# yangliu9527/Object_SLAM

Measured on AMD Instinct MI355X. Metric: frames/sec tracking+localBA, higher is better.
Workload: dtype f64

## Files before the change

include/oslam_hip.h:

```cpp
#ifndef OSLAM_HIP_H
#define OSLAM_HIP_H

#include <stddef.h>
#include <stdint.h>

#ifdef __cplusplus
extern "C" {
#endif

#define OSLAM_OK 0
#define OSLAM_E_INVALID (-1)
#define OSLAM_E_HIP (-2)
#define OSLAM_E_CAPACITY (-3)
#define OSLAM_E_NUMERIC (-4)

#define OSLAM_MAX_LEVELS 16

typedef struct oslam_keypoint {
    float x, y;
    float size;
    float angle;
    float response;
    int32_t octave;
    int32_t class_id;
} oslam_keypoint_t;

const char* oslam_last_error(void);
int oslam_device_count(void);

typedef struct oslam_orb oslam_orb_t;

int oslam_orb_create(oslam_orb_t** out, int nfeatures, float scaleFactor, int nlevels, int iniThFAST,
                     int minThFAST, int width, int height, int max_batch, int device);
void oslam_orb_destroy(oslam_orb_t* h);

int oslam_orb_get_scale_tables(const oslam_orb_t* h, float* scaleFactors, float* invScaleFactors,
                               float* levelSigma2, float* invLevelSigma2, int* nFeaturesPerLevel);
int oslam_orb_set_blur_rounding(oslam_orb_t* h, int sse2);
int oslam_orb_max_keypoints(const oslam_orb_t* h);

int oslam_orb_extract(oslam_orb_t* h, const uint8_t* gray, int width, int height, int stride,
                      oslam_keypoint_t* keypoints, uint8_t* descriptors, int cap, int* n_out);

int oslam_orb_extract_batch_device(oslam_orb_t* h, const uint8_t* d_gray, int batch, int stride,
                                   size_t image_stride, void* stream);
int oslam_orb_results_device(const oslam_orb_t* h, const oslam_keypoint_t** d_keypoints,
                             const uint8_t** d_descriptors, const int32_t** d_counts,
                             const int32_t** d_status);
int oslam_orb_fetch(oslam_orb_t* h, int b, oslam_keypoint_t* keypoints, uint8_t* descriptors, int cap,
                    int* n_out);

int oslam_orb_level_size(const oslam_orb_t* h, int level, int* width, int* height);
int oslam_orb_get_pyramid_level(oslam_orb_t* h, int b, int level, uint8_t* out);
int oslam_orb_pyramid_level_device(const oslam_orb_t* h, int b, int level, const uint8_t** d_ptr,
                                   int* pitch);

int oslam_orb_debug_get_blurred(oslam_orb_t* h, int b, int level, uint8_t* out);
int oslam_orb_debug_get_candidates(oslam_orb_t* h, int b, int level, int32_t* out, int cap, int* n_out);
int oslam_orb_debug_get_level_keys(oslam_orb_t* h, int b, int level, int32_t* out, int cap, int* n_out);

#define OSLAM_ORB_RESIZE_NONE 0
#define OSLAM_ORB_RESIZE_PLAIN 1
#define OSLAM_ORB_RESIZE_WORDS 2
#define OSLAM_ORB_RESIZE_LDS 3
typedef struct oslam_orb_plan {
    int32_t nlevels;
    int32_t batch;
    int32_t n_halves;
    int32_t half_nb[2];
    int32_t half_kpw[2];
    int32_t half_src_aligned4[2];
    int32_t half_src_aligned16[2];
    int32_t half_oct_nodes_hbm[2];
    int32_t half_big_cell_kernel[2];
    int32_t half_resize[2][OSLAM_MAX_LEVELS];
    int32_t big_cell[OSLAM_MAX_LEVELS];
    int32_t skipped_cells[OSLAM_MAX_LEVELS];
} oslam_orb_plan_t;
int oslam_orb_debug_get_plan(const oslam_orb_t* h, oslam_orb_plan_t* out);

int oslam_orb_set_profiling(oslam_orb_t* h, int on);
int oslam_orb_get_profile(oslam_orb_t* h, double ms[5], long long* batches, long long* images);

int oslam_orb_debug_counters(oslam_orb_t* h, unsigned long long out[16], int reset);

int oslam_memcpy_from_device(void* dst, const void* d_src, size_t bytes);
int64_t oslam_orb_algorithmic_bytes(const oslam_orb_t* h, int n_keypoints);
// ... 119 lines not shown
                       float bf, float b, float* uRight, float* depth);
int oslam_stereo_match_batch_device(oslam_stereo_t* h, oslam_orb_t* orbL, oslam_orb_t* orbR, int batch, int kp_stride,
                                    const oslam_keypoint_t* d_kpL, const uint8_t* d_descL, const int32_t* d_nL,
                                    int nL_const, const oslam_keypoint_t* d_kpR, const uint8_t* d_descR,
                                    const int32_t* d_nR, int nR_const, int nlevels, float bf, float b, void* stream);
int oslam_stereo_results_device(const oslam_stereo_t* h, const float** d_uRight, const float** d_depth,
                                const int32_t** d_n_matched);

typedef struct oslam_poseopt oslam_poseopt_t;
int oslam_poseopt_create(oslam_poseopt_t** out, int max_batch, int max_points , int device);
void oslam_poseopt_destroy(oslam_poseopt_t* h);
int oslam_pose_optimize(oslam_poseopt_t* h, int N, const float Tcw_in[16], const float* Xw, const float* obs,
                        const float* invSigma2, const uint8_t* has_mp, const float K5[5], float Tcw_out[16],
                        uint8_t* outlier, int32_t* n_inliers, int32_t stats[2] );
int oslam_poseopt_trace(oslam_poseopt_t* h, int cap);
int oslam_poseopt_trace_read(oslam_poseopt_t* h, double* out, int32_t* n);
int oslam_pose_optimize_batch_device(oslam_poseopt_t* h, int batch, int stride, const int32_t* d_n, int n_const,
                                     const float* d_Tcw, const float* d_Xw, const float* d_obs,
                                     const float* d_invSigma2, const uint8_t* d_has_mp, const float K5[5],
                                     void* stream);
int oslam_poseopt_results_device(const oslam_poseopt_t* h, const float** d_Tcw_out, const uint8_t** d_outlier,
                                 const int32_t** d_n_inliers, const int32_t** d_stats);

typedef struct oslam_semantic {
    int32_t nObj, H, W;
    const uint8_t* masks;
    int32_t nObjMp; const float* objmp_Xw; const int32_t* objmp_obj;
    int32_t nJoint; const int32_t* joint_kp; const int32_t* joint_obj;
    const float* kp_uv;
    float bounds[4];
    float invSigma2_0;
} oslam_semantic_t;
int oslam_pose_optimize2(oslam_poseopt_t* h, int N, const float Tcw_in[16], const float* Xw, const float* obs,
                         const float* invSigma2, const uint8_t* has_mp, const float K5[5], const oslam_semantic_t* sem,
                         float Tcw_out[16], uint8_t* outlier, int32_t* n_inliers, int32_t* n_semantic);

typedef struct oslam_sem_frame { int32_t nObj, obj0, nObjMp, objmp0, nJoint, joint0; } oslam_sem_frame_t;
int oslam_pose_optimize2_batch_device(oslam_poseopt_t* h, int batch, int stride, const int32_t* d_n, const float* d_Tcw, const float* d_Xw, const float* d_obs,
                                      const float* d_invSigma2, const uint8_t* d_has_mp, const float K5[5], const oslam_sem_frame_t* d_frames, int total_obj,
                                      const uint8_t* const* d_mask_ptrs, int H, int W, int mask_pitch, int total_objmp, const float* d_objmp_Xw,
                                      const int32_t* d_objmp_obj, int total_joint, const int32_t* d_joint_kp, const int32_t* d_joint_obj, const float bounds[4],
                                      float invSigma2_0, void* stream);
int oslam_poseopt_semantic_results_device(const oslam_poseopt_t* h, const int32_t** d_n_semantic);
int oslam_mask_bits_device(const uint8_t* const* d_mask_ptrs, int n, int H, int W, int pitch, uint64_t* d_bits, void* stream);
int oslam_poseopt_use_mask_bits(oslam_poseopt_t* h, const uint64_t* d_bits, const int32_t* d_bits_index);
int oslam_frame_object_kp_test_bits_batch_device(const oslam_keypoint_t* d_keysUn, int kp_stride, const int32_t* d_n_kps, int batch, const uint64_t* d_bits,
                                                 const int32_t* d_mask0, const int32_t* d_n_masks, int H, int W, uint8_t* d_out, void* stream);
int oslam_frame_object_kp_test_batch_device(const oslam_keypoint_t* d_keysUn, int kp_stride, const int32_t* d_n_kps, int batch, const uint8_t* const* d_mask_ptrs,
                                            const int32_t* d_mask0, const int32_t* d_n_masks, int H, int W, int mask_pitch, uint8_t* d_out, void* stream);

typedef struct oslam_lba oslam_lba_t;
int oslam_lba_create(oslam_lba_t** out, int max_batch, int max_keyframes , int max_points,
                     int max_edges, int device);
void oslam_lba_destroy(oslam_lba_t* h);
volatile int32_t* oslam_lba_stop_flag(oslam_lba_t* h);
int oslam_lba_set_mode(oslam_lba_t* h, int wide);
int oslam_lba_set_schur(oslam_lba_t* h, int mode);
int oslam_lba_kernel_time(oslam_lba_t* h, int enable, double* ms_out, long long* launches_out);
int oslam_lba_trace(oslam_lba_t* h, int cap);
int oslam_lba_trace_read(oslam_lba_t* h, double* out, int32_t* n);
int oslam_lba_set_solver(oslam_lba_t* h, int mode);
int oslam_lba_debug_stats(oslam_lba_t* h, int32_t out[16]);
int oslam_lba_optimize(oslam_lba_t* h, int nKF, const float* poses, const uint8_t* fixed, int nP,
                       const float* points, int nE, const int32_t* edge_kf, const int32_t* edge_pt,
                       const float* edge_obs, const float* edge_invSigma2, const float K5[5], int use_stop_flag,
                       float* poses_out, float* points_out, uint8_t* erase,
                       int32_t stats[4] );

typedef struct oslam_lba_problem {
    int32_t nKF; const float* poses; const uint8_t* fixed;
    int32_t nP; const float* points;
    int32_t nE; const int32_t* edge_kf; const int32_t* edge_pt; const float* edge_obs; const float* edge_invSigma2;
    float* poses_out; float* points_out; uint8_t* erase; int32_t* stats;
} oslam_lba_problem_t;
int oslam_lba_optimize_batch(oslam_lba_t* h, int n, const oslam_lba_problem_t* probs, const float K5[5]);

int oslam_ba_optimize(oslam_lba_t* h, int nKF, const float* poses, const uint8_t* fixed, int nP, const float* points, int nE,
                      const int32_t* edge_kf, const int32_t* edge_pt, const float* edge_obs, const float* edge_invSigma2,
                      const float K5[5], int nIterations, int bRobust, int use_stop_flag, float* poses_out, float* points_out);

typedef struct oslam_mappoint oslam_mappoint_t;
int oslam_mappoint_create(oslam_mappoint_t** out, int device);
void oslam_mappoint_destroy(oslam_mappoint_t* h);
int oslam_bow_kernel_time(oslam_bow_t* h, int enable, double* ms_out, long long* launches_out);
int oslam_mappoint_kernel_time(oslam_mappoint_t* h, int enable, double* ms_out, long long* launches_out);

int oslam_mp_distinctive_descriptors(oslam_mappoint_t* h, int P, const int32_t* obs_start, const uint8_t* obs_desc ,
                                     int32_t* best_idx , uint8_t* out_desc );

int oslam_mp_update_normal_depth(oslam_mappoint_t* h, int P, const float* Pos , const int32_t* obs_start, const float* obs_Ow ,
                                 const float* OwRef , const float* levelScaleFactor , float lastScaleFactor, float* out );

int oslam_mp_update_fused_device(int P, int do_desc, int do_normal, const int32_t* d_obs_start, const int32_t* d_desc_start, const int32_t* d_rec, const uint8_t* const* d_rec_desc,
                                 const float* d_obs_Ow, const float* d_Pos, const float* d_OwRef, const float* d_lsf, float lastScale, const int32_t* d_items, uint8_t* const* d_tab,
                                 int32_t* o_best, uint8_t* o_desc, float* o_out5, void* stream);
int oslam_mp_update_windows_device(int P, const int32_t* d_items, uint8_t* const* d_tab, const int32_t* d_e0, const int32_t* d_ne, const int32_t* d_kbase, const int32_t* d_ref,
                                   const float* d_lsf, const uint8_t* d_skip, const float* d_Pos, const int32_t* d_edge_kf, const uint8_t* d_erase, const float* d_Ow, float lastScale,
                                   float* d_out5, void* stream);
int oslam_mp_table_write_device(int P, const int32_t* d_items, uint8_t* const* d_tab, const int32_t* d_obs_start, const int32_t* d_desc_start, const float* d_Pos,
                                const float* d_out5, const uint8_t* d_out_desc, int do_desc, int do_normal, void* stream);
int oslam_pose_inputs_gather_device(int batch, int stride, const int32_t* d_slots, const int32_t* d_n, const int32_t* d_ids, uint8_t* const* d_tab,
                                    const oslam_keypoint_t* d_keysUn, const float* d_uRight, int kp_stride, const float* invLevelSigma2, int nLevels,
                                    float* d_Xw, float* d_obs, float* d_invSigma2, uint8_t* d_has_mp, void* stream);
int oslam_fuse_queries_device(int n, int stride, const int32_t* d_slots, const int32_t* d_M, const int32_t* d_ids, const uint8_t* d_excl, uint8_t* const* d_tab,
                              const float* d_Tcw, const float* d_Ow, const float K5[5], const float bounds[4], float th, float logScaleFactor,
                              const float* scaleFactors, int nLevels, oslam_proj_query_t* d_q, void* stream);
// ... 649 lines not shown
```

include/oslam_slam.h:

```cpp
#ifndef OSLAM_SLAM_H
#define OSLAM_SLAM_H

#include "oslam_hip.h"

#ifdef __cplusplus
extern "C" {
#endif

typedef struct oslam_slam oslam_slam_t;

typedef struct oslam_slam_config {
    int32_t width, height;
    float fx, fy, cx, cy;
    float dist[5]; int32_t ndist;
    float bf;
    float thDepth;
    float fps;
    int32_t nFeatures; float scaleFactor; int32_t nLevels, iniThFAST, minThFAST;
    int32_t n_sequences;
    int32_t device;
    int32_t host_threads;
    int32_t local_mapping;
    int32_t sensor;
} oslam_slam_config_t;

#define OSLAM_SLAM_LM_DEFERRED 0x20
#define OSLAM_SLAM_NOT_INITIALIZED 1
#define OSLAM_SLAM_OK 2
#define OSLAM_SLAM_LOST 3

typedef struct oslam_slam_frame {
    int32_t N;
    oslam_keypoint_t* keys;
    oslam_keypoint_t* keysUn;
    uint8_t* desc;
    float* uRight;
    float* depth;
} oslam_slam_frame_t;

typedef struct oslam_job_search_last {
    int32_t slot;
    const oslam_slam_frame_t* cur;
    int32_t Nlast; const float* Xw; const uint8_t* has_mp; const oslam_keypoint_t* last_keysUn; const uint8_t* mp_desc;
    float Tcw[16], Tlw[16]; float th;
    int32_t* kp_match;
    int32_t nmatches;
    const int32_t* mp_ids;
} oslam_job_search_last_t;

typedef struct oslam_job_search_local {
    int32_t slot; const oslam_slam_frame_t* cur; const uint8_t* blocked ;
    int32_t M; const float* Pw; const float* Pn; const float* maxDist; const float* minDist; const uint8_t* obs_gt0; const uint8_t* mp_desc;
    float Tcw[16]; float th;
    const uint8_t* skip;
    int64_t content_id;
    uint8_t* in_view;
    int32_t* kp_match;
    int32_t nmatches;
    const int32_t* local_ids;
} oslam_job_search_local_t;

typedef struct oslam_job_pose {
    int32_t slot; int32_t N; float Tcw_in[16];
    const float* Xw; const float* obs; const float* invSigma2; const uint8_t* has_mp;
    float Tcw_out[16]; uint8_t* outlier; int32_t n_inliers;
    const int32_t* mp_ids;
} oslam_job_pose_t;

typedef struct oslam_job_mp_update {
    int32_t P; const int32_t* obs_start; const uint8_t* obs_desc; const float* obs_Ow;
    const float* Pos; const float* OwRef; const float* levelScaleFactor;
    int32_t do_desc, do_normal;
    const int32_t* items;
    const int32_t* desc_start;
    int32_t* best_idx; uint8_t* out_desc; float* out5;
} oslam_job_mp_update_t;

typedef struct oslam_job_mp_window {
    int32_t slot;
    int32_t nP, nE, nK;
    const int32_t* pt_ids;
    const int32_t* pt_start;
    const int32_t* edge_kf;
// ... 173 lines not shown
```

object_slam_amd/_lib.py:

```python
import contextlib
import ctypes as C
import os

import numpy as np

HERE = os.path.dirname(os.path.abspath(__file__))
LIB_PATH = os.environ.get("OSLAM_LIB_PATH") or os.path.join(HERE, "liboslam_hip.so")

KP_DTYPE = np.dtype([("x", "<f4"), ("y", "<f4"), ("size", "<f4"), ("angle", "<f4"),
                     ("response", "<f4"), ("octave", "<i4"), ("class_id", "<i4")])

OSLAM_E_INVALID, OSLAM_E_HIP, OSLAM_E_CAPACITY, OSLAM_E_NUMERIC = -1, -2, -3, -4


class OslamError(RuntimeError):
    def __init__(self, code, msg):
        super().__init__("oslam error %d: %s" % (code, msg))
        self.code = code


_lib = None


def lib():
    global _lib
    if _lib is None:
        if not os.path.exists(LIB_PATH):
            raise OslamError(OSLAM_E_HIP, "%s not built: run python -m object_slam_amd.build "
                             "(the HIP path has no CPU fallback)" % LIB_PATH)
        try:
            import torch
        except ImportError:
            pass
        L = C.CDLL(LIB_PATH)
        L.oslam_last_error.restype = C.c_char_p
        L.oslam_orb_algorithmic_bytes.restype = C.c_int64
        L.oslam_orb_algorithmic_bytes.argtypes = [C.c_void_p, C.c_int]
        L.oslam_orb_create.argtypes = [C.POINTER(C.c_void_p), C.c_int, C.c_float, C.c_int, C.c_int, C.c_int,
                                       C.c_int, C.c_int, C.c_int, C.c_int]
        L.oslam_orb_destroy.argtypes = [C.c_void_p]
        L.oslam_orb_extract_batch_device.argtypes = [C.c_void_p, C.c_void_p, C.c_int, C.c_int, C.c_size_t, C.c_void_p]
        _lib = L
    return _lib


def check(rc):
    if rc != 0:
        raise OslamError(rc, lib().oslam_last_error().decode())


def ptr(a):
    return C.c_void_p(a.__array_interface__["data"][0])


def optptr(a):
    return None if a is None else ptr(a)


class Handle:

    def __init__(self, L, prefix, *args):
        self.L, self.h, self._destroy = L, C.c_void_p(), prefix + "_destroy"
        check(getattr(L, prefix + "_create")(C.byref(self.h), *args))

    def close(self):
        h = getattr(self, "h", None)
        if h is not None and h.value:
            getattr(self.L, self._destroy)(h)
            h.value = None

    def __del__(self):
        try:
            self.close()
        except Exception:
            pass


def upload(a):
    if a is None:
        return None
    import torch
    return torch.from_numpy(np.ascontiguousarray(a).view(np.uint8).reshape(-1) if a.size else np.zeros(8, np.uint8)).to(torch.device("cuda", torch.cuda.current_device()))


@contextlib.contextmanager
def device_call(arrays, outputs):
    import torch
    t = {id(a): upload(a) for a in arrays if a is not None}
    torch.cuda.synchronize()
    side = torch.cuda.Stream()
    with torch.cuda.stream(side):
        yield (lambda a: None if a is None else t[id(a)].data_ptr()), C.c_void_p(side.cuda_stream)
    side.synchronize()
    for a in outputs:
        if a is not None and a.size:
            a.reshape(-1).view(np.uint8)[:] = t[id(a)].cpu().numpy()[:a.nbytes]
# ... 1 lines not shown
```

object_slam_amd/csrc/bow_matcher.hip:

```cpp
#include <hip/hip_runtime.h>
#include <stdint.h>

#include <algorithm>
#include <vector>

#include "common.h"
#include "slam_pool.h"

namespace oslam {

constexpr int kBowThreads = 1024;
constexpr int kBowMaxKps = 2400;
constexpr int kBowHisto = 30;

struct BowCtx {
    int mode;
    int nq; const int* q_idx1; const uint32_t* q_node;
    int N1; const oslam_keypoint_t* keys1; const uint8_t* desc1; const float* uRight1; const uint8_t* flag1;
    int N2; const oslam_keypoint_t* keys2; const uint8_t* desc2; const float* uRight2; const uint8_t* has_mp2;
    int nNodes; const uint32_t* nodes; const int* start; const int* items;
    float nnratio; int checkOri; int bOnlyStereo;
    float F12[9], ex, ey, scale[OSLAM_MAX_LEVELS], sigma2[OSLAM_MAX_LEVELS];
    int* out; int* nmatches; int* q_best;
};
// ... 146 lines not shown
            int bin = (int)roundf(rot * factor);
            if (bin == kBowHisto) bin = 0;
            if (bin != s_ind[0] && bin != s_ind[1] && bin != s_ind[2]) {
                removed++;
                if (c.mode == 0) c.out[k] = -2; else c.out[idx1] = c.mode == 2 ? -2 : -1;
            }
        }
        if (removed) atomicSub(&s_nm, removed);
        __syncthreads();
    }
    if (tid == 0) *c.nmatches = s_nm;
}

__global__ __launch_bounds__(kBowThreads) void k_search_bow(BowCtx c, int ncap) { bow_body(c, ncap); }
__global__ __launch_bounds__(kBowThreads) void k_search_bow_batch(const BowCtx* cs, int ncap) { bow_body(cs[blockIdx.x], ncap); }

}

using namespace oslam;

struct oslam_bow {
    int device = 0, max_kps = 0;
    size_t lds = 0;
    DeviceBuffer q_idx1, q_node, keys1, desc1, ur1, flag1, keys2, desc2, ur2, mp2, nodes, start, items, out, qbest, nm;
    StagePair st;
    hipStream_t strm = nullptr;
    bool owns_strm = true;
    int timing = 0; hipEvent_t ev0 = nullptr, ev1 = nullptr; double kern_ms = 0; long long kern_n = 0;
};

static int bow_up(DeviceBuffer& b, const void* src, size_t bytes) {
    int rc = b.grow(bytes ? bytes : 4, 256);
    if (rc) return rc;
    if (bytes && src) OSLAM_HIP_CHECK(hipMemcpy(b.ptr(), src, bytes, hipMemcpyHostToDevice));
    return OSLAM_OK;
}

extern "C" {

int oslam_bow_kernel_time(oslam_bow_t* h, int enable, double* ms_out, long long* launches_out) {
    if (!h) { set_error("NULL handle"); return OSLAM_E_INVALID; }
    OSLAM_HIP_CHECK(hipSetDevice(h->device));
    if (enable && !h->ev0) { OSLAM_HIP_CHECK(hipEventCreate(&h->ev0)); OSLAM_HIP_CHECK(hipEventCreate(&h->ev1)); }
    if (ms_out) *ms_out = h->kern_ms;
    if (launches_out) *launches_out = h->kern_n;
    h->kern_ms = 0; h->kern_n = 0; h->timing = enable;
    return OSLAM_OK;
}

void oslam_bow_destroy(oslam_bow_t* h) {
    if (!h) return;
    if (h->ev0) (void)hipEventDestroy(h->ev0);
    if (h->ev1) (void)hipEventDestroy(h->ev1);
    if (h->strm && h->owns_strm) (void)hipStreamDestroy(h->strm);
    delete h;
}

extern "C++" {
namespace oslam {
void bow_use_stream(oslam_bow* h, hipStream_t s) {
    if (!h || !s) return;
    if (h->strm && h->owns_strm) (void)hipStreamDestroy(h->strm);
    h->strm = s; h->owns_strm = false;
}
}
}

int oslam_bow_create(oslam_bow_t** out, int max_keypoints, int device) {
    if (!out) { set_error("out is NULL"); return OSLAM_E_INVALID; }
    *out = nullptr;
    if (max_keypoints < 1 || max_keypoints > kBowMaxKps) { set_error("oslam_bow_create: max_keypoints must be in [1,%d]", kBowMaxKps); return OSLAM_E_INVALID; }
    int ndev = oslam_device_count();
    if (ndev <= 0) { set_error("no HIP device visible: the gfx950 BoW matchers have no CPU fallback"); return OSLAM_E_HIP; }
    if (device < 0 || device >= ndev) { set_error("device out of range"); return OSLAM_E_INVALID; }
    OSLAM_HIP_CHECK(hipSetDevice(device));
    oslam_bow* h = new oslam_bow();
    h->device = device; h->max_kps = max_keypoints;
    h->lds = (size_t)max_keypoints * 40 + 64;
    OSLAM_HIP_CHECK(hipFuncSetAttribute((const void*)k_search_bow, hipFuncAttributeMaxDynamicSharedMemorySize, (int)h->lds));
    *out = h;
    return OSLAM_OK;
}

static int bow_run(oslam_bow_t* h, int mode, const oslam_bow_side1_t* s1, const oslam_bow_side2_t* s2, float nnratio, int checkOri,
                   const float* F12, float ex, float ey, const float* scaleFactors, const float* levelSigma2, int nlevels, int bOnlyStereo,
                   int32_t* out, int32_t* nmatches) {
    if (!h || !s1 || !s2 || !out || !nmatches) { set_error("NULL argument"); return OSLAM_E_INVALID; }
    if (s1->N < 0 || s2->N < 0 || s1->nq < 0 || s2->nNodes < 0 || s2->N > h->max_kps || s1->N > 65536 * 16) { set_error("keypoint counts exceed capacity %d", h->max_kps); return OSLAM_E_CAPACITY; }
    for (int q = 0; q < s1->nq; q++)
        if (s1->q_idx[q] < 0 || s1->q_idx[q] >= s1->N) { set_error("side-1 index out of range"); return OSLAM_E_INVALID; }
    const int nitems = s2->nNodes ? s2->start[s2->nNodes] : 0;
    for (int i = 0; i < nitems; i++)
        if (s2->items[i] < 0 || s2->items[i] >= s2->N) { set_error("side-2 index out of range"); return OSLAM_E_INVALID; }
    for (int i = 1; i < s2->nNodes; i++)
        if (!(s2->nodes[i - 1] < s2->nodes[i])) { set_error("side-2 node ids must be strictly ascending"); return OSLAM_E_INVALID; }
    OSLAM_HIP_CHECK(hipSetDevice(h->device));
    int rc;
    std::vector<float> negs((size_t)std::max(std::max(s1->N, s2->N), 1), -1.0f);
    std::vector<uint8_t> zeros((size_t)std::max(std::max(s1->N, s2->N), 1), 0);
    if ((rc = bow_up(h->q_idx1, s1->q_idx, (size_t)s1->nq * 4)) || (rc = bow_up(h->q_node, s1->q_node, (size_t)s1->nq * 4)) ||
        (rc = bow_up(h->keys1, s1->keys, (size_t)s1->N * sizeof(oslam_keypoint_t))) || (rc = bow_up(h->desc1, s1->desc, (size_t)s1->N * 32)) ||
        (rc = bow_up(h->ur1, s1->uRight ? s1->uRight : negs.data(), (size_t)s1->N * 4)) || (rc = bow_up(h->flag1, s1->flag ? s1->flag : zeros.data(), (size_t)s1->N)) ||
        (rc = bow_up(h->keys2, s2->keys, (size_t)s2->N * sizeof(oslam_keypoint_t))) || (rc = bow_up(h->desc2, s2->desc, (size_t)s2->N * 32)) ||
        (rc = bow_up(h->ur2, s2->uRight ? s2->uRight : negs.data(), (size_t)s2->N * 4)) || (rc = bow_up(h->mp2, s2->has_mp ? s2->has_mp : zeros.data(), (size_t)s2->N)) ||
        (rc = bow_up(h->nodes, s2->nodes, (size_t)s2->nNodes * 4)) || (rc = bow_up(h->start, s2->start, (size_t)(s2->nNodes + 1) * 4)) ||
        (rc = bow_up(h->items, s2->items, (size_t)nitems * 4)) || (rc = h->out.grow((size_t)std::max(std::max(s1->N, s2->N), 1) * 4, 256)) ||
        (rc = h->qbest.grow((size_t)std::max(s1->nq, 1) * 4, 256)) || (rc = h->nm.grow(4, 256)))
        return rc;
    BowCtx c;
    memset(&c, 0, sizeof(c));
    c.mode = mode; c.nq = s1->nq; c.q_idx1 = (const int*)h->q_idx1.ptr(); c.q_node = (const uint32_t*)h->q_node.ptr();
    c.N1 = s1->N; c.keys1 = (const oslam_keypoint_t*)h->keys1.ptr(); c.desc1 = (const uint8_t*)h->desc1.ptr(); c.uRight1 = (const float*)h->ur1.ptr(); c.flag1 = (const uint8_t*)h->flag1.ptr();
    c.N2 = s2->N; c.keys2 = (const oslam_keypoint_t*)h->keys2.ptr(); c.desc2 = (const uint8_t*)h->desc2.ptr(); c.uRight2 = (const float*)h->ur2.ptr(); c.has_mp2 = (const uint8_t*)h->mp2.ptr();
    c.nNodes = s2->nNodes; c.nodes = (const uint32_t*)h->nodes.ptr(); c.start = (const int*)h->start.ptr(); c.items = (const int*)h->items.ptr();
    c.nnratio = nnratio; c.checkOri = checkOri; c.bOnlyStereo = bOnlyStereo;
// ... 69 lines not shown
        Off& o = off[i];
        o.nitems = nitems; o.nout = jobs[i].triangulation ? s1.N : s2.N;
        const bool r1 = res && res[i].d_keys1 && res[i].d_desc1, r2 = res && res[i].d_keys2 && res[i].d_desc2;
        const bool u1 = r1 && res[i].d_uRight1 && s1.uRight, u2 = r2 && res[i].d_uRight2 && s2.uRight;
        o.q_idx = take((size_t)s1.nq * 4); o.q_node = take((size_t)s1.nq * 4);
        o.keys1 = r1 ? 0 : take((size_t)s1.N * sizeof(oslam_keypoint_t)); o.desc1 = r1 ? 0 : take((size_t)s1.N * 32);
        o.ur1 = u1 ? 0 : take((size_t)s1.N * 4); o.flag1 = take((size_t)s1.N);
        o.keys2 = r2 ? 0 : take((size_t)s2.N * sizeof(oslam_keypoint_t)); o.desc2 = r2 ? 0 : take((size_t)s2.N * 32);
        o.ur2 = u2 ? 0 : take((size_t)s2.N * 4); o.mp2 = take((size_t)s2.N); o.nodes = take((size_t)s2.nNodes * 4); o.start = take((size_t)(s2.nNodes + 1) * 4);
        o.items = take((size_t)nitems * 4);
    }
    const size_t in_bytes = at;
    for (int i = 0; i < n; i++) { off[i].out = take((size_t)std::max(off[i].nout, 1) * 4); off[i].nm = take(4); }
    const size_t io_bytes = at;
    for (int i = 0; i < n; i++) off[i].qbest = take((size_t)std::max(jobs[i].s1.nq, 1) * 4);
    OSLAM_HIP_CHECK(hipSetDevice(h->device));
    if (at > h->st.cap()) OSLAM_HIP_CHECK(hipDeviceSynchronize());
    OSLAM_CHECK(h->st.grow(at, 0));
    uint8_t* H = h->st.h.bytes();
    uint8_t* D = h->st.d.bytes();
    BowCtx* cs = (BowCtx*)H;
    oslam_drv::shared_parallel_for(n, [&](int i) {
        const oslam_bow_job_t& j = jobs[i];
        const oslam_bow_side1_t& s1 = j.s1;
        const oslam_bow_side2_t& s2 = j.s2;
        const Off& o = off[i];
        memcpy(H + o.q_idx, s1.q_idx, (size_t)s1.nq * 4); memcpy(H + o.q_node, s1.q_node, (size_t)s1.nq * 4);
        if (o.keys1) { memcpy(H + o.keys1, s1.keys, (size_t)s1.N * sizeof(oslam_keypoint_t)); memcpy(H + o.desc1, s1.desc, (size_t)s1.N * 32); }
        if (o.ur1) { if (s1.uRight) memcpy(H + o.ur1, s1.uRight, (size_t)s1.N * 4); else for (int k = 0; k < s1.N; k++) ((float*)(H + o.ur1))[k] = -1.0f; }
        if (s1.flag) memcpy(H + o.flag1, s1.flag, (size_t)s1.N); else memset(H + o.flag1, 0, (size_t)s1.N);
        if (o.keys2) { memcpy(H + o.keys2, s2.keys, (size_t)s2.N * sizeof(oslam_keypoint_t)); memcpy(H + o.desc2, s2.desc, (size_t)s2.N * 32); }
        if (o.ur2) { if (s2.uRight) memcpy(H + o.ur2, s2.uRight, (size_t)s2.N * 4); else for (int k = 0; k < s2.N; k++) ((float*)(H + o.ur2))[k] = -1.0f; }
        if (s2.has_mp) memcpy(H + o.mp2, s2.has_mp, (size_t)s2.N); else memset(H + o.mp2, 0, (size_t)s2.N);
        memcpy(H + o.nodes, s2.nodes, (size_t)s2.nNodes * 4);
        if (s2.nNodes) memcpy(H + o.start, s2.start, (size_t)(s2.nNodes + 1) * 4); else *(int*)(H + o.start) = 0;
        memcpy(H + o.items, s2.items, (size_t)o.nitems * 4);
        BowCtx& c = cs[i];
        memset(&c, 0, sizeof(c));
        c.mode = j.triangulation == 2 ? 2 : (j.triangulation ? 1 : 0); c.nq = s1.nq; c.q_idx1 = (const int*)(D + o.q_idx); c.q_node = (const uint32_t*)(D + o.q_node);
        c.N1 = s1.N; c.keys1 = o.keys1 ? (const oslam_keypoint_t*)(D + o.keys1) : res[i].d_keys1; c.desc1 = o.desc1 ? D + o.desc1 : res[i].d_desc1;
        c.uRight1 = o.ur1 ? (const float*)(D + o.ur1) : res[i].d_uRight1; c.flag1 = D + o.flag1;
        c.N2 = s2.N; c.keys2 = o.keys2 ? (const oslam_keypoint_t*)(D + o.keys2) : res[i].d_keys2; c.desc2 = o.desc2 ? D + o.desc2 : res[i].d_desc2;
        c.uRight2 = o.ur2 ? (const float*)(D + o.ur2) : res[i].d_uRight2; c.has_mp2 = D + o.mp2;
        c.nNodes = s2.nNodes; c.nodes = (const uint32_t*)(D + o.nodes); c.start = (const int*)(D + o.start); c.items = (const int*)(D + o.items);
        c.nnratio = j.nnratio; c.checkOri = j.checkOri; c.bOnlyStereo = 0;
        for (int k = 0; k < 9; k++) c.F12[k] = j.F12[k];
        c.ex = j.ex; c.ey = j.ey;
        for (int k = 0; k < OSLAM_MAX_LEVELS; k++) {
            c.scale[k] = (scaleFactors && k < nlevels) ? scaleFactors[k] : 0.f;
            c.sigma2[k] = (levelSigma2 && k < nlevels) ? levelSigma2[k] : 0.f;
        }
        c.out = (int*)(D + o.out); c.nmatches = (int*)(D + o.nm); c.q_best = (int*)(D + o.qbest);
    });
    if (!h->strm) OSLAM_HIP_CHECK(hipStreamCreateWithFlags(&h->strm, hipStreamNonBlocking));
    OSLAM_HIP_CHECK(hipMemcpyAsync(D, H, in_bytes, hipMemcpyHostToDevice, h->strm));
    if (h->timing) (void)hipEventRecord(h->ev0, h->strm);
    hipLaunchKernelGGL(k_search_bow_batch, dim3(n), dim3(kBowThreads), h->lds, h->strm, (const BowCtx*)D, h->max_kps);
    if (h->timing) (void)hipEventRecord(h->ev1, h->strm);
    OSLAM_HIP_CHECK(hipGetLastError());
    OSLAM_HIP_CHECK(hipMemcpyAsync(H + in_bytes, D + in_bytes, io_bytes - in_bytes, hipMemcpyDeviceToHost, h->strm));
    OSLAM_HIP_CHECK(stream_wait(h->strm));
    if (h->timing) { float ms = 0.f; if (hipEventElapsedTime(&ms, h->ev0, h->ev1) == hipSuccess) { h->kern_ms += ms; h->kern_n += 1; } }
    for (int i = 0; i < n; i++) {
        jobs[i].nmatches = *(const int*)(H + off[i].nm);
        if (jobs[i].nmatches < 0) { set_error("BoW matcher kernel rejected pair %d (capacity)", i); return OSLAM_E_CAPACITY; }
        memcpy(jobs[i].match, H + off[i].out, (size_t)off[i].nout * 4);
    }
    return OSLAM_OK;
}
```

object_slam_amd/csrc/common.h:

```cpp
#pragma once
#include <hip/hip_runtime.h>
#include <mutex>

#include <cstdarg>
#include <cstdint>
#include <cstdio>
#include <cstdlib>
#include <cstring>

#include "../../include/oslam_hip.h"
#include "device_buffer.h"

namespace oslam {

void set_error(const char* fmt, ...);

#define OSLAM_HIP_CHECK(expr)                                                              \
    do {                                                                                   \
        hipError_t _e = (expr);                                                            \
        if (_e != hipSuccess) {                                                            \
            oslam::set_error("%s failed: %s (%s:%d)", #expr, hipGetErrorString(_e), __FILE__, __LINE__); \
            return OSLAM_E_HIP;                                                            \
        }                                                                                  \
    } while (0)
#define OSLAM_CHECK(expr) do { const int rc_ = (expr); if (rc_) return rc_; } while (0)

hipError_t stream_wait(hipStream_t s);
void stream_wait_thread_mode(int spin_us);
void lba_use_stream(struct ::oslam_lba* h, hipStream_t s);
void lba_use_gate(struct ::oslam_lba* h, std::mutex* gate);
void bow_use_stream(struct ::oslam_bow* h, hipStream_t s);
void mappoint_use_stream(struct ::oslam_mappoint* h, hipStream_t s);

static inline int no_device(const char* fn) {
    set_error("no HIP device visible: %s has no CPU fallback", fn);
    return OSLAM_E_HIP;
}

static inline int div_up(int a, int b) { return (a + b - 1) / b; }

hipError_t copy_to_host_async(void* dst_pinned, const void* src_dev, size_t bytes, hipStream_t s);
static inline size_t align_up(size_t a, size_t b) { return (a + b - 1) / b * b; }

struct PinStage {
    PinnedBuffer blk;
    size_t off = 0;
    void reset() { off = 0; }
    int reserve_total(size_t bytes) {
        if (bytes > blk.cap()) OSLAM_HIP_CHECK(hipDeviceSynchronize());
        return blk.grow(bytes, 4096);
    }
    uint8_t* take(size_t bytes) { uint8_t* at = blk.bytes() + off; off += align_up(bytes ? bytes : 1, 256); return at; }
    int upload(void* dst, const void* src, size_t bytes) {
        if (!bytes) return OSLAM_OK;
        if (off + align_up(bytes, 256) > blk.cap()) { set_error("pinned staging overflow"); return OSLAM_E_CAPACITY; }
        uint8_t* at = take(bytes);
        memcpy(at, src, bytes);
        OSLAM_HIP_CHECK(hipMemcpyAsync(dst, at, bytes, hipMemcpyHostToDevice, nullptr));
        return OSLAM_OK;
    }
    int download(const void* src, size_t bytes, uint8_t** at_out) {
        if (off + align_up(bytes ? bytes : 1, 256) > blk.cap()) { set_error("pinned staging overflow"); return OSLAM_E_CAPACITY; }
        uint8_t* at = take(bytes);
        if (bytes) OSLAM_HIP_CHECK(hipMemcpyAsync(at, src, bytes, hipMemcpyDeviceToHost, nullptr));
        *at_out = at;
        return OSLAM_OK;
    }
};

}
```

object_slam_amd/csrc/covisibility.hip:

```cpp
#include <climits>
#include <mutex>
#include <vector>

#include "common.h"
#include "stage_layout.h"

using oslam::set_error;

namespace {

constexpr int kThreads = 256, kWaves = kThreads / 64;
constexpr int kTh = 15;
constexpr int kLocalLimit = 80;
constexpr int kBest = 10;
constexpr uint32_t kPtCnt = 0xffu, kPtBad = OSLAM_COVIS_PT_BAD << 8, kPtOvf = OSLAM_COVIS_PT_OVERFLOW << 8;
constexpr uint32_t kKfAll = OSLAM_COVIS_KF_ORDERED_ALL, kKfConnected = OSLAM_COVIS_KF_CONNECTED, kKfBad = OSLAM_COVIS_KF_IS_BAD;
static_assert(OSLAM_COVIS_MAX_OBS == 64, "an observation list is at most one entry per lane");
static_assert(OSLAM_COVIS_MAX_KEYFRAMES <= 2048, "three rows of K ints and two bitsets in LDS");

struct CovisState {
    int2* obs;
    uint32_t* pmeta;
    int32_t* weights;
    uint32_t* kmeta;
    int32_t* parent;
    int n_graphs, K, P, C, W;
};

size_t lds_bytes(int K, int W) { return ((size_t)3 * K + 2 * W) * 4; }

}

struct oslam_covis {
    int device = 0;
    size_t lds = 0;
    CovisState st{};
    oslam::DeviceBuffer obs, pmeta, weights, kmeta, parent, unsorted;
    hipStream_t stream = nullptr;
    oslam::StagePair io;
    std::mutex mu;
    ~oslam_covis() { if (stream) (void)hipStreamDestroy(stream); }
};

namespace {

struct Shared {
    int wcnt[kWaves];
    int nnz, nq, tmp;
    unsigned long long lo, hi, key;
};

__device__ int compact(bool hit, int base, Shared& s, int* total) {
    const int lane = threadIdx.x & 63, wave = threadIdx.x >> 6;
    const unsigned long long m = __ballot(hit);
    if (lane == 0) s.wcnt[wave] = __popcll(m);
    __syncthreads();
    int before = 0, all = 0;
    for (int w = 0; w < kWaves; w++) { const int c = s.wcnt[w]; before += w < wave ? c : 0; all += c; }
    __syncthreads();
    *total = all;
    return base + before + __popcll(m & ((1ull << lane) - 1ull));
}

__device__ void row_stats(const int32_t* row, int K, Shared& s) {
    if (threadIdx.x == 0) { s.nnz = 0; s.nq = 0; s.lo = 0; s.hi = 0; }
    __syncthreads();
    int nnz = 0, nq = 0;
    unsigned long long lo = 0, hi = 0;
    for (int o = threadIdx.x; o < K; o += kThreads) {
        const int w = row[o];
        if (w > 0) {
            nnz++; nq += w >= kTh ? 1 : 0;
            const unsigned long long klo = ((unsigned long long)w << 32) | (0xffffffffu - (uint32_t)o), khi = ((unsigned long long)w << 32) | (uint32_t)o;
            lo = klo > lo ? klo : lo; hi = khi > hi ? khi : hi;
        }
    }
    if (nnz) { atomicAdd(&s.nnz, nnz); atomicAdd(&s.nq, nq); atomicMax(&s.lo, lo); atomicMax(&s.hi, hi); }
    __syncthreads();
}
__device__ inline int lo_id(const Shared& s) { return (int)(0xffffffffu - (uint32_t)s.lo); }
__device__ inline int hi_id(const Shared& s) { return (int)(uint32_t)s.hi; }

__device__ inline bool in_ordered(int w, int o, bool all, int nq, int lo) { return w > 0 && (all || w >= kTh || (nq == 0 && o == lo)); }

__device__ int emit_ordered(const int32_t* row, bool all, int K, int max_n, int min_w, int32_t* out_ids, int32_t* out_w, int* s_q, int* s_qw, Shared& s) {
    row_stats(row, K, s);
    const int nq = s.nq, lo = lo_id(s);
    int m = 0;
    for (int o0 = 0; o0 < K; o0 += kThreads) {
        const int o = o0 + threadIdx.x, w = o < K ? row[o] : 0;
        const bool hit = o < K && in_ordered(w, o, all, nq, lo);
        int n;
        const int pos = compact(hit, m, s, &n);
        if (hit) { s_q[pos] = o; s_qw[pos] = w; }
// ... 397 lines not shown
    if (!h) { set_error("%s: NULL handle", fn); return OSLAM_E_INVALID; }
    if (n < 0 || n2 < 0 || n3 < 0) { set_error("%s: a count is negative", fn); return OSLAM_E_INVALID; }
    return OSLAM_OK;
}

bool span_ok(int off, int n, int total) { return n >= 0 && off >= 0 && off <= total - n; }

}

extern "C" {

void oslam_covis_destroy(oslam_covis_t* h) {
    if (!h) return;
    delete h;
}

static int covis_clear(oslam_covis* h, size_t g0, size_t ng) {
    const size_t K = (size_t)h->st.K, P = (size_t)h->st.P, C = (size_t)h->st.C;
    OSLAM_HIP_CHECK(hipMemsetAsync(h->obs.bytes() + g0 * P * C * 8, 0, ng * P * C * 8, h->stream));
    OSLAM_HIP_CHECK(hipMemsetAsync(h->pmeta.bytes() + g0 * P * 4, 0, ng * P * 4, h->stream));
    OSLAM_HIP_CHECK(hipMemsetAsync(h->weights.bytes() + g0 * K * K * 4, 0, ng * K * K * 4, h->stream));
    OSLAM_HIP_CHECK(hipMemsetAsync(h->kmeta.bytes() + g0 * K * 4, 0, ng * K * 4, h->stream));
    OSLAM_HIP_CHECK(hipMemsetAsync(h->parent.bytes() + g0 * K * 4, 0xff, ng * K * 4, h->stream));
    return OSLAM_OK;
}

int oslam_covis_create(oslam_covis_t** out, int n_graphs, int max_keyframes, int max_points, int obs_cap, int device) {
    const char* fn = "oslam_covis_create";
    if (!out) { set_error("%s: out is NULL", fn); return OSLAM_E_INVALID; }
    *out = nullptr;
    if (n_graphs < 1 || max_keyframes < 1 || max_keyframes > OSLAM_COVIS_MAX_KEYFRAMES || max_points < 1 || obs_cap < 1 || obs_cap > OSLAM_COVIS_MAX_OBS) {
        set_error("%s: n_graphs %d, max_keyframes %d (1 .. %d), max_points %d or obs_cap %d (1 .. %d) out of range", fn, n_graphs, max_keyframes, OSLAM_COVIS_MAX_KEYFRAMES,
                  max_points, obs_cap, OSLAM_COVIS_MAX_OBS);
        return OSLAM_E_INVALID;
    }
    const size_t G = (size_t)n_graphs, K = (size_t)max_keyframes, P = (size_t)max_points, C = (size_t)obs_cap;
    if (G * K * K > (1ull << 34) || G * P * C > (1ull << 34)) { set_error("%s: %zu graphs of this size are more than the handle holds", fn, G); return OSLAM_E_INVALID; }
    const int ndev = oslam_device_count();
    if (ndev <= 0) return oslam::no_device(fn);
    if (device < 0 || device >= ndev) { set_error("%s: device out of range", fn); return OSLAM_E_INVALID; }
    OSLAM_HIP_CHECK(hipSetDevice(device));
    oslam_covis* h = new oslam_covis;
    h->device = device;
    const int W = oslam::div_up(max_keyframes, 32);
    h->lds = lds_bytes(max_keyframes, W);
    int rc = OSLAM_OK;
    if ((rc = h->obs.alloc(G * P * C * 8)) || (rc = h->pmeta.alloc(G * P * 4)) || (rc = h->weights.alloc(G * K * K * 4)) || (rc = h->kmeta.alloc(G * K * 4)) ||
        (rc = h->parent.alloc(G * K * 4)) || (rc = h->unsorted.alloc(4))) {
        delete h;
        return rc;
    }
    h->st = CovisState{h->obs.as<int2>(), h->pmeta.as<uint32_t>(), h->weights.as<int32_t>(), h->kmeta.as<uint32_t>(), h->parent.as<int32_t>(), n_graphs, max_keyframes,
                       max_points, obs_cap, W};
    hipError_t e = hipStreamCreateWithFlags(&h->stream, hipStreamNonBlocking);
    if (e == hipSuccess) {
        rc = covis_clear(h, 0, G);
        if (rc == OSLAM_OK) e = hipStreamSynchronize(h->stream);
    }
    if (e != hipSuccess || rc != OSLAM_OK) {
        if (e != hipSuccess) set_error("%s: %s", fn, hipGetErrorString(e));
        delete h;
        return rc ? rc : OSLAM_E_HIP;
    }
    *out = h;
    return OSLAM_OK;
}

int oslam_covis_reset(oslam_covis_t* h, int n, const int32_t* graphs) {
    const char* fn = "oslam_covis_reset";
    if (!h || n < 0 || (n > 0 && !graphs)) { set_error("%s: bad argument", fn); return OSLAM_E_INVALID; }
    if (n == 0) return OSLAM_OK;
    std::lock_guard<std::mutex> lock(h->mu);
    for (int r = 0; r < n; r++)
        if (graphs[r] < 0 || graphs[r] >= h->st.n_graphs) { set_error("%s: record %d names graph %d of %d", fn, r, graphs[r], h->st.n_graphs); return OSLAM_E_INVALID; }
    OSLAM_HIP_CHECK(hipSetDevice(h->device));
    for (int r = 0; r < n; r++) OSLAM_CHECK(covis_clear(h, (size_t)graphs[r], 1));
    OSLAM_HIP_CHECK(hipStreamSynchronize(h->stream));
    return OSLAM_OK;
}

int oslam_covis_apply(oslam_covis_t* h, int n_events, const oslam_covis_event_t* events, int32_t* n_overflow_out) {
    const char* fn = "oslam_covis_apply";
    OSLAM_CHECK(check_counts(fn, h, n_events));
    if (!n_overflow_out || (n_events > 0 && !events)) { set_error("%s: NULL argument", fn); return OSLAM_E_INVALID; }
    std::lock_guard<std::mutex> lock(h->mu);
    const int K = h->st.K, P = h->st.P, G = h->st.n_graphs;
    for (int i = 0; i < n_events; i++) {
        const oslam_covis_event_t& e = events[i];
        const bool kf_a = e.a >= 0 && e.a < K, kf_b = e.b >= 0 && e.b < K, pt_a = e.a >= 0 && e.a < P;
        bool ok = e.graph >= 0 && e.graph < G;
        switch (e.type) {
            case OSLAM_COVIS_EV_OBS_ADD: case OSLAM_COVIS_EV_OBS_ERASE: ok = ok && pt_a && kf_b; break;
            case OSLAM_COVIS_EV_POINT_BAD: ok = ok && pt_a; break;
            case OSLAM_COVIS_EV_CONN_ADD: ok = ok && kf_a && kf_b && e.c > 0; break;
            case OSLAM_COVIS_EV_CONN_ERASE: case OSLAM_COVIS_EV_PARENT_SET: ok = ok && kf_a && kf_b; break;
            case OSLAM_COVIS_EV_KF_BAD: ok = ok && kf_a; break;
            default: ok = false;
        }
        if (!ok) { set_error("%s: event %d {graph %d, type %d, %d, %d, %d} names an id outside the handle or has an unknown type", fn, i, e.graph, e.type, e.a, e.b, e.c); return OSLAM_E_INVALID; }
    }
    OSLAM_HIP_CHECK(hipSetDevice(h->device));
    oslam::StageLayout lay;
    const auto fEv = lay.add<oslam_covis_event_t>((size_t)n_events);
    const auto fOv = lay.add<int32_t>((size_t)G);
    OSLAM_CHECK(h->io.grow(lay.total(), 4096));
    uint8_t *ph = h->io.h.bytes(), *pd = h->io.d.bytes();
    put(fEv, ph, events);
// ... 241 lines not shown
```

object_slam_amd/csrc/keyframe_db.hip:

```cpp
#include <algorithm>
#include <climits>
#include <cmath>
#include <mutex>
#include <vector>

#include "common.h"
#include "kfdb_state.h"
#include "lane_ops.h"
#include "stage_layout.h"

using oslam::KfdbState;
using oslam::set_error;

namespace {

constexpr int kThreads = 512, kGroup = 16, kGroups = kThreads / kGroup;
constexpr int kChunk = OSLAM_KFDB_CHUNK, kCovis = OSLAM_KFDB_COVIS;
constexpr int kMutThreads = 256;

struct AddRec { int32_t slot, n_words, word_off, chunk_off; uint32_t serial; };

__global__ __launch_bounds__(kMutThreads) void k_kfdb_add(KfdbState st, const AddRec* recs, const uint32_t* ids, const double* vals, const int32_t* chunk_list) {
    const AddRec r = recs[blockIdx.x];
    const int nc = (r.n_words + kChunk - 1) / kChunk;
// ... 399 lines not shown

void free_slot(oslam_kfdb* h, size_t slot) {
    const int nw = h->h_nwords[slot];
    if (nw < 0) return;
    for (int i = 0; i < oslam::div_up(nw, kChunk); i++) h->free_chunks.push_back(h->h_chunks[slot * h->st.MC + i]);
    h->h_nwords[slot] = -1;
    h->n_present--;
}

int stage_up(oslam_kfdb* h, size_t bytes) {
    OSLAM_HIP_CHECK(hipMemcpyAsync(h->io.d.bytes(), h->io.h.bytes(), bytes, hipMemcpyHostToDevice, h->stream));
    return OSLAM_OK;
}

}

extern "C" {

void oslam_kfdb_destroy(oslam_kfdb_t* h) {
    if (!h) return;
    delete h;
}

int oslam_kfdb_create(oslam_kfdb_t** out, int n_databases, int max_keyframes, int max_words, long long pool_words, int device) {
    const char* fn = "oslam_kfdb_create";
    if (!out) { set_error("%s: out is NULL", fn); return OSLAM_E_INVALID; }
    *out = nullptr;
    if (n_databases < 1 || max_keyframes < 1 || max_words < 1 || pool_words < 1) { set_error("%s: bad argument", fn); return OSLAM_E_INVALID; }
    if (max_keyframes > OSLAM_KFDB_MAX_KEYFRAMES || max_words > OSLAM_KFDB_MAX_WORDS) {
        set_error("%s: max_keyframes %d > %d or max_words %d > %d (the query vector and the per-slot scratch of a query live in LDS)", fn, max_keyframes, OSLAM_KFDB_MAX_KEYFRAMES,
                  max_words, OSLAM_KFDB_MAX_WORDS);
        return OSLAM_E_INVALID;
    }
    const long long S = (long long)n_databases * max_keyframes, n_chunks = (pool_words + kChunk - 1) / kChunk;
    if (S > (1ll << 28) || n_chunks > (1ll << 24)) { set_error("%s: %lld slots or %lld chunks are more than the handle's index types hold", fn, S, n_chunks); return OSLAM_E_INVALID; }
    const int ndev = oslam_device_count();
    if (ndev <= 0) return oslam::no_device(fn);
    if (device < 0 || device >= ndev) { set_error("%s: device out of range", fn); return OSLAM_E_INVALID; }
    OSLAM_HIP_CHECK(hipSetDevice(device));
    oslam_kfdb* h = new oslam_kfdb;
    h->device = device;
    const int MC = oslam::div_up(max_words, kChunk);
    int P = 1;
    while (P < max_keyframes) P <<= 1;
    h->P = P;
    h->lds = lds_bytes(max_keyframes, max_words, P);
    h->n_chunks = n_chunks;
    int rc = OSLAM_OK;
    if ((rc = h->nwords.alloc((size_t)S * 4)) || (rc = h->serial.alloc((size_t)S * 4)) || (rc = h->reloc.alloc((size_t)S * 4)) || (rc = h->covis.alloc((size_t)S * kCovis * 4)) ||
        (rc = h->chunks.alloc((size_t)S * MC * 4)) || (rc = h->pool_ids.alloc((size_t)n_chunks * kChunk * 4)) || (rc = h->pool_vals.alloc((size_t)n_chunks * kChunk * 8))) {
        delete h;
        return rc;
    }
    hipError_t e = hipStreamCreateWithFlags(&h->stream, hipStreamNonBlocking);
    if (e == hipSuccess) e = hipMemsetAsync(h->nwords.ptr(), 0xff, (size_t)S * 4, h->stream);
    if (e == hipSuccess) e = hipMemsetAsync(h->serial.ptr(), 0, (size_t)S * 4, h->stream);
    if (e == hipSuccess) e = hipMemsetAsync(h->reloc.ptr(), 0, (size_t)S * 4, h->stream);
    if (e == hipSuccess) e = hipMemsetAsync(h->covis.ptr(), 0xff, (size_t)S * kCovis * 4, h->stream);
    if (e == hipSuccess) e = hipMemsetAsync(h->chunks.ptr(), 0, (size_t)S * MC * 4, h->stream);
    if (e == hipSuccess) e = hipMemsetAsync(h->pool_ids.ptr(), 0, (size_t)n_chunks * kChunk * 4, h->stream);
    if (e == hipSuccess) e = hipMemsetAsync(h->pool_vals.ptr(), 0, (size_t)n_chunks * kChunk * 8, h->stream);
    if (e == hipSuccess) e = hipFuncSetAttribute((const void*)k_kfdb_query, hipFuncAttributeMaxDynamicSharedMemorySize,
                                                 (int)lds_bytes(OSLAM_KFDB_MAX_KEYFRAMES, OSLAM_KFDB_MAX_WORDS, OSLAM_KFDB_MAX_KEYFRAMES));
    if (e == hipSuccess) e = hipStreamSynchronize(h->stream);
    if (e != hipSuccess) {
        set_error("%s: %s", fn, hipGetErrorString(e));
        delete h;
        return OSLAM_E_HIP;
    }
    h->st = KfdbState{h->nwords.as<int32_t>(), h->serial.as<uint32_t>(), h->reloc.as<float>(), h->covis.as<int32_t>(), h->chunks.as<int32_t>(), h->pool_ids.as<uint32_t>(),
                      h->pool_vals.as<double>(), n_databases, max_keyframes, max_words, MC};
    h->h_nwords.assign((size_t)S, -1);
    h->h_chunks.assign((size_t)S * MC, 0);
    h->next_serial.assign(n_databases, 0);
    h->free_chunks.resize((size_t)n_chunks);
    for (long long i = 0; i < n_chunks; i++) h->free_chunks[i] = (int32_t)(n_chunks - 1 - i);
    *out = h;
    return OSLAM_OK;
}

int oslam_kfdb_info(const oslam_kfdb_t* h, int64_t out[3]) {
    if (!h || !out) { set_error("oslam_kfdb_info: NULL argument"); return OSLAM_E_INVALID; }
    out[0] = (int64_t)h->free_chunks.size(); out[1] = h->n_chunks; out[2] = h->n_present;
    return OSLAM_OK;
}

int oslam_kfdb_add(oslam_kfdb_t* h, int n, const oslam_kfdb_add_t* recs, int n_words_total, const uint32_t* ids, const double* vals) {
    const char* fn = "oslam_kfdb_add";
    if (!h || n < 0 || n_words_total < 0 || (n > 0 && !recs) || (n_words_total > 0 && (!ids || !vals))) { set_error("%s: bad argument", fn); return OSLAM_E_INVALID; }
    if (n == 0) return OSLAM_OK;
    std::lock_guard<std::mutex> lock(h->mu);
    const int K = h->st.K, MC = h->st.MC;
    size_t need = 0;
    std::vector<size_t> slots(n);
    for (int r = 0; r < n; r++) {
        const oslam_kfdb_add_t& A = recs[r];
        if (A.database < 0 || A.database >= h->st.n_db || A.keyframe < 0) { set_error("%s: record %d names database %d, keyframe %d", fn, r, A.database, A.keyframe); return OSLAM_E_INVALID; }
        if (A.keyframe >= K) { set_error("%s: record %d: keyframe %d, a database holds %d", fn, r, A.keyframe, K); return OSLAM_E_CAPACITY; }
        if (A.n_words > h->st.MW) { set_error("%s: record %d has %d words, a keyframe holds %d", fn, r, A.n_words, h->st.MW); return OSLAM_E_CAPACITY; }
        if (A.n_words < 0 || A.word_off < 0 || A.word_off > n_words_total - A.n_words) { set_error("%s: record %d's words lie outside the %d given", fn, r, n_words_total); return OSLAM_E_INVALID; }
        for (int i = 1; i < A.n_words; i++)
            if (ids[A.word_off + i - 1] >= ids[A.word_off + i]) { set_error("%s: record %d's word ids are not strictly ascending at %d", fn, r, i); return OSLAM_E_INVALID; }
        slots[r] = (size_t)A.database * K + A.keyframe;
        if (h->h_nwords[slots[r]] >= 0) { set_error("%s: record %d: keyframe %d of database %d is present already", fn, r, A.keyframe, A.database); return OSLAM_E_INVALID; }
        need += (size_t)oslam::div_up(A.n_words, kChunk);
    }
    {
// ... 138 lines not shown
```

object_slam_amd/csrc/kfdb_state.h:

```cpp
#pragma once
#include <mutex>
#include <vector>

#include "common.h"

namespace oslam {

struct KfdbState {
    int32_t* nwords;
    uint32_t* serial;
    float* reloc;
    int32_t* covis;
    int32_t* chunks;
    uint32_t* pool_ids;
    double* pool_vals;
    int n_db, K, MW, MC;
};

}

struct oslam_kfdb {
    int device = 0, P = 1;
    size_t lds = 0;
    oslam::KfdbState st{};
    oslam::DeviceBuffer nwords, serial, reloc, covis, chunks, pool_ids, pool_vals;
    std::vector<int32_t> h_nwords, h_chunks, free_chunks;
    std::vector<uint32_t> next_serial;
    long long n_chunks = 0, n_present = 0;
    hipStream_t stream = nullptr;
    oslam::StagePair io;
    std::mutex mu;
    ~oslam_kfdb() { if (stream) (void)hipStreamDestroy(stream); }
};

namespace oslam {

int kfdb_check_query_call(const char* fn, const oslam_kfdb* h, const oslam_voc_t* voc, int n_queries, int n_words_total, int n_conn_total);
int kfdb_check_queries(const char* fn, const oslam_kfdb* h, bool loop, int n_queries, const oslam_kfdb_query_t* queries, int n_words_total, const uint32_t* ids, int n_conn_total);
int kfdb_launch_query(oslam_kfdb* h, bool loop, int n_queries, const oslam_kfdb_query_t* d_queries, int n_words_total, const uint32_t* d_ids, const double* d_vals,
                      int n_conn_total, const int32_t* d_conn, int32_t* d_cand, float* d_cand_acc, int32_t* d_n_cand, int32_t* d_diag, float* d_conn_score,
                      float* d_min_score, hipStream_t stream);

}
```

object_slam_amd/csrc/lba.hip:

```cpp
#include <hip/hip_runtime.h>
#include <string.h>
#include <type_traits>
#include <stdint.h>

#include <algorithm>
#include <atomic>
#include <chrono>
#include <mutex>
#include <array>
#include <vector>

#include "common.h"
#include "se3_math.h"
#include "lane_ops.h"
#include "slam_pool.h"

namespace oslam {

#ifdef OSLAM_LBA_PROFILE
#define LBA_STAMP(i) do { if (tid == 0) { long long t_ = clock64(); prof[i] += t_ - tlast; tlast = t_; } } while (0)
#else
#define LBA_STAMP(i) do { } while (0)
#endif

// ... 1917 lines not shown
    return OSLAM_OK;
}

extern "C" {

int oslam_lba_kernel_time(oslam_lba_t* h, int enable, double* ms_out, long long* launches_out) {
    if (!h) { set_error("NULL handle"); return OSLAM_E_INVALID; }
    OSLAM_HIP_CHECK(hipSetDevice(h->device));
    if (enable && !h->ev0) { OSLAM_HIP_CHECK(hipEventCreate(&h->ev0)); OSLAM_HIP_CHECK(hipEventCreate(&h->ev1)); }
    if (ms_out) *ms_out = h->kern_ms;
    if (launches_out) *launches_out = h->kern_launches;
    h->kern_ms = 0; h->kern_launches = 0;
    h->timing = enable;
    return OSLAM_OK;
}

static double* s_lba_trace_buf = nullptr;
static int s_lba_trace_cap = 0;
int oslam_lba_trace(oslam_lba_t* h, int cap) {
    if (!h || cap < 0) { set_error("oslam_lba_trace: bad argument"); return OSLAM_E_INVALID; }
    OSLAM_HIP_CHECK(hipSetDevice(h->device));
    OSLAM_HIP_CHECK(hipDeviceSynchronize());
    double* none = nullptr; int zero = 0;
    OSLAM_HIP_CHECK(hipMemcpyToSymbol(HIP_SYMBOL(g_lba_trace), &none, sizeof(none)));
    OSLAM_HIP_CHECK(hipMemcpyToSymbol(HIP_SYMBOL(g_lba_trace_cap), &zero, sizeof(zero)));
    if (s_lba_trace_buf) (void)hipFree(s_lba_trace_buf);
    s_lba_trace_buf = nullptr; s_lba_trace_cap = 0;
    if (cap == 0) return OSLAM_OK;
    OSLAM_HIP_CHECK(hipMalloc((void**)&s_lba_trace_buf, sizeof(double) * (1 + 6 * (size_t)cap)));
    OSLAM_HIP_CHECK(hipMemset(s_lba_trace_buf, 0, sizeof(double) * (1 + 6 * (size_t)cap)));
    s_lba_trace_cap = cap;
    OSLAM_HIP_CHECK(hipMemcpyToSymbol(HIP_SYMBOL(g_lba_trace), &s_lba_trace_buf, sizeof(s_lba_trace_buf)));
    OSLAM_HIP_CHECK(hipMemcpyToSymbol(HIP_SYMBOL(g_lba_trace_cap), &cap, sizeof(cap)));
    return OSLAM_OK;
}

int oslam_lba_trace_read(oslam_lba_t* h, double* out, int32_t* n) {
    if (!h || !out || !n || !s_lba_trace_buf) { set_error("oslam_lba_trace_read: no trace"); return OSLAM_E_INVALID; }
    OSLAM_HIP_CHECK(hipSetDevice(h->device));
    OSLAM_HIP_CHECK(hipDeviceSynchronize());
    double cnt = 0;
    OSLAM_HIP_CHECK(hipMemcpy(&cnt, s_lba_trace_buf, sizeof(double), hipMemcpyDeviceToHost));
    OSLAM_HIP_CHECK(hipMemcpy(out, s_lba_trace_buf + 1, sizeof(double) * 6 * (size_t)s_lba_trace_cap, hipMemcpyDeviceToHost));
    OSLAM_HIP_CHECK(hipMemset(s_lba_trace_buf, 0, sizeof(double)));
    *n = (int32_t)cnt;
    return OSLAM_OK;
}

void oslam_lba_destroy(oslam_lba_t* h) {
    if (!h) return;
    (void)hipSetDevice(h->device);
    if (h->ev0) (void)hipEventDestroy(h->ev0);
    if (h->ev1) (void)hipEventDestroy(h->ev1);
    if (h->strm && h->owns_strm) (void)hipStreamDestroy(h->strm);
    delete h;
}

extern "C++" {
namespace oslam {
void lba_use_gate(oslam_lba* h, std::mutex* gate) { if (h) h->launch_gate = gate; }
void lba_use_stream(oslam_lba* h, hipStream_t s) {
    if (!h || !s) return;
    if (h->strm && h->owns_strm) { (void)hipStreamSynchronize(h->strm); (void)hipStreamDestroy(h->strm); }
    h->strm = s; h->owns_strm = false;
}
}
}

int oslam_lba_create(oslam_lba_t** out, int max_batch, int max_keyframes, int max_points, int max_edges, int device) {
    if (!out) { set_error("out is NULL"); return OSLAM_E_INVALID; }
    *out = nullptr;
    if (max_batch < 1 || max_keyframes < 1 || max_keyframes > kLbaMaxWindowKF || max_points < 1 || max_edges < 1) {
        set_error("oslam_lba_create: invalid argument (max_keyframes <= %d)", kLbaMaxWindowKF);
        return OSLAM_E_INVALID;
    }
    int ndev = oslam_device_count();
    if (ndev <= 0) { set_error("no HIP device visible: the gfx950 local BA has no CPU fallback"); return OSLAM_E_HIP; }
    if (device < 0 || device >= ndev) { set_error("device out of range"); return OSLAM_E_INVALID; }
    OSLAM_HIP_CHECK(hipSetDevice(device));
    oslam_lba* h = new oslam_lba();
    if (hipStreamCreateWithFlags(&h->strm, hipStreamNonBlocking) != hipSuccess) { set_error("hipStreamCreate failed"); delete h; return OSLAM_E_HIP; }
    h->device = device; h->max_batch = max_batch; h->max_kf = max_keyframes;
    if (const int rc = h->h_stop.alloc_mapped(sizeof(int))) { oslam_lba_destroy(h); return rc; }
    *h->h_stop.as<int>() = 0;
    if (hipHostGetDevicePointer((void**)&h->d_stop, h->h_stop.ptr(), 0) != hipSuccess) { set_error("hipHostGetDevicePointer failed"); oslam_lba_destroy(h); return OSLAM_E_HIP; }
    h->lds = kRowBufBytes + 64;
    h->win_lds_max = kWinLdsMax;
    if (hipFuncSetAttribute((const void*)k_lba, hipFuncAttributeMaxDynamicSharedMemorySize, (int)h->lds) != hipSuccess ||
        hipFuncSetAttribute((const void*)k_w_chol<true>, hipFuncAttributeMaxDynamicSharedMemorySize, kCholLdsN * (kCholLdsN + 1) * (int)sizeof(double)) != hipSuccess ||
        hipFuncSetAttribute((const void*)k_w_chol_mfma, hipFuncAttributeMaxDynamicSharedMemorySize, kMB * (kMfmaMaxN + 2 * kMB) * (int)sizeof(double)) != hipSuccess ||
        hipFuncSetAttribute((const void*)k_lba_win, hipFuncAttributeMaxDynamicSharedMemorySize, kWinLdsMax) != hipSuccess ||
        hipFuncSetAttribute((const void*)k_w_schur_tiles, hipFuncAttributeMaxDynamicSharedMemorySize, kWinLdsMax) != hipSuccess ||
        hipFuncSetAttribute((const void*)k_w_chol_packed, hipFuncAttributeMaxDynamicSharedMemorySize, kCholPackedLds) != hipSuccess ||
        hipFuncSetAttribute((const void*)k_w_chol_lds_mfma, hipFuncAttributeMaxDynamicSharedMemorySize, (int)chol16_lds_bytes(kCholLdsMfmaN)) != hipSuccess) {
        set_error("hipFuncSetAttribute failed"); oslam_lba_destroy(h); return OSLAM_E_HIP;
    }
    *out = h;
    return OSLAM_OK;
}

int oslam_lba_debug_stats(oslam_lba_t* h, int32_t out[16]) {
    if (!h || h->n_prep < 1 || !h->out_h.ptr()) return OSLAM_E_INVALID;
    memcpy(out, h->out_h.bytes() + h->prep[0].o_out_stats, 64);
    return OSLAM_OK;
}

int oslam_lba_set_mode(oslam_lba_t* h, int wide) {
    if (!h || wide < 0 || wide > 2) { set_error("oslam_lba_set_mode: mode must be 0 (compact), 1 (wide) or 2 (one workgroup per window, LDS-resident)"); return OSLAM_E_INVALID; }
    h->wide = wide;
    return OSLAM_OK;
}

int oslam_lba_set_schur(oslam_lba_t* h, int mode) {
    if (!h || mode < 0 || mode > 3) { set_error("oslam_lba_set_schur: mode must be 0 (pair gather), 1 (LDS tiles), 2 (per call) or 3 (pair gather, host-built lists)"); return OSLAM_E_INVALID; }
    h->schur_tiles = mode == 3 ? 0 : mode;
    h->device_pairs = mode != 3;
    return OSLAM_OK;
}

int oslam_lba_set_solver(oslam_lba_t* h, int mode) {
    if (!h || mode < 0 || mode > 4) { set_error("oslam_lba_set_solver: bad argument"); return OSLAM_E_INVALID; }
    h->chol_mode = mode;
    return OSLAM_OK;
}

volatile int32_t* oslam_lba_stop_flag(oslam_lba_t* h) { return h ? h->h_stop.as<volatile int32_t>() : nullptr; }

}

static int lba_build_tiles(oslam_lba::Prep& q, const std::vector<int>& blk, int nfree, int nP, int nE, size_t region_bytes, char* err, size_t errn) {
#pragma clang diagnostic push
#pragma clang diagnostic ignored "-Wformat-security"
    auto fail = [&](int rc, const char* fmt, auto... a) { snprintf(err, errn, fmt, a...); return rc; };
#pragma clang diagnostic pop
// ... 618 lines not shown
```

object_slam_amd/csrc/mappoint.hip:

```cpp
#include <hip/hip_runtime.h>
#include <stdint.h>

#include <string.h>

#include <algorithm>
#include <atomic>
#include <mutex>
#include <vector>

#include "common.h"
#include "small_svd.h"

namespace oslam {

constexpr int kDdMaxObs = 128;

__global__ __launch_bounds__(256) void k_distinctive(int P, const int* obs_start, const uint8_t* obs_desc, int* best_idx, uint8_t* out_desc) {
    const int lane = threadIdx.x & 63, wv = threadIdx.x >> 6;
    const int p = blockIdx.x * 4 + wv;
    __shared__ uint32_t s_d[4][kDdMaxObs * 8];
    if (p >= P) return;
    const int s = obs_start[p], N = obs_start[p + 1] - s;
    if (N <= 0) { if (lane == 0) best_idx[p] = -1; return; }
    const uint32_t* g = (const uint32_t*)(obs_desc + (size_t)s * 32);
// ... 139 lines not shown
    if (ok) {
        float r = (double)viewCos > 0.998 ? 2.5f : 4.0f;
        if (th != 1.0f) r *= th;
        q.u = u; q.v = v; q.ur = u - c.bf * invz;
        q.radius = r * c.scale[nScale];
        q.minLevel = nScale - 1; q.maxLevel = nScale;
        q.flags = 1 | (c.obs_gt0[i] ? 2 : 0);
        q.angle = viewCos;
    }
    const uint32_t* sd = (const uint32_t*)(c.mp_desc + (size_t)i * 32);
    uint32_t* qd = (uint32_t*)q.desc;
#pragma unroll
    for (int w = 0; w < 8; w++) qd[w] = ok ? sd[w] : 0u;
    *out = q;
    return ok;
}

}

using namespace oslam;

struct oslam_mappoint {
    int device = 0;
    DeviceBuffer a, b, c, d, e, e2, f, g, g2, o1, o2;
    StagePair st;
    hipStream_t strm = nullptr;
    bool owns_strm = true;
    int timing = 0; hipEvent_t ev0 = nullptr, ev1 = nullptr; double kern_ms = 0; long long kern_n = 0;
};

static int mp_up(DeviceBuffer& b, const void* src, size_t bytes) {
    int rc = b.grow(bytes ? bytes : 4, 256);
    if (rc) return rc;
    if (bytes && src) OSLAM_HIP_CHECK(hipMemcpy(b.ptr(), src, bytes, hipMemcpyHostToDevice));
    return OSLAM_OK;
}

extern "C" {

int oslam_mappoint_kernel_time(oslam_mappoint_t* h, int enable, double* ms_out, long long* launches_out) {
    if (!h) { set_error("NULL handle"); return OSLAM_E_INVALID; }
    OSLAM_HIP_CHECK(hipSetDevice(h->device));
    if (enable && !h->ev0) { OSLAM_HIP_CHECK(hipEventCreate(&h->ev0)); OSLAM_HIP_CHECK(hipEventCreate(&h->ev1)); }
    if (ms_out) *ms_out = h->kern_ms;
    if (launches_out) *launches_out = h->kern_n;
    h->kern_ms = 0; h->kern_n = 0; h->timing = enable;
    return OSLAM_OK;
}

void oslam_mappoint_destroy(oslam_mappoint_t* h) {
    if (!h) return;
    if (h->ev0) (void)hipEventDestroy(h->ev0);
    if (h->ev1) (void)hipEventDestroy(h->ev1);
    if (h->strm && h->owns_strm) (void)hipStreamDestroy(h->strm);
    delete h;
}

extern "C++" {
namespace oslam {
void mappoint_use_stream(oslam_mappoint* h, hipStream_t s) {
    if (!h || !s) return;
    if (h->strm && h->owns_strm) (void)hipStreamDestroy(h->strm);
    h->strm = s; h->owns_strm = false;
}
}
}

int oslam_mappoint_create(oslam_mappoint_t** out, int device) {
    if (!out) { set_error("out is NULL"); return OSLAM_E_INVALID; }
    *out = nullptr;
    int ndev = oslam_device_count();
    if (ndev <= 0) { set_error("no HIP device visible: the gfx950 map-point kernels have no CPU fallback"); return OSLAM_E_HIP; }
    if (device < 0 || device >= ndev) { set_error("device out of range"); return OSLAM_E_INVALID; }
    OSLAM_HIP_CHECK(hipSetDevice(device));
    oslam_mappoint* h = new oslam_mappoint();
    h->device = device;
    *out = h;
    return OSLAM_OK;
}

int oslam_mp_distinctive_descriptors(oslam_mappoint_t* h, int P, const int32_t* obs_start, const uint8_t* obs_desc, int32_t* best_idx, uint8_t* out_desc) {
    if (!h || P < 0 || (P > 0 && (!obs_start || !best_idx || !out_desc))) { set_error("bad argument"); return OSLAM_E_INVALID; }
    if (P == 0) return OSLAM_OK;
    const int total = obs_start[P];
    if (total < 0 || (total > 0 && !obs_desc)) { set_error("bad observation table"); return OSLAM_E_INVALID; }
    for (int p = 0; p < P; p++) if (obs_start[p + 1] < obs_start[p]) { set_error("obs_start not monotone"); return OSLAM_E_INVALID; }
    OSLAM_HIP_CHECK(hipSetDevice(h->device));
    int rc;
    if ((rc = mp_up(h->a, obs_start, (size_t)(P + 1) * 4)) || (rc = mp_up(h->b, obs_desc, (size_t)total * 32)) || (rc = h->o1.grow((size_t)P * 4, 256)) ||
        (rc = h->o2.grow((size_t)P * 32, 256)))
        return rc;
    OSLAM_HIP_CHECK(hipMemset(h->o2.ptr(), 0, (size_t)P * 32));
    hipLaunchKernelGGL(k_distinctive, dim3(div_up(P, 4)), dim3(256), 0, nullptr, P, (const int*)h->a.ptr(), (const uint8_t*)h->b.ptr(), (int*)h->o1.ptr(), (uint8_t*)h->o2.ptr());
    OSLAM_HIP_CHECK(hipGetLastError());
    OSLAM_HIP_CHECK(hipMemcpy(best_idx, h->o1.ptr(), (size_t)P * 4, hipMemcpyDeviceToHost));
    OSLAM_HIP_CHECK(hipMemcpy(out_desc, h->o2.ptr(), (size_t)P * 32, hipMemcpyDeviceToHost));
    return OSLAM_OK;
}

__global__ __launch_bounds__(256) void k_mp_table_write(int P, const int32_t* items, uint8_t* const* tab, const int32_t* obs_start, const int32_t* desc_start,
                                                        const float* Pos, const float* out5, const uint8_t* out_desc, int do_desc, int do_normal) {
    const int i = blockIdx.x * 32 + (threadIdx.x >> 3), part = threadIdx.x & 7;
    if (i >= P) return;
    uint32_t* rec = (uint32_t*)(tab[items[2 * i]] + (size_t)items[2 * i + 1] * 64);
    const bool has_obs = obs_start[i + 1] > obs_start[i];
    if (do_normal) {
        const uint32_t* ps = (const uint32_t*)(Pos + (size_t)i * 3);
        const uint32_t* o5 = (const uint32_t*)(out5 + (size_t)i * 5);
        if (part < 3) rec[part] = ps[part];
        else if (has_obs) rec[part] = part < 6 ? o5[part - 3] : part == 6 ? o5[4] : o5[3];
    }
    if (!has_obs) return;
    if (do_desc && desc_start[i + 1] > desc_start[i]) rec[8 + part] = ((const uint32_t*)(out_desc + (size_t)i * 32))[part];
}

// ... 751 lines not shown
    auto put = [&](const oslam_tri_kf_t& k, size_t off) {
        if (!k.n_kps) return;
        memcpy(&kun[off], k.keysUn, (size_t)k.n_kps * sizeof(oslam_keypoint_t));
        memcpy(&kraw[off], k.keys, (size_t)k.n_kps * sizeof(oslam_keypoint_t));
        memcpy(&ur[off], k.uRight, (size_t)k.n_kps * 4);
        memcpy(&dep[off], k.depth, (size_t)k.n_kps * 4);
    };
    put(*kf1, 0);
    for (int p = 0; p < nPairs; p++) put(kf2[p], (size_t)dev2[p].kp_off);
    int rc;
    if ((rc = mp_up(h->a, kun.data(), total * sizeof(oslam_keypoint_t))) || (rc = mp_up(h->b, kraw.data(), total * sizeof(oslam_keypoint_t))) ||
        (rc = mp_up(h->c, ur.data(), total * 4)) || (rc = mp_up(h->d, dep.data(), total * 4)) || (rc = mp_up(h->e, dev2.data(), dev2.size() * sizeof(TriKfDev))) ||
        (rc = mp_up(h->f, pair_of.data(), (size_t)M * 4)) || (rc = mp_up(h->g, idx1, (size_t)M * 4)) || (rc = mp_up(h->g2, idx2, (size_t)M * 4)) ||
        (rc = h->o1.grow((size_t)M, 256)) || (rc = h->o2.grow((size_t)M * 12, 256)))
        return rc;
    TriCtx c;
    c.M = M; c.nLevels = nLevels;
    fill(c.kf1, *kf1, 0);
    c.kf1s = nullptr;
    c.kf2 = (const TriKfDev*)h->e.ptr(); c.pair_of = (const int*)h->f.ptr(); c.idx1 = (const int*)h->g.ptr(); c.idx2 = (const int*)h->g2.ptr();
    c.keysUn = (const oslam_keypoint_t*)h->a.ptr(); c.keys = (const oslam_keypoint_t*)h->b.ptr(); c.uRight = (const float*)h->c.ptr(); c.depth = (const float*)h->d.ptr();
    for (int i = 0; i < OSLAM_MAX_LEVELS; i++) { c.scale[i] = i < nLevels ? scaleFactors[i] : 1.f; c.sigma2[i] = i < nLevels ? levelSigma2[i] : 1.f; }
    c.ratioFactor = ratioFactor;
    c.ok = (uint8_t*)h->o1.ptr(); c.x3D = (float*)h->o2.ptr();
    hipLaunchKernelGGL(k_triangulate, dim3(div_up(M, 128)), dim3(128), 0, nullptr, c);
    OSLAM_HIP_CHECK(hipGetLastError());
    OSLAM_HIP_CHECK(hipMemcpy(ok, h->o1.ptr(), (size_t)M, hipMemcpyDeviceToHost));
    OSLAM_HIP_CHECK(hipMemcpy(x3D, h->o2.ptr(), (size_t)M * 12, hipMemcpyDeviceToHost));
    if (nnew) { int n = 0; for (int m = 0; m < M; m++) n += ok[m]; *nnew = n; }
    return OSLAM_OK;
}

extern "C" int oslam_mp_triangulate_pairs(oslam_mappoint_t* h, int nPairs, const oslam_tri_kf_t* kf1, const oslam_tri_kf_t* kf2, const int32_t* pair_start,
                                          const int32_t* idx1, const int32_t* idx2, const float* scaleFactors, const float* levelSigma2, int nLevels,
                                          float ratioFactor, uint8_t* ok, float* x3D) {
    if (!h || nPairs < 0 || (nPairs > 0 && (!kf1 || !kf2 || !pair_start)) || !scaleFactors || !levelSigma2 || nLevels < 1 || nLevels > OSLAM_MAX_LEVELS) {
        set_error("bad argument");
        return OSLAM_E_INVALID;
    }
    const int M = nPairs ? pair_start[nPairs] : 0;
    if (M == 0) return OSLAM_OK;
    if (M < 0 || !idx1 || !idx2 || !ok || !x3D || pair_start[0] != 0) { set_error("bad match table"); return OSLAM_E_INVALID; }
    OSLAM_HIP_CHECK(hipSetDevice(h->device));
    size_t at = 0;
    auto take = [&](size_t bytes) { const size_t o = at; at += (bytes + 255) & ~(size_t)255; return o; };
    const size_t total = (size_t)2 * M;
    const size_t o_kun = take(total * sizeof(oslam_keypoint_t)), o_kraw = take(total * sizeof(oslam_keypoint_t)), o_ur = take(total * 4), o_dep = take(total * 4),
                 o_dev1 = take((size_t)nPairs * sizeof(TriKfDev)), o_dev2 = take((size_t)nPairs * sizeof(TriKfDev)), o_pair = take((size_t)M * 4), o_d1 = take((size_t)M * 4),
                 o_d2 = take((size_t)M * 4);
    const size_t in_bytes = at;
    const size_t o_ok = take((size_t)M), o_x3 = take((size_t)M * 12);
    if (at > h->st.cap()) OSLAM_HIP_CHECK(hipDeviceSynchronize());
    OSLAM_CHECK(h->st.grow(at, 4096));
    if (!h->strm) OSLAM_HIP_CHECK(hipStreamCreateWithFlags(&h->strm, hipStreamNonBlocking));
    uint8_t* H = h->st.h.bytes();
    uint8_t* D = h->st.d.bytes();
    int* pair_of = (int*)(H + o_pair); int* d1 = (int*)(H + o_d1); int* d2 = (int*)(H + o_d2);
    TriKfDev* dev1 = (TriKfDev*)(H + o_dev1); TriKfDev* dev2 = (TriKfDev*)(H + o_dev2);
    oslam_keypoint_t* kun = (oslam_keypoint_t*)(H + o_kun); oslam_keypoint_t* kraw = (oslam_keypoint_t*)(H + o_kraw);
    float* ur = (float*)(H + o_ur); float* dep = (float*)(H + o_dep);
    auto fill = [](TriKfDev& d, const oslam_tri_kf_t& k) {
        for (int i = 0; i < 16; i++) { d.Tcw[i] = k.Tcw[i]; d.Twc[i] = k.Twc[i]; }
        d.fx = k.fx; d.fy = k.fy; d.cx = k.cx; d.cy = k.cy; d.invfx = k.invfx; d.invfy = k.invfy; d.mbf = k.mbf; d.mb = k.mb;
        d.kp_off = 0;
    };
    for (int p = 0; p < nPairs; p++) {
        const oslam_tri_kf_t& a = kf1[p];
        const oslam_tri_kf_t& b = kf2[p];
        if (pair_start[p + 1] < pair_start[p]) { set_error("bad pair %d", p); return OSLAM_E_INVALID; }
        fill(dev1[p], a); fill(dev2[p], b);
        for (int m = pair_start[p]; m < pair_start[p + 1]; m++) {
            if (idx1[m] < 0 || idx1[m] >= a.n_kps || idx2[m] < 0 || idx2[m] >= b.n_kps || !a.keysUn || !a.keys || !a.uRight || !a.depth || !b.keysUn || !b.keys ||
                !b.uRight || !b.depth) { set_error("match %d: keypoint index out of range", m); return OSLAM_E_INVALID; }
            const int o1 = a.keysUn[idx1[m]].octave, o2 = b.keysUn[idx2[m]].octave;
            if (o1 < 0 || o1 >= nLevels || o2 < 0 || o2 >= nLevels) { set_error("match %d: octave out of range", m); return OSLAM_E_INVALID; }
            pair_of[m] = p; d1[m] = 2 * m; d2[m] = 2 * m + 1;
            kun[(size_t)2 * m] = a.keysUn[idx1[m]]; kraw[(size_t)2 * m] = a.keys[idx1[m]]; ur[(size_t)2 * m] = a.uRight[idx1[m]]; dep[(size_t)2 * m] = a.depth[idx1[m]];
            kun[(size_t)2 * m + 1] = b.keysUn[idx2[m]]; kraw[(size_t)2 * m + 1] = b.keys[idx2[m]]; ur[(size_t)2 * m + 1] = b.uRight[idx2[m]]; dep[(size_t)2 * m + 1] = b.depth[idx2[m]];
        }
    }
    OSLAM_HIP_CHECK(hipMemcpyAsync(D, H, in_bytes, hipMemcpyHostToDevice, h->strm));
    TriCtx c;
    c.M = M; c.nLevels = nLevels;
    fill(c.kf1, kf1[0]);
    c.kf1s = (const TriKfDev*)(D + o_dev1);
    c.kf2 = (const TriKfDev*)(D + o_dev2); c.pair_of = (const int*)(D + o_pair); c.idx1 = (const int*)(D + o_d1); c.idx2 = (const int*)(D + o_d2);
    c.keysUn = (const oslam_keypoint_t*)(D + o_kun); c.keys = (const oslam_keypoint_t*)(D + o_kraw); c.uRight = (const float*)(D + o_ur); c.depth = (const float*)(D + o_dep);
    for (int i = 0; i < OSLAM_MAX_LEVELS; i++) { c.scale[i] = i < nLevels ? scaleFactors[i] : 1.f; c.sigma2[i] = i < nLevels ? levelSigma2[i] : 1.f; }
    c.ratioFactor = ratioFactor;
    c.ok = D + o_ok; c.x3D = (float*)(D + o_x3);
    if (h->timing) (void)hipEventRecord(h->ev0, h->strm);
    hipLaunchKernelGGL(k_triangulate, dim3(div_up(M, 128)), dim3(128), 0, h->strm, c);
    if (h->timing) (void)hipEventRecord(h->ev1, h->strm);
    OSLAM_HIP_CHECK(hipGetLastError());
    OSLAM_HIP_CHECK(hipMemcpyAsync(H + o_ok, D + o_ok, at - in_bytes, hipMemcpyDeviceToHost, h->strm));
    OSLAM_HIP_CHECK(stream_wait(h->strm));
    if (h->timing) { float ms = 0.f; if (hipEventElapsedTime(&ms, h->ev0, h->ev1) == hipSuccess) { h->kern_ms += ms; h->kern_n += 1; } }
    memcpy(ok, H + o_ok, (size_t)M);
    memcpy(x3D, H + o_x3, (size_t)M * 12);
    return OSLAM_OK;
}
```

object_slam_amd/csrc/orb_extractor.hip:

```cpp
#include "orb_kernels.hip"

#include <algorithm>
#include <cmath>
#include <vector>

#include "common.h"

#include <time.h>
#include <stdlib.h>

namespace oslam {

static thread_local char g_err[512] = "";
void set_error(const char* fmt, ...) {
    va_list ap;
    va_start(ap, fmt);
    vsnprintf(g_err, sizeof(g_err), fmt, ap);
    va_end(ap);
}

static thread_local int t_wait_mode = -3;
void stream_wait_thread_mode(int spin_us) { t_wait_mode = spin_us; }
hipError_t stream_wait(hipStream_t s) {
    static const int spin_env = [] { const char* e = getenv("OSLAM_WAIT_SPIN_US"); return e ? atoi(e) : -1; }();
    const int spin_us = t_wait_mode != -3 ? t_wait_mode : spin_env;
    if (spin_us == -2) {
        for (;;) {
            const hipError_t q = hipStreamQuery(s);
            if (q != hipErrorNotReady) return q;
#if defined(__x86_64__)
            __builtin_ia32_pause();
#endif
        }
    }
    if (spin_us < 0) return hipStreamSynchronize(s);
    struct Ev { hipEvent_t ev = nullptr; int dev = -1; };
    static thread_local Ev t;
    int dev = 0;
    hipError_t e = hipGetDevice(&dev);
    if (e != hipSuccess) return e;
    if (!t.ev || t.dev != dev) {
        if (t.ev) (void)hipEventDestroy(t.ev);
        t.ev = nullptr;
        if ((e = hipEventCreateWithFlags(&t.ev, hipEventBlockingSync | hipEventDisableTiming)) != hipSuccess) return e;
        t.dev = dev;
    }
    if ((e = hipEventRecord(t.ev, s)) != hipSuccess) return e;
    timespec t0, t1;
    clock_gettime(CLOCK_MONOTONIC, &t0);
    for (;;) {
        e = hipEventQuery(t.ev);
        if (e != hipErrorNotReady) return e;
        clock_gettime(CLOCK_MONOTONIC, &t1);
        if ((t1.tv_sec - t0.tv_sec) * 1000000L + (t1.tv_nsec - t0.tv_nsec) / 1000 > spin_us) break;
#if defined(__x86_64__)
        __builtin_ia32_pause();
#endif
    }
    return hipEventSynchronize(t.ev);
}

__global__ void k_copy_to_host(uint8_t* __restrict__ dst, const uint8_t* __restrict__ src, size_t n16, size_t bytes) {
    const size_t stride = (size_t)gridDim.x * blockDim.x, t0 = (size_t)blockIdx.x * blockDim.x + threadIdx.x;
    for (size_t i = t0; i < n16; i += stride) ((uint4*)dst)[i] = ((const uint4*)src)[i];
    for (size_t i = n16 * 16 + t0; i < bytes; i += stride) dst[i] = src[i];
}
hipError_t copy_to_host_async(void* dst_pinned, const void* src_dev, size_t bytes, hipStream_t s) {
    if (!bytes) return hipSuccess;
    const bool aligned = ((((uintptr_t)dst_pinned) | ((uintptr_t)src_dev)) & 15) == 0;
    const size_t n16 = aligned ? bytes / 16 : 0, units = n16 + (bytes - n16 * 16);
    const int blocks = (int)((units + 255) / 256 < 1024 ? (units + 255) / 256 : 1024);
    hipLaunchKernelGGL(k_copy_to_host, dim3(blocks), dim3(256), 0, s, (uint8_t*)dst_pinned, (const uint8_t*)src_dev, n16, bytes);
    return hipGetLastError();
}

static inline int cv_round(float v) { return (int)lrintf(v); }
static inline int cv_round(double v) { return (int)lrint(v); }
static inline short sat_short(float v) {
    int i = cv_round(v);
    return (short)std::min(std::max(i, -32768), 32767);
}

}

using namespace oslam;

struct oslam_orb {
    int device = 0;
    int nfeatures = 0, nlevels = 0, iniTh = 0, minTh = 0;
    double scaleFactor = 0;
    int width = 0, height = 0, max_batch = 0;
    int blur_sse2 = 1;
    OrbParams P;
    std::vector<float> scale, invScale, sigma2, invSigma2;
    std::vector<int> quota;

    DeviceBuffer dP;
    DeviceBuffer d_rtab;
    DeviceBuffer d_qbase; DeviceBuffer d_qpx;
    DeviceBuffer d_root_of_x;
    DeviceBuffer d_root_x;
    DeviceBuffer d_stage;
    int stage_pitch = 0;
    DeviceBuffer d_pyr;
    long long pyr_stride = 0;
    DeviceBuffer d_blur;
    long long blur_stride = 0;
    DeviceBuffer d_cell_count;
    DeviceBuffer d_cand;
    DeviceBuffer d_fast_cells;
    DeviceBuffer d_ovf_count;
    DeviceBuffer d_ent_g;
    DeviceBuffer d_knode_g;
    DeviceBuffer d_sel;
    DeviceBuffer d_sel_count;
    DeviceBuffer d_out_kp;
    DeviceBuffer d_out_desc;
    DeviceBuffer d_out_count;
    DeviceBuffer d_status;
    DeviceBuffer d_dbg;
    size_t oct_lds = 0;
    DeviceBuffer d_oct_nodes; long long oct_nodes_stride = 0;
    hipStream_t side_stream = nullptr;
    hipEvent_t ev_fork = nullptr, ev_join = nullptr;
    hipStream_t fast0_stream = nullptr;
    hipEvent_t ev_fork0 = nullptr, ev_join0 = nullptr;
    hipStream_t aux_stream = nullptr, aux_side_stream = nullptr;
    hipEvent_t ev_fork2 = nullptr, ev_join2 = nullptr, ev_fork3 = nullptr, ev_join3 = nullptr;
    int split_min = 1 << 30;
    int prof_batch_images = 0;
    bool no_lds_resize = false;

    int profiling = 0;
    hipEvent_t ev[10] = {nullptr, nullptr, nullptr, nullptr, nullptr, nullptr, nullptr, nullptr, nullptr, nullptr};
    double prof_ms[5] = {0, 0, 0, 0, 0};
    long long prof_batches = 0, prof_images = 0;
    bool prof_pending = false, prof_fast0 = false;

    OrbCtx ctx;
    int last_batch = 0;
    oslam_orb_plan_t plan = {};
    hipStream_t last_stream = nullptr;
};

static void build_resize_tab(int ssize, int dsize, bool is_x, std::vector<int2>& tab) {
    const double inv_scale = (double)dsize / ssize;
    const double scale = 1. / inv_scale;
    for (int d = 0; d < dsize; d++) {
        float f = (float)((d + 0.5) * scale - 0.5);
        int s = (int)std::floor(f);
        f -= s;
        if (is_x) {
            if (s < 0) { f = 0; s = 0; }
            if (s >= ssize - 1) { f = 0; s = ssize - 1; }
        }
        const float c0 = 1.f - f, c1 = f;
        const int a0 = (unsigned short)sat_short(c0 * 2048), a1 = (unsigned short)sat_short(c1 * 2048);
        tab.push_back(make_int2(s, a0 | (a1 << 16)));
    }
}

extern "C" {

const char* oslam_last_error(void) { return g_err; }

int oslam_device_count(void) {
    int n = 0;
    if (hipGetDeviceCount(&n) != hipSuccess) return 0;
    return n;
}

void oslam_orb_destroy(oslam_orb_t* h) {
    if (!h) return;
    for (hipEvent_t e : h->ev)
        if (e) (void)hipEventDestroy(e);
    if (h->ev_fork) (void)hipEventDestroy(h->ev_fork);
    if (h->ev_join) (void)hipEventDestroy(h->ev_join);
    if (h->side_stream) (void)hipStreamDestroy(h->side_stream);
    if (h->fast0_stream) (void)hipStreamDestroy(h->fast0_stream);
    if (h->ev_fork0) (void)hipEventDestroy(h->ev_fork0);
    if (h->ev_join0) (void)hipEventDestroy(h->ev_join0);
    if (h->aux_stream) (void)hipStreamDestroy(h->aux_stream);
    if (h->aux_side_stream) (void)hipStreamDestroy(h->aux_side_stream);
    for (hipEvent_t e : {h->ev_fork2, h->ev_join2, h->ev_fork3, h->ev_join3}) if (e) (void)hipEventDestroy(e);
    delete h;
}

int oslam_orb_create(oslam_orb_t** out, int nfeatures, float scaleFactor_, int nlevels, int iniTh, int minTh,
                     int width, int height, int max_batch, int device) {
    if (!out) { set_error("out is NULL"); return OSLAM_E_INVALID; }
    *out = nullptr;
    if (nfeatures <= 0 || nlevels < 1 || nlevels > OSLAM_MAX_LEVELS || !(scaleFactor_ > 1.0f) || width <= 0 ||
        height <= 0 || max_batch < 1 || iniTh < 1 || minTh < 1 || iniTh > 255 || minTh > 255) {
        set_error("oslam_orb_create: invalid argument");
        return OSLAM_E_INVALID;
    }
    int ndev = oslam_device_count();
    if (ndev <= 0) { set_error("no HIP device visible: the gfx950 extractor has no CPU fallback"); return OSLAM_E_HIP; }
    if (device < 0 || device >= ndev) { set_error("device %d out of range (%d visible)", device, ndev); return OSLAM_E_INVALID; }
    OSLAM_HIP_CHECK(hipSetDevice(device));

    oslam_orb* h = new oslam_orb();
#define ORB_CREATE_CHECK(expr) do { hipError_t e_ = (expr); if (e_ != hipSuccess) { set_error("%s failed: %s (%s:%d)", #expr, hipGetErrorString(e_), __FILE__, __LINE__); oslam_orb_destroy(h); return OSLAM_E_HIP; } } while (0)
    h->device = device; h->nfeatures = nfeatures; h->nlevels = nlevels; h->iniTh = iniTh; h->minTh = minTh;
    h->scaleFactor = scaleFactor_;
    h->width = width; h->height = height; h->max_batch = max_batch;
    const double scaleFactor = h->scaleFactor;

    h->scale.resize(nlevels); h->sigma2.resize(nlevels); h->invScale.resize(nlevels); h->invSigma2.resize(nlevels);
    h->scale[0] = 1.0f; h->sigma2[0] = 1.0f;
    for (int i = 1; i < nlevels; i++) {
        h->scale[i] = (float)(h->scale[i - 1] * scaleFactor);
        h->sigma2[i] = h->scale[i] * h->scale[i];
    }
    for (int i = 0; i < nlevels; i++) {
        h->invScale[i] = 1.0f / h->scale[i];
        h->invSigma2[i] = 1.0f / h->sigma2[i];
    }
    h->quota.resize(nlevels);
    {
        float factor = (float)(1.0f / scaleFactor);
        float nDesired = nfeatures * (1 - factor) / (1 - (float)pow((double)factor, (double)nlevels));
        int sum = 0;
        for (int l = 0; l < nlevels - 1; l++) {
            h->quota[l] = cv_round(nDesired);
            sum += h->quota[l];
            nDesired *= factor;
        }
        h->quota[nlevels - 1] = std::max(nfeatures - sum, 0);
    }

    OrbParams& P = h->P;
    memset(&P, 0, sizeof(P));
    P.nlevels = nlevels; P.iniTh = iniTh; P.minTh = minTh;
    {
        int v, v0, vmax = (int)std::floor(kHalfPatch * sqrt(2.f) / 2 + 1);
        int vmin = (int)std::ceil(kHalfPatch * sqrt(2.f) / 2);
        const double hp2 = kHalfPatch * kHalfPatch;
        for (v = 0; v <= vmax; ++v) P.umax[v] = cv_round(sqrt(hp2 - v * v));
        for (v = kHalfPatch, v0 = 0; v >= vmin; --v) {
            while (P.umax[v0] == P.umax[v0 + 1]) ++v0;
            P.umax[v] = v0;
// ... 169 lines not shown
        (rc = h->d_sel.alloc(B * (size_t)P.sel_per_image * sizeof(uint32_t))) || (rc = h->d_sel_count.alloc(B * (size_t)nlevels * sizeof(int))) ||
        (rc = h->d_out_kp.alloc(B * (size_t)P.out_cap * sizeof(oslam_keypoint_t))) || (rc = h->d_out_desc.alloc(B * (size_t)P.out_cap * 32)) ||
        (rc = h->d_out_count.alloc(B * sizeof(int))) || (rc = h->d_status.alloc(sizeof(int))) || (rc = h->d_dbg.alloc(16 * sizeof(unsigned long long)))) {
        oslam_orb_destroy(h);
        return rc;
    }
    ORB_CREATE_CHECK(hipMemset(h->d_ovf_count.as<int>(), 0, 64));
    ORB_CREATE_CHECK(hipMemset(h->d_dbg.as<unsigned long long>(), 0, 16 * sizeof(unsigned long long)));
    ORB_CREATE_CHECK(hipMemcpy(h->dP.as<OrbParams>(), &P, sizeof(P), hipMemcpyHostToDevice));
    {
        std::vector<FastCellRec> cells((size_t)P.total_cells);
        for (int l = 0; l < nlevels; l++) {
            const LevelGeom& g = P.lv[l];
            const int ncell = g.nCols * g.nRows;
            for (int cell = 0; cell < ncell; cell++) {
                FastCellRec r{};
                const int ci = cell / g.nCols, cj = cell - ci * g.nCols;
                const int maxBX = g.w - kRegionBorder, maxBY = g.h - kRegionBorder;
                const int iniY = kRegionBorder + ci * g.hCell, iniX = kRegionBorder + cj * g.wCell;
                int maxY = iniY + g.hCell + 6, maxX = iniX + g.wCell + 6;
                const bool skip = (iniY >= maxBY - 3) || (iniX >= maxBX - 6);
                if (maxY > maxBY) maxY = maxBY;
                if (maxX > maxBX) maxX = maxBX;
                const int cw = maxX - iniX - 6, ch = maxY - iniY - 6;
                int valid = 1;
                if (g.wCell > kWCell || g.hCell > kWCell) { valid = 0; h->plan.big_cell[l] = 1; }
                else if (skip || cw <= 0 || ch <= 0) { valid = 2; h->plan.skipped_cells[l]++; }
                if (iniX > 0xFFFF || iniY > 0xFFFF || g.img_off > 0xFFFFFFFFll) { set_error("oslam_orb_create: image too large for the FAST cell records"); oslam_orb_destroy(h); return OSLAM_E_INVALID; }
                r.xy = (uint32_t)iniX | ((uint32_t)iniY << 16);
                r.dims = (uint32_t)(valid == 1 ? cw : 0) | ((uint32_t)(valid == 1 ? ch : 0) << 8) | ((uint32_t)l << 16) | ((uint32_t)valid << 24);
                r.cand_ofs = (uint32_t)(g.cand_base + (long long)cell * g.cell_cap);
                r.img_off = (uint32_t)g.img_off;
                r.cell_cap = (uint32_t)g.cell_cap;
                r.pitch = (uint32_t)g.pitch;
                cells[(size_t)g.cell_base + cell] = r;
            }
        }
        if ((rc = h->d_fast_cells.alloc(cells.size() * sizeof(FastCellRec)))) { oslam_orb_destroy(h); return rc; }
        ORB_CREATE_CHECK(hipMemcpy(h->d_fast_cells.as<FastCellRec>(), cells.data(), cells.size() * sizeof(FastCellRec), hipMemcpyHostToDevice));
    }
    if (!rtab.empty()) ORB_CREATE_CHECK(hipMemcpy(h->d_rtab.as<int2>(), rtab.data(), rtab.size() * sizeof(int2), hipMemcpyHostToDevice));
    if (!qbase.empty()) {
        ORB_CREATE_CHECK(hipMemcpy(h->d_qbase.as<int>(), qbase.data(), qbase.size() * sizeof(int), hipMemcpyHostToDevice));
        ORB_CREATE_CHECK(hipMemcpy(h->d_qpx.as<uint4>(), qpx.data(), qpx.size() * sizeof(uint4), hipMemcpyHostToDevice));
    }
    ORB_CREATE_CHECK(hipMemcpy(h->d_root_of_x.bytes(), root_of_x.data(), root_of_x.size(), hipMemcpyHostToDevice));
    ORB_CREATE_CHECK(hipMemcpy(h->d_root_x.as<short>(), root_x.data(), root_x.size() * sizeof(short), hipMemcpyHostToDevice));
    ORB_CREATE_CHECK(hipMemset(h->d_status.as<int>(), 0, sizeof(int)));
    ORB_CREATE_CHECK(hipMemset(h->d_out_count.as<int>(), 0, B * sizeof(int)));
    ORB_CREATE_CHECK(hipFuncSetAttribute((const void*)k_octree, hipFuncAttributeMaxDynamicSharedMemorySize, (int)h->oct_lds));
    ORB_CREATE_CHECK(hipFuncSetAttribute((const void*)k_octree_spill, hipFuncAttributeMaxDynamicSharedMemorySize, (int)h->oct_lds));
    ORB_CREATE_CHECK(hipFuncSetAttribute((const void*)k_octree_hbm, hipFuncAttributeMaxDynamicSharedMemorySize, (int)h->oct_lds));
    {
        ORB_CREATE_CHECK(hipStreamCreateWithFlags(&h->side_stream, hipStreamNonBlocking));
    }
    ORB_CREATE_CHECK(hipEventCreateWithFlags(&h->ev_fork, hipEventDisableTiming));
    if (getenv("OSLAM_ORB_FAST0_STREAM")) {
        ORB_CREATE_CHECK(hipStreamCreateWithFlags(&h->fast0_stream, hipStreamNonBlocking));
        ORB_CREATE_CHECK(hipEventCreateWithFlags(&h->ev_fork0, hipEventDisableTiming));
        ORB_CREATE_CHECK(hipEventCreateWithFlags(&h->ev_join0, hipEventDisableTiming));
    }
    ORB_CREATE_CHECK(hipEventCreateWithFlags(&h->ev_join, hipEventDisableTiming));
    if (getenv("OSLAM_ORB_SPLIT_MIN")) h->split_min = atoi(getenv("OSLAM_ORB_SPLIT_MIN"));
    h->no_lds_resize = getenv("OSLAM_ORB_NO_LDS_RESIZE") != nullptr;
    if (max_batch >= h->split_min) {
        ORB_CREATE_CHECK(hipStreamCreateWithFlags(&h->aux_stream, hipStreamNonBlocking));
        ORB_CREATE_CHECK(hipStreamCreateWithFlags(&h->aux_side_stream, hipStreamNonBlocking));
        for (hipEvent_t* e : {&h->ev_fork2, &h->ev_join2, &h->ev_fork3, &h->ev_join3}) ORB_CREATE_CHECK(hipEventCreateWithFlags(e, hipEventDisableTiming));
    }
#undef ORB_CREATE_CHECK
    *out = h;
    return OSLAM_OK;
}

int oslam_orb_get_scale_tables(const oslam_orb_t* h, float* sf, float* isf, float* s2, float* is2, int* nf) {
    if (!h) { set_error("NULL handle"); return OSLAM_E_INVALID; }
    for (int i = 0; i < h->nlevels; i++) {
        if (sf) sf[i] = h->scale[i];
        if (isf) isf[i] = h->invScale[i];
        if (s2) s2[i] = h->sigma2[i];
        if (is2) is2[i] = h->invSigma2[i];
        if (nf) nf[i] = h->quota[i];
    }
    return OSLAM_OK;
}

int oslam_orb_max_keypoints(const oslam_orb_t* h) { return h ? h->P.out_cap : OSLAM_E_INVALID; }

int oslam_orb_set_blur_rounding(oslam_orb_t* h, int sse2) {
    if (!h) return OSLAM_E_INVALID;
    h->blur_sse2 = sse2 != 0;
    return OSLAM_OK;
}

static int collect_profile(oslam_orb* h) {
    if (!h->prof_pending) return OSLAM_OK;
    OSLAM_HIP_CHECK(hipEventSynchronize(h->ev[5]));
    const int a[5] = {0, 1, 6, 2, 4}, b[5] = {1, 2, 7, 3, 5};
    OSLAM_HIP_CHECK(hipEventSynchronize(h->ev[7]));
    for (int i = 0; i < 5; i++) {
        float ms = 0;
        OSLAM_HIP_CHECK(hipEventElapsedTime(&ms, h->ev[a[i]], h->ev[b[i]]));
        h->prof_ms[i] += ms;
    }
    if (h->prof_fast0) {
        float ms = 0;
        OSLAM_HIP_CHECK(hipEventSynchronize(h->ev[9]));
        OSLAM_HIP_CHECK(hipEventElapsedTime(&ms, h->ev[8], h->ev[9]));
        h->prof_ms[1] += ms;
    }
    h->prof_batches++;
    h->prof_images += h->prof_batch_images;
    h->prof_pending = false;
    return OSLAM_OK;
}

static int launch_batch(oslam_orb* h, const uint8_t* d_gray, int batch, int stride, size_t image_stride, hipStream_t st) {
    const OrbParams& P = h->P;
    OrbCtx c;
    c.P = h->dP.as<OrbParams>();
    c.img0 = d_gray; c.img0_pitch = stride; c.img0_stride = (long long)image_stride;
    c.pyr = h->d_pyr.bytes(); c.pyr_stride = h->pyr_stride;
    c.blur = h->d_blur.bytes(); c.blur_stride = h->blur_stride;
    c.rtab = h->d_rtab.as<int2>(); c.qbase = h->d_qbase.as<int>(); c.qpx = h->d_qpx.as<uint4>(); c.root_of_x = h->d_root_of_x.bytes(); c.root_x = h->d_root_x.as<short>();
    c.cell_count = h->d_cell_count.as<int>(); c.cand = h->d_cand.as<uint32_t>(); c.fast_cells = h->d_fast_cells.as<FastCellRec>(); c.oct_nodes = h->d_oct_nodes.as<int>(); c.oct_nodes_stride = h->oct_nodes_stride; c.ovf_count = h->d_ovf_count.as<int>(); c.ent_g = h->d_ent_g.as<uint32_t>(); c.knode_g = h->d_knode_g.as<uint16_t>(); c.sel = h->d_sel.as<uint32_t>(); c.sel_count = h->d_sel_count.as<int>();
    c.out_kp = h->d_out_kp.as<oslam_keypoint_t>(); c.out_desc = h->d_out_desc.bytes(); c.out_count = h->d_out_count.as<int>(); c.status = h->d_status.as<int>(); c.dbg = h->d_dbg.as<unsigned long long>();
    const bool prof = h->profiling != 0;
    if (prof) {
        int rc = collect_profile(h);
        if (rc) return rc;
    }
    h->ctx = c; h->last_batch = batch; h->last_stream = st;
    oslam_orb_plan_t& plan = h->plan;
    plan.nlevels = P.nlevels; plan.batch = batch; plan.n_halves = 0;
    for (int i = 0; i < 2; i++) {
        plan.half_nb[i] = plan.half_kpw[i] = plan.half_oct_nodes_hbm[i] = plan.half_big_cell_kernel[i] = 0;
        plan.half_src_aligned4[i] = plan.half_src_aligned16[i] = -1;
        for (int l = 0; l < OSLAM_MAX_LEVELS; l++) plan.half_resize[i][l] = OSLAM_ORB_RESIZE_NONE;
    }
    auto issue = [&](const OrbCtx& cs, int nb, hipStream_t sm, hipStream_t sb, hipStream_t f0, hipEvent_t fork, hipEvent_t join, bool pr) -> int {
#define PROF_MARK(i) do { if (pr) OSLAM_HIP_CHECK(hipEventRecord(h->ev[i], sm)); } while (0)
        if (pr) h->prof_fast0 = false;
        const int hi = plan.n_halves++;
        plan.half_nb[hi] = nb;
        PROF_MARK(0);
        const int cells0 = (f0 && P.nlevels > 1) ? P.lv[1].cell_base : 0;
        if (cells0 > 0) {
            OSLAM_HIP_CHECK(hipEventRecord(h->ev_fork0, sm));
            OSLAM_HIP_CHECK(hipStreamWaitEvent(f0, h->ev_fork0, 0));
            if (pr) OSLAM_HIP_CHECK(hipEventRecord(h->ev[8], f0));
            hipLaunchKernelGGL(k_fast_cells_wave, dim3(div_up(cells0, 4 * kFastCellsPerWave), nb), dim3(256), 0, f0, cs, 0, cells0);
            if (pr) { OSLAM_HIP_CHECK(hipEventRecord(h->ev[9], f0)); h->prof_fast0 = true; }
            OSLAM_HIP_CHECK(hipEventRecord(h->ev_join0, f0));
        }
        for (int l = 1; l < P.nlevels; l++) {
            const LevelGeom& g = P.lv[l];
            dim3 grid(div_up(g.w, 256), div_up(g.h, 4), nb);
            dim3 gridw(div_up(g.w, 256), div_up(g.h, 4 * kResizeRows), nb);
            const bool src_aligned = l > 1 || (((stride & 3) == 0) && ((((uintptr_t)cs.img0) & 3) == 0) && ((image_stride & 3) == 0));
            const bool src_aligned16 = l > 1 || (((stride & 15) == 0) && ((((uintptr_t)cs.img0) & 15) == 0) && ((image_stride & 15) == 0));
            if (l == 1) { plan.half_src_aligned4[hi] = src_aligned; plan.half_src_aligned16[hi] = src_aligned16; }
            if (g.qtab_off >= 0 && g.lds_tile_ok && src_aligned16 && !h->no_lds_resize) {
                plan.half_resize[hi][l] = OSLAM_ORB_RESIZE_LDS;
                hipLaunchKernelGGL(k_resize_lds, dim3(div_up(g.w, kRzTW), div_up(g.h, kRzTH), nb), dim3(256), 0, sm, cs, l);
            } else if (g.qtab_off >= 0 && src_aligned) {
                plan.half_resize[hi][l] = OSLAM_ORB_RESIZE_WORDS;
                hipLaunchKernelGGL(k_resize_words, gridw, dim3(256), 0, sm, cs, l);
            } else {
                plan.half_resize[hi][l] = OSLAM_ORB_RESIZE_PLAIN;
                hipLaunchKernelGGL(k_resize, grid, dim3(256), 0, sm, cs, l);
            }
        }
        PROF_MARK(1);
        const bool overlap = sb != sm;
        if (overlap) {
            OSLAM_HIP_CHECK(hipEventRecord(fork, sm));
            OSLAM_HIP_CHECK(hipStreamWaitEvent(sb, fork, 0));
        }
        hipLaunchKernelGGL(k_fast_cells_wave, dim3(div_up(P.total_cells - cells0, 4 * kFastCellsPerWave), nb), dim3(256), 0, sm, cs, cells0, P.total_cells);
        if (cells0 > 0) OSLAM_HIP_CHECK(hipStreamWaitEvent(sm, h->ev_join0, 0));
        if (getenv("OSLAM_ORB_DEBUG_OVF")) { int n = 0; (void)hipStreamSynchronize(sm); (void)hipMemcpy(&n, cs.ovf_count, 4, hipMemcpyDeviceToHost); fprintf(stderr, "fast overflow cells since creation: %d (this batch has %d cells)\n", n, P.total_cells * nb); }
        if (P.any_big_cell) {
            plan.half_big_cell_kernel[hi] = 1;
            hipLaunchKernelGGL(k_fast_cells, dim3(P.total_cells, nb), dim3(256), 0, sm, cs);
        }
        PROF_MARK(2);
        if (pr) OSLAM_HIP_CHECK(hipEventRecord(h->ev[6], sb));
        hipLaunchKernelGGL(k_blur_strip<false>, dim3(P.blur_block_base[P.nlevels], nb), dim3(256), 0, sb, cs, h->blur_sse2);
        hipLaunchKernelGGL(k_blur_strip<true>, dim3(P.blurb_block_base[P.nlevels], nb), dim3(256), 0, sb, cs, h->blur_sse2);
        if (pr) OSLAM_HIP_CHECK(hipEventRecord(h->ev[7], sb));
        if (cs.oct_nodes) {
            plan.half_oct_nodes_hbm[hi] = 1;
            hipLaunchKernelGGL(k_octree_hbm, dim3(P.nlevels, nb), dim3(kOctThreads), h->oct_lds, sm, cs);
        } else {
            hipLaunchKernelGGL(k_octree, dim3(P.nlevels, nb), dim3(kOctThreads), h->oct_lds, sm, cs);
            hipLaunchKernelGGL(k_octree_spill, dim3(P.nlevels, nb), dim3(kOctThreads), h->oct_lds, sm, cs);
        }
        PROF_MARK(3);
        if (overlap) {
            OSLAM_HIP_CHECK(hipEventRecord(join, sb));
            OSLAM_HIP_CHECK(hipStreamWaitEvent(sm, join, 0));
        }
        PROF_MARK(4);
        {
            const int kpw = nb >= 32 ? 16 : (nb >= 8 ? 4 : 1);
            plan.half_kpw[hi] = kpw;
            hipLaunchKernelGGL(k_orient_describe, dim3(div_up(P.out_cap, 4 * kpw), nb), dim3(256), 0, sm, cs, kpw);
        }
        PROF_MARK(5);
#undef PROF_MARK
        return OSLAM_OK;
    };
    auto sub_ctx = [&](int b0) {
        OrbCtx cs = c;
        const long long o = b0;
        cs.img0 += o * c.img0_stride; cs.pyr += o * c.pyr_stride; cs.blur += o * c.blur_stride;
        cs.cell_count += o * P.total_cells; if (cs.oct_nodes) cs.oct_nodes += o * P.nlevels * c.oct_nodes_stride; cs.cand += o * P.cand_per_image; cs.ent_g += o * P.cand_per_image; cs.knode_g += o * P.cand_per_image;
        cs.sel += o * P.sel_per_image; cs.sel_count += o * P.nlevels;
        cs.out_kp += o * P.out_cap; cs.out_desc += o * P.out_cap * 32; cs.out_count += o;
        return cs;
    };
    int rc;
    const bool split = batch >= h->split_min && h->aux_stream != nullptr;
    if (!split) {
        rc = issue(c, batch, st, h->side_stream ? h->side_stream : st, h->fast0_stream, h->ev_fork, h->ev_join, prof);
        if (rc) return rc;
        h->prof_batch_images = batch;
    } else {
        const int nb0 = batch / 2, nb1 = batch - nb0;
        OSLAM_HIP_CHECK(hipEventRecord(h->ev_fork2, st));
        OSLAM_HIP_CHECK(hipStreamWaitEvent(h->aux_stream, h->ev_fork2, 0));
        if ((rc = issue(c, nb0, st, h->side_stream, h->fast0_stream, h->ev_fork, h->ev_join, prof))) return rc;
        if ((rc = issue(sub_ctx(nb0), nb1, h->aux_stream, h->aux_side_stream, nullptr, h->ev_fork3, h->ev_join3, false))) return rc;
        OSLAM_HIP_CHECK(hipEventRecord(h->ev_join2, h->aux_stream));
        OSLAM_HIP_CHECK(hipStreamWaitEvent(st, h->ev_join2, 0));
        h->prof_batch_images = nb0;
    }
    if (prof) h->prof_pending = true;
    OSLAM_HIP_CHECK(hipGetLastError());
    return OSLAM_OK;
}

int oslam_orb_extract_batch_device(oslam_orb_t* h, const uint8_t* d_gray, int batch, int stride, size_t image_stride,
                                   void* stream) {
    if (!h || !d_gray) { set_error("NULL argument"); return OSLAM_E_INVALID; }
    if (batch < 1 || batch > h->max_batch) { set_error("batch %d outside [1,%d]", batch, h->max_batch); return OSLAM_E_INVALID; }
    if (stride < h->width || (batch > 1 && image_stride < (size_t)stride * h->height)) { set_error("bad strides"); return OSLAM_E_INVALID; }
    OSLAM_HIP_CHECK(hipSetDevice(h->device));
    return launch_batch(h, d_gray, batch, stride, image_stride, (hipStream_t)stream);
}

int oslam_orb_results_device(const oslam_orb_t* h, const oslam_keypoint_t** kp, const uint8_t** desc, const int32_t** counts,
                             const int32_t** status) {
    if (!h) { set_error("NULL handle"); return OSLAM_E_INVALID; }
    if (kp) *kp = h->d_out_kp.as<oslam_keypoint_t>();
    if (desc) *desc = h->d_out_desc.bytes();
    if (counts) *counts = h->d_out_count.as<int>();
    if (status) *status = h->d_status.as<int>();
    return OSLAM_OK;
}

static int check_status(oslam_orb* h) {
    int st = 0;
    OSLAM_HIP_CHECK(hipMemcpy(&st, h->d_status.as<int>(), sizeof(int), hipMemcpyDeviceToHost));
    if (st) {
        OSLAM_HIP_CHECK(hipMemset(h->d_status.as<int>(), 0, sizeof(int)));
        set_error("extractor arena overflow, status bits 0x%x (1 cell, 2 candidates per level, 4/8 quad-tree nodes, 16 outputs)", st);
        return OSLAM_E_CAPACITY;
    }
    return OSLAM_OK;
}

int oslam_orb_fetch(oslam_orb_t* h, int b, oslam_keypoint_t* kps, uint8_t* desc, int cap, int* n_out) {
    if (!h || !n_out) { set_error("NULL argument"); return OSLAM_E_INVALID; }
    if (b < 0 || b >= h->last_batch) { set_error("image %d not in the last batch (%d)", b, h->last_batch); return OSLAM_E_INVALID; }
    OSLAM_HIP_CHECK(hipSetDevice(h->device));
    OSLAM_HIP_CHECK(hipStreamSynchronize(h->last_stream));
    int rc = check_status(h);
    if (rc) return rc;
    int n = 0;
    OSLAM_HIP_CHECK(hipMemcpy(&n, h->d_out_count.as<int>() + b, sizeof(int), hipMemcpyDeviceToHost));
    *n_out = n;
    if (n > cap) { set_error("caller capacity %d < %d keypoints", cap, n); return OSLAM_E_CAPACITY; }
    if (n > 0) {
        if (!kps || !desc) { set_error("NULL output"); return OSLAM_E_INVALID; }
// ... 145 lines not shown
```

object_slam_amd/csrc/slam_driver.hip:

```cpp
#include <atomic>
#include <chrono>
#include <map>
#include <memory>

#include "common.h"
#include "slam_map.h"
#include "slam_pool.h"


namespace oslam_drv {

struct Vocab {
    uint64_t top[10][4], sub[10][10][4];
    Vocab() {
        uint64_t s = 0x853c49e6748fea9bULL;
        auto next = [&]() {
            const uint64_t old = s;
            s = old * 6364136223846793005ULL + 1442695040888963407ULL;
            const uint32_t x = (uint32_t)(((old >> 18u) ^ old) >> 27u), r = (uint32_t)(old >> 59u);
            return (x >> r) | (x << ((-r) & 31));
        };
        auto word = [&]() { const uint64_t hi = next(); const uint64_t lo = next(); return (hi << 32) | lo; };
        for (int i = 0; i < 10; i++)
            for (int w = 0; w < 4; w++) top[i][w] = word();
// ... 186 lines not shown
};

}

using namespace oslam_drv;

struct oslam_slam { Ctx c; };

namespace oslam_drv {

static void compute_bow(const Ctx& c, int N, const uint8_t* desc, std::vector<uint32_t>& out) {
    if (!out.empty()) return;
    out.resize(N);
    if (c.realVoc) {
        (void)oslam_voc_transform_host(c.realVoc, desc, N, 4, nullptr, out.data(), nullptr);
        return;
    }
    for (int i = 0; i < N; i++) out[i] = c.voc.node(desc + (size_t)i * 32);
}

BowViews& Seq::bow_views(const Ctx& c, int kf) {
    if ((int)kfBow.size() <= kf) kfBow.resize(kf + 1);
    if (!kfBow[kf]) {
        KeyFrm& k = map.kfs[kf];
        compute_bow(c, k.N, k.desc.data(), k.bowNode);
        kfBow[kf].reset(new BowViews);
        kfBow[kf]->side1(k.bowNode);
        kfBow[kf]->side2(k.bowNode);
    }
    return *kfBow[kf];
}

static bool unproject_frame(const Ctx& c, const Frame& f, int i, float out[3]) {
    const float z = f.depth[i];
    if (!(z > 0)) return false;
    const float u = f.keysUn[i].x, v = f.keysUn[i].y;
    const float x = (u - c.cfg.cx) * z * c.invfx, y = (v - c.cfg.cy) * z * c.invfy;
    for (int r = 0; r < 3; r++) {
        float s = f.pose.Rwc[r * 3] * x;
        s += f.pose.Rwc[r * 3 + 1] * y;
        s += f.pose.Rwc[r * 3 + 2] * z;
        out[r] = (float)((double)s + (double)f.pose.Ow[r]);
    }
    return true;
}

static int new_keyframe(Seq& s, const Frame& f) {
    s.mapVersion++;
    s.map.kfs.emplace_back();
    KeyFrm& k = s.map.kfs.back();
    k.id = (int)s.map.kfs.size() - 1;
    k.frameId = f.id; k.stamp = f.stamp; k.N = f.N;
    if (!s.lazyKeys) k.keys.assign(f.keys.begin(), f.keys.begin() + f.N);
    k.keysUn.assign(f.keysUn.begin(), f.keysUn.begin() + f.N);
    k.oct.resize(f.N);
    for (int i = 0; i < f.N; i++) k.oct[i] = (uint8_t)f.keysUn[i].octave;
    if (!s.lazyDesc) k.desc.assign(f.desc.begin(), f.desc.begin() + (size_t)f.N * 32);
    k.uRight.assign(f.uRight.begin(), f.uRight.begin() + f.N);
    k.depth.assign(f.depth.begin(), f.depth.begin() + f.N);
    k.mp.assign(f.mp.begin(), f.mp.begin() + f.N);
    k.bowNode = f.bowNode;
    k.pose.set_keyframe(f.pose.Tcw);
    k.Tcp = eye4();
    s.counter.resize(s.map.kfs.size() + 8, 0);
    s.st[1]++;
    s.pendingKF.push_back(k.id);
    s.map.jr_new_kf(k.id);
    return k.id;
}

struct MpUpdate {
    struct Item { int seq, p; };
    std::vector<Item> items;
    std::vector<int> start;
    std::vector<uint8_t> odesc, outdesc;
    std::vector<int32_t> okey;
    std::vector<float> oOw, pos, owref, lsf, out5;
    std::vector<int> best;
    void clear() { items.clear(); }
    void add(int seq, int p) { items.push_back({seq, p}); }
    std::vector<int> dstart;
    std::vector<int32_t> ikey;
    struct Prof {
        std::atomic<long long> ns[4], calls{0}, pts{0}, obs{0};
        Prof() { for (auto& x : ns) x = 0; }
        ~Prof() {
            if (calls.load()) fprintf(stderr, "[mp_update prof] %lld calls, %lld points, %lld observations: count %.1f ms, pack %.1f ms, operator %.1f ms, scatter %.1f ms\n", calls.load(), pts.load(),
                                      obs.load(), ns[0] * 1e-6, ns[1] * 1e-6, ns[2] * 1e-6, ns[3] * 1e-6);
        }
    };
    static Prof* prof() { static Prof* p = getenv("OSLAM_MPU_PROF") ? new Prof : nullptr; static struct D { ~D() { delete prof(); } } d; return p; }
    bool pending = false, pDesc = false, pNormal = false;
    oslam_job_mp_update_t pjob;
    int run(Ctx& c, bool do_desc, bool do_normal) {
        const int rc = submit(c, do_desc, do_normal, false);
        return rc ? rc : finish(c);
    }
    int submit(Ctx& c, bool do_desc, bool do_normal, bool defer) {
        if (pending) { const int rc0 = finish(c); if (rc0) return rc0; }
        const int P = (int)items.size();
        if (P == 0) return OSLAM_OK;
        Prof* pf = prof();
        auto t0_ = std::chrono::steady_clock::now();
        auto lap_ = [&](int k) { if (pf) { auto t1_ = std::chrono::steady_clock::now(); pf->ns[k] += std::chrono::duration_cast<std::chrono::nanoseconds>(t1_ - t0_).count(); t0_ = t1_; } };
        start.assign(P + 1, 0); dstart.assign(P + 1, 0);
        const int chunk = 256, nchunks = (P + chunk - 1) / chunk;
        c.pool->parallel_for(nchunks, [&](int ch) {
            const int i0 = ch * chunk, i1 = std::min(P, i0 + chunk);
            for (int i = i0; i < i1; i++) {
                if (i + kPF < i1) prefetch_mp(&c.seq[items[i + kPF].seq]->map.mps[items[i + kPF].p]);
                if (i + kPF / 2 < i1) __builtin_prefetch(c.seq[items[i + kPF / 2].seq]->map.mps[items[i + kPF / 2].p].obs.data());
                const Map& m = c.seq[items[i].seq]->map;
// ... 1582 lines not shown
            const int kf = new_keyframe(s, f);
            s.refKF = kf; f.refKF = kf;
            create_stereo_points(c, s, f, kf, false);
            s.newKFs.push_back(kf);
            s.lastKFFrameId = f.id;
        }
        for (int k = 0; k < f.N; k++)
            if (f.mp[k] >= 0 && f.outlier[k]) f.mp[k] = -1;
        if (!f.objs.empty()) update_current_objects(s);
    } else {
        s.st[8]++;
        if (m.nKFsInMap <= 5) s.resetRequested = true;
    }
    if (f.refKF < 0) f.refKF = s.refKF;
}

static int run_pose_jobs(Ctx& c, const std::vector<int>& who) {
    if (who.empty()) return OSLAM_OK;
    std::vector<oslam_job_pose_t> pj(who.size());
    for (size_t q = 0; q < who.size(); q++) pj[q] = c.seq[who[q]]->jPose;
    const int rc = c.ops.pose_opt(c.ops.ctx, (int)pj.size(), pj.data());
    for (size_t q = 0; q < who.size(); q++) c.seq[who[q]]->jPose = pj[q];
    return rc;
}

struct TrackInput {
    enum Kind { RGBD, RAW16, STEREO } kind;
    const uint8_t* const* gray;
    const uint8_t* const* right = nullptr;
    const float* const* depth = nullptr;
    const uint16_t* const* depth16 = nullptr; float depth_factor = 1.f;
    int gray_stride, depth_pitch = 0, on_device;
    const double* stamps;
    const oslam_slam_objects_t* objs; int mask_stride;
    float* Tcw_out; int32_t* state_out;
    TrackInput(Kind k, const uint8_t* const* g, int gs, int dev, const double* ts, const oslam_slam_objects_t* o, int ms, float* T, int32_t* st)
        : kind(k), gray(g), gray_stride(gs), on_device(dev), stamps(ts), objs(o), mask_stride(ms), Tcw_out(T), state_out(st) {}
};

struct TrackPass : PassClock {
    const TrackInput& in;
    const int S;
    std::vector<int> tracking;
    std::vector<int> mapping;
    TrackPass(Ctx& c_, const TrackInput& in_) : PassClock(c_), in(in_), S(c_.S) {}
    Seq& seq(int i) const { return *c.seq[i]; }
    void charge(int stage) { charge_host(4, stage); }
};

static int tk_frames(TrackPass& T) {
    Ctx& c = T.c; const TrackInput& in = T.in;
    std::vector<int32_t> slots(T.S);
    std::vector<oslam_slam_frame_t*> outs(T.S);
    for (int i = 0; i < T.S; i++) { slots[i] = i; outs[i] = &T.seq(i).cur->view; }
    int rc;
    if (in.kind == TrackInput::STEREO) rc = c.ops.frames_stereo(c.ops.ctx, T.S, slots.data(), in.gray, in.right, in.gray_stride, in.on_device, outs.data());
    else if (in.kind == TrackInput::RAW16) rc = c.ops.frames_rgbd_raw16(c.ops.ctx, T.S, slots.data(), in.gray, in.gray_stride, in.depth16, in.depth_pitch, in.depth_factor, in.on_device, outs.data());
    else rc = c.ops.frames_rgbd(c.ops.ctx, T.S, slots.data(), in.gray, in.gray_stride, in.depth, in.depth_pitch, in.on_device, outs.data());
    if (rc) return rc;
    T.charge_op(0);
    return OSLAM_OK;
}

static void tk_begin_frames(TrackPass& T) {
    Ctx& c = T.c;
    T.pool.parallel_for(T.S, [&](int i) {
        Seq& s = T.seq(i);
        if (s.resetRequested) s.reset();
        const int fid = s.nextFrameId++;
        s.cur->begin(fid, T.in.stamps ? T.in.stamps[i] : (double)fid);
        s.seenList.clear(); s.updList.clear();
        s.st[0]++;
        s.path = 0; s.ok = false; s.hasSL = s.hasLoc = false;
        Frame& f = *s.cur;
        if (s.state == ST_NOT_INITIALIZED && f.N > 500) {
            f.pose.set_frame(eye4());
            const int kf = new_keyframe(s, f);
            create_stereo_points(c, s, f, kf, true);
            s.newKFs.push_back(kf);
            s.lastKFFrameId = f.id;
            s.localKFs.assign(1, kf);
            s.localMPs.clear();
            for (int p : s.map.kfs[kf].mp) if (p >= 0) s.localMPs.push_back(p);
            s.locVersion = -1;
            s.refKF = kf; f.refKF = kf;
            s.state = ST_OK;
            s.path = -1;
        }
    });
}

static int tk_object_keypoints(TrackPass& T) {
    Ctx& c = T.c; const TrackInput& in = T.in;
    std::vector<oslam_job_object_kps_t> oj;
    std::vector<int> ojw;
    int rc;
    c.mask_stride = in.mask_stride; c.masks_on_device = in.on_device;
    for (int i = 0; i < T.S; i++) {
        Seq& s = T.seq(i);
        s.det = (in.objs && in.objs[i].n > 0) ? &in.objs[i] : nullptr;
        if (!s.det) continue;
        if (s.det->n > OSLAM_SLAM_MAX_OBJECTS || !s.det->masks) { oslam::set_error("track: sequence %d has %d detections (max %d) or no masks", i, s.det->n, OSLAM_SLAM_MAX_OBJECTS); return OSLAM_E_INVALID; }
        if (!c.ops.object_kps || !c.ops.pose_opt2) { oslam::set_error("track: this operator table has no semantic operators"); return OSLAM_E_INVALID; }
        s.jInMask.assign(s.cur->N + 1, 0);
        oslam_job_object_kps_t j;
        j.slot = i; j.cur = &s.cur->view; j.n_masks = s.det->n; j.masks = s.det->masks; j.mask_stride = in.mask_stride; j.on_device = in.on_device; j.in_mask = s.jInMask.data();
        oj.push_back(j); ojw.push_back(i);
// ... 559 lines not shown
```

object_slam_amd/csrc/slam_map.h:

```cpp
#pragma once
#include <algorithm>
#include <cmath>
#include <cstdint>
#include <cstring>
#include <map>
#include <set>
#include <utility>
#include <vector>

#include "../../include/oslam_slam.h"
#include "seq_arena.h"

namespace oslam_drv {

typedef oslam_keypoint_t KP;

struct M4 { float m[16]; };
inline M4 eye4() { M4 r; memset(r.m, 0, sizeof(r.m)); r.m[0] = r.m[5] = r.m[10] = r.m[15] = 1.f; return r; }
inline M4 mul4(const M4& a, const M4& b) {
    M4 r;
    for (int i = 0; i < 4; i++)
        for (int j = 0; j < 4; j++) {
            float s = a.m[i * 4] * b.m[j];
            s += a.m[i * 4 + 1] * b.m[4 + j];
            s += a.m[i * 4 + 2] * b.m[8 + j];
            s += a.m[i * 4 + 3] * b.m[12 + j];
            r.m[i * 4 + j] = s;
        }
    return r;
}
inline float norm3(const float* v) {
    double s = 0;
    for (int k = 0; k < 3; k++) s += (double)v[k] * (double)v[k];
    return (float)std::sqrt(s);
}

struct PoseM {
    M4 Tcw, Twc;
    float Rwc[9], Ow[3];
    bool valid = false;
    void set_frame(const M4& T) {
        Tcw = T; valid = true;
        for (int r = 0; r < 3; r++)
            for (int c = 0; c < 3; c++) Rwc[r * 3 + c] = T.m[c * 4 + r];
        for (int r = 0; r < 3; r++) {
            double s = 0;
            for (int k = 0; k < 3; k++) s += (double)T.m[k * 4 + r] * (double)T.m[k * 4 + 3];
            Ow[r] = (float)(-1.0 * s);
        }
        fill_twc();
    }
    void set_keyframe(const M4& T) {
        Tcw = T; valid = true;
        for (int r = 0; r < 3; r++)
            for (int c = 0; c < 3; c++) Rwc[r * 3 + c] = T.m[c * 4 + r];
        for (int r = 0; r < 3; r++) {
            float s = Rwc[r * 3] * T.m[3];
            s += Rwc[r * 3 + 1] * T.m[7];
            s += Rwc[r * 3 + 2] * T.m[11];
            Ow[r] = (float)((double)s * -1.0);
        }
        fill_twc();
    }
    void fill_twc() {
        Twc = eye4();
        for (int r = 0; r < 3; r++) {
            for (int c = 0; c < 3; c++) Twc.m[r * 4 + c] = Rwc[r * 3 + c];
            Twc.m[r * 4 + 3] = Ow[r];
        }
    }
};

struct Frame {
    int id = -1;
    double stamp = 0;
    int N = 0;
    std::vector<KP> keys, keysUn;
    std::vector<uint8_t> desc;
    std::vector<float> uRight, depth;
    std::vector<int> mp;
    std::vector<uint8_t> outlier;
    std::vector<uint32_t> bowNode;
    PoseM pose;
    int refKF = -1;
    oslam_slam_frame_t view;
    struct Obj2D { int det = -1, track = -1, obj3d = -1; std::vector<int> kps; };
    std::vector<Obj2D> objs;
    std::vector<int> objOfKp;
    void alloc(int cap) {
        keys.resize(cap); keysUn.resize(cap); desc.resize((size_t)cap * 32); uRight.resize(cap); depth.resize(cap);
        mp.assign(cap, -1); outlier.assign(cap, 0);
        view.N = 0; view.keys = keys.data(); view.keysUn = keysUn.data(); view.desc = desc.data(); view.uRight = uRight.data(); view.depth = depth.data();
    }
    void begin(int id_, double stamp_) {
        id = id_; stamp = stamp_; N = view.N;
        std::fill(mp.begin(), mp.end(), -1);
        std::fill(outlier.begin(), outlier.end(), 0);
        bowNode.clear(); pose.valid = false; refKF = -1;
        objs.clear(); objOfKp.assign(N, -1);
    }
};

struct ObsKp { float x, y, ur; int octave; };
typedef std::pair<int, int> Obs;

struct ObsListRaw { char* blk; uint32_t n, cap; };
struct ObsView {
    char* blk; uint32_t n, cap;
    size_t size() const { return n; }
    bool empty() const { return n == 0; }
    const Obs* data() const { return (const Obs*)blk; }
    const Obs* begin() const { return data(); }
    const Obs* end() const { return data() + n; }
    const Obs& operator[](size_t i) const { return data()[i]; }
    const Obs& front() const { return data()[0]; }
};
struct OkpView {
    char* blk; uint32_t n, cap;
    size_t size() const { return n; }
    bool empty() const { return n == 0; }
    const ObsKp* data() const { return (const ObsKp*)(blk + (size_t)cap * sizeof(Obs)); }
    const ObsKp* begin() const { return data(); }
    const ObsKp* end() const { return data() + n; }
    const ObsKp& operator[](size_t i) const { return data()[i]; }
    const ObsKp& front() const { return data()[0]; }
};
constexpr size_t obs_block_bytes(uint32_t cap) { return (size_t)cap * (sizeof(Obs) + sizeof(ObsKp)); }

struct alignas(64) MapPt {
    union { ObsListRaw lst = {nullptr, 0, 0}; ObsView obs; OkpView okp; };
    float pos[3];
    float normal[3] = {0, 0, 0};
    float minD = 0, maxD = 0;
    int refKF = -1;
    int trackRefForFrame = 0;
    int fuseListIdx = 0, fuseListStamp = 0;
    uint8_t desc[32];
    int firstKF = 0, firstFrame = 0;
    int obsVer = 0, updVer = -1, updStep = -1;
    int obs_index(int kf) const {
        for (size_t i = 0; i < obs.size(); i++) if (obs[i].first == kf) return obs[i].second;
        return -1;
    }
};
static_assert(sizeof(MapPt) == 128 && offsetof(MapPt, desc) == 64, "MapPt: two cache lines, the per-frame fields in the first");

typedef ChunkVec<MapPt, 6> PtTable;
static_assert((sizeof(MapPt) << 6) <= SeqArena::kMaxSmall, "a block of the point table is an arena block");
template <class T> using PtArray = ChunkVec<T, 8>;

constexpr int kPF = 12;
inline void prefetch_mp(const MapPt* p) { __builtin_prefetch(p); __builtin_prefetch((const char*)p + 64); }
template <class Ids>
inline void prefetch_ahead(const PtTable& mps, const Ids& ids, size_t i, size_t n) {
    if (i + kPF < n) { const int q = ids[i + kPF]; if (q >= 0) prefetch_mp(&mps[q]); }
}
template <class Ids>
inline void prefetch_obs_ahead(const PtTable& mps, const Ids& ids, size_t i, size_t n) {
    prefetch_ahead(mps, ids, i, n);
    if (i + kPF / 2 < n) { const int q = ids[i + kPF / 2]; if (q >= 0) __builtin_prefetch(mps[q].obs.data()); }
}
template <class Ids>
inline void prefetch_okp_ahead(const PtTable& mps, const Ids& ids, size_t i, size_t n) {
    prefetch_obs_ahead(mps, ids, i, n);
}

struct KeyFrm {
    int id = 0, frameId = 0;
    double stamp = 0;
    int N = 0;
    std::vector<KP> keys, keysUn;
    std::vector<uint8_t> desc, oct;
    std::vector<float> uRight, depth;
    std::vector<int> mp;
    std::vector<uint32_t> bowNode;
    PoseM pose;
    M4 Tcp;
    std::map<int, int> connW;
    std::vector<int> ordered, orderedW;
    int parent = -1;
    std::set<int> children;
    bool firstConnection = true, bad = false;
    int trackRefForFrame = 0, fuseTargetForKF = 0;
};

struct RelPose { M4 Tcr; int refKF; double stamp; bool lost; };

struct Map {
    SeqArena arena;
    PtTable mps;
    std::vector<KeyFrm> kfs;
    Map() = default;
    Map(Map&&) = default;
    Map& operator=(Map&&) = default;
    int nKFsInMap = 0, nMPsInMap = 0;
    int64_t nCulledKF = 0, nCulledMP = 0;

    PtArray<int> pNObs, pVisible, pFound, pLastSeen, pReplaced;
    PtArray<uint8_t> pBad;
    PtArray<uint64_t> pLvl;
    bool lvlOverflow = false;
    void lvl_add(int p, int oct) {
        if ((unsigned)oct >= 8u || ((pLvl[p] >> (8 * oct)) & 0xFFull) == 0xFFull) { lvlOverflow = true; return; }
        pLvl[p] += 1ull << (8 * oct);
    }
    void lvl_sub(int p, int oct) {
        if ((unsigned)oct >= 8u || ((pLvl[p] >> (8 * oct)) & 0xFFull) == 0ull) { lvlOverflow = true; return; }
        pLvl[p] -= 1ull << (8 * oct);
    }
    int lvl_count_le(int p, int oct) const {
        const uint64_t h = oct >= 7 ? pLvl[p] : (pLvl[p] & ((1ull << (8 * (oct + 1))) - 1ull));
        uint64_t s2 = (h & 0x00FF00FF00FF00FFull) + ((h >> 8) & 0x00FF00FF00FF00FFull);
        s2 = (s2 & 0x0000FFFF0000FFFFull) + ((s2 >> 16) & 0x0000FFFF0000FFFFull);
        return (int)((s2 & 0xFFFFFFFFull) + (s2 >> 32));
    }
    enum { JR_KFMP = 1, JR_KFMP_BULK = 2, JR_OKF_SET = 3, JR_OKF_CLR = 4, JR_PT = 5, JR_RESET = 6 };
    bool jrOn = false, jrReset = false;
    std::vector<std::pair<int, int>> jrCells;
    std::vector<uint32_t> jrOkf;
    std::vector<int> jrPts, jrNewKFs;
    std::vector<uint8_t> jrPtMark;
    bool jr_pending() const { return jrReset || !jrCells.empty() || !jrOkf.empty() || !jrPts.empty() || !jrNewKFs.empty(); }
    void jr_kfmp(int kf, int idx, int) { if (jrOn) jrCells.push_back(std::make_pair(kf, idx)); }
    void jr_okf(int op, int kf, int idx, int p) { if (jrOn) { jrOkf.push_back((uint32_t)kf); jrOkf.push_back((uint32_t)idx | (op == JR_OKF_SET ? 0x80000000u : 0u)); jrOkf.push_back((uint32_t)p); } }
    void jr_pt(int p) {
        if (!jrOn) return;
        if (jrPtMark.size() <= (size_t)p) jrPtMark.resize((size_t)p + 1 + jrPtMark.size() / 2, 0);
        if (!jrPtMark[p]) { jrPtMark[p] = 1; jrPts.push_back(p); }
    }
    void jr_new_kf(int kf) { if (jrOn) jrNewKFs.push_back(kf); }
    struct JrScratch { std::vector<oslam_map_new_kf_t> kfs; std::vector<uint32_t> good, pts; std::vector<int32_t> cells; std::vector<uint32_t> events; };
    void journal_changes(int slot, float thDepth, JrScratch& sc, oslam_map_changes_t& ch) {
        ch.slot = slot; ch.reset = jrReset ? 1 : 0; jrReset = false;
        sc.kfs.clear(); sc.good.clear();
        size_t gw = 0;
        for (int kf : jrNewKFs) gw += (kfs[kf].mp.size() + 31) / 32;
        sc.good.resize(gw);
// ... 266 lines not shown
```

object_slam_amd/csrc/slam_ops_hip.hip:

```cpp
#include <algorithm>
#include <cmath>
#include <atomic>
#include <chrono>
#include <condition_variable>
#include <deque>
#include <memory>
#include <mutex>
#include <thread>
#include <unordered_map>
#include <functional>
#include <vector>

#include "../../include/oslam_slam.h"
#include "common.h"
#include "kf_record_layout.h"
#include "slam_pool.h"
#include "stage_layout.h"

namespace {

using oslam::StageLayout;
using oslam::copy_elems;

class SlotTable {
// ... 19 lines not shown
    int sync(hipStream_t strm) {
        if (!dirty_) return OSLAM_OK;
        if (!d_tab_.ptr()) OSLAM_CHECK(d_tab_.alloc(sizeof(uint8_t*) * blocks_.size()));
        OSLAM_HIP_CHECK(hipMemcpyAsync(d_tab_.ptr(), blocks_.data(), sizeof(uint8_t*) * blocks_.size(), hipMemcpyHostToDevice, strm));
        OSLAM_HIP_CHECK(hipStreamSynchronize(strm));
        dirty_ = false;
        return OSLAM_OK;
    }
private:
    const size_t rec_bytes_;
    const bool zero_fill_;
    oslam::DeviceBlocks blocks_; std::vector<size_t> cap_;
    oslam::DeviceBuffer d_tab_;
    bool dirty_ = true;
};

struct LbaService;
struct LbaJob {
    int n = 0; const oslam_lba_problem_t* probs = nullptr; float K5[5] = {0, 0, 0, 0, 0};
    bool timing = false, done = false; int rc = 0; char err[256] = "";
    double ms = 0, launches = 0, flop = 0;
};

struct HipOps {
    LbaService* svc = nullptr;
    LbaJob job; bool job_active = false;
    oslam_slam_config_t cfg;
    int S = 0, cap = 0;
    oslam_orb_t* orb = nullptr;
    oslam_orb_t* orbR = nullptr;
    oslam_stereo_t* stereo = nullptr;
    oslam::DeviceBuffer d_grayR;
    const float* cur_uRight = nullptr;
    oslam_matcher_t* m_last = nullptr;
    oslam_matcher_t* m_map = nullptr;
    oslam_poseopt_t* po = nullptr;
    oslam_lba_t* ba1 = nullptr;
    oslam_mappoint_t* mp = nullptr;
    oslam_frame_t* fr = nullptr;
    oslam_bow_t* bow = nullptr;
    float scale[OSLAM_MAX_LEVELS], invScale[OSLAM_MAX_LEVELS], sigma2[OSLAM_MAX_LEVELS], invSigma2[OSLAM_MAX_LEVELS];
    float bounds[4], K4[4], K5[5];
    oslam_camera_t cam;
    float logScale;
    int max_local = 0;
    oslam::DeviceBuffer d_gray, d_depth; size_t gray_pitch = 0;
    oslam::DeviceBuffer d_keysUn_prev;
    oslam::DeviceBuffer d_keysUn, d_uRight, d_mvDepth, d_status;
    const oslam_keypoint_t* d_kp = nullptr; const uint8_t* d_desc = nullptr; const int32_t* d_cnt = nullptr;
    std::vector<oslam_proj_query_t> q;
    std::vector<int32_t> qm, qd;
    oslam::StagePair up;
    oslam::PinnedBuffer dn;
    oslam::StagePair upB;
    oslam::PinnedBuffer dnB;
    hipEvent_t tevB0 = nullptr, tevB1 = nullptr;
    bool lazy_rows = false;
    oslam::PinnedBuffer kfk; std::vector<int32_t> kfk_slots;
    oslam::Field<oslam_keypoint_t> kfk_keys{}; oslam::Field<uint8_t> kfk_desc{};
    static constexpr int kFuseCurStride = 16384, kFuseCurPairs = 2048;
    oslam::DeviceBuffer fc; uint32_t fc_stamp = 0;
    struct MpuPending {
        bool on = false; oslam_job_mp_update_t* j = nullptr; oslam::Field<int32_t> rBest{}; oslam::Field<uint8_t> rOut{}; oslam::Field<float> rOut5{}; double dtotal = 0; std::function<int()> launch;
    } mpu_pend;
    int mpu_launch_pending() { if (mpu_pend.on && mpu_pend.launch) { std::function<int()> f; f.swap(mpu_pend.launch); return f(); } return OSLAM_OK; }
    void swap_staging() { std::swap(up, upB); std::swap(dn, dnB); std::swap(tev0, tevB0); std::swap(tev1, tevB1); }
    oslam::DeviceBuffer d_lq, d_inview;
    oslam::DeviceBuffer d_objbits;
    oslam::DeviceBuffer d_loc; size_t loc_st = 0;
    std::vector<long long> loc_id;
    float* loc_Pw() const { return d_loc.as<float>(); }
    float* loc_Pn() const { return (float*)(d_loc.bytes() + 12 * loc_st * S); }
    float* loc_Max() const { return (float*)(d_loc.bytes() + 24 * loc_st * S); }
    float* loc_Min() const { return (float*)(d_loc.bytes() + 28 * loc_st * S); }
    uint8_t* loc_Obs() const { return d_loc.bytes() + 32 * loc_st * S; }
    uint8_t* loc_Desc() const { return d_loc.bytes() + 33 * loc_st * S; }
    int ensure_loc() {
        const size_t want = oslam::align_up((size_t)std::max(max_local, 1), 64);
        if (d_loc.ptr() && loc_st == want) return OSLAM_OK;
        OSLAM_HIP_CHECK(hipStreamSynchronize(strm));
        loc_st = want;
        OSLAM_CHECK(d_loc.alloc(65 * loc_st * S));
        loc_id.assign(S, 0);
        return OSLAM_OK;
    }
    static constexpr int kRecChunk = 256;
    oslam::DeviceBlocks rec_chunks;
    std::vector<std::vector<int>> rec_of_kf;
    long long n_released = 0;
    std::vector<int32_t> mpu_rec;
    std::vector<int> free_recs;
    int n_rec = 0;
    oslam::DeviceBuffer d_rec_desc; int rec_desc_n = 0;
    std::vector<uint8_t*> h_rec_desc;
    oslam::KfRecordLayout rec_lay;
    size_t rec_bytes() const { return rec_lay.bytes; }
    std::vector<uint32_t> okf_seq;
    size_t mir_used = 0;
    oslam::PinnedBuffer cull;
    struct CullPending { int32_t* out; int n; };
    std::vector<CullPending> cull_pending;
    oslam::StagePair mir;
    int ensure_mir(size_t bytes) {
        if (bytes > mir.cap()) OSLAM_HIP_CHECK(hipStreamSynchronize(strm));
        return mir.grow(bytes, 1 << 20);
    }
// ... 28 lines not shown
    long long step_epoch = 0, bits_epoch = -1;
    int ensure_maskbits(size_t words) {
        if (words * 8 > d_maskbits.cap()) OSLAM_HIP_CHECK(hipStreamSynchronize(strm));
        return d_maskbits.reserve(words * 8, (words + words / 4) * 8);
    }
    int ensure_masks(size_t bytes) {
        if (bytes > d_maskstage.cap()) OSLAM_HIP_CHECK(hipDeviceSynchronize());
        return d_maskstage.grow(bytes, 4096);
    }
    oslam_drv::Pool* pool = nullptr;
    hipStream_t strm = nullptr;
    int timing = 0;
    hipEvent_t tev0 = nullptr, tev1 = nullptr;
    double kt[OSLAM_SLAM_KT_GROUPS * 3] = {0};
    void t_begin() { if (timing) (void)hipEventRecord(tev0, strm); }
    void t_end() { if (timing) (void)hipEventRecord(tev1, strm); }
    void t_collect(int g, double launches, double work) {
        if (!timing) return;
        float ms = 0.f;
        if (hipEventElapsedTime(&ms, tev0, tev1) == hipSuccess) { kt[3 * g] += ms; kt[3 * g + 1] += launches; kt[3 * g + 2] += work; }
    }
    int ensure_up(size_t bytes) {
        if (bytes > up.cap()) OSLAM_HIP_CHECK(hipDeviceSynchronize());
        return up.grow(bytes, 4096);
    }
    int ensure_dn(size_t bytes) {
        if (bytes > dn.cap()) OSLAM_HIP_CHECK(hipDeviceSynchronize());
        return dn.grow(bytes, 4096);
    }
    int ensure_lq(size_t entries) {
        if (entries <= d_inview.cap()) return OSLAM_OK;
        OSLAM_HIP_CHECK(hipDeviceSynchronize());
        d_lq.release(); d_inview.release();
        const size_t ncap = entries + entries / 2 + 1024;
        OSLAM_CHECK(d_lq.alloc(ncap * sizeof(oslam_proj_query_t)));
        return d_inview.alloc(ncap);
    }
};

int h_max_keypoints(void* p) { return ((HipOps*)p)->cap; }
int h_scale_tables(void* p, float* a, float* b, float* c, float* d) {
    HipOps* o = (HipOps*)p;
    const int n = o->cfg.nLevels;
    memcpy(a, o->scale, 4 * n); memcpy(b, o->invScale, 4 * n); memcpy(c, o->sigma2, 4 * n); memcpy(d, o->invSigma2, 4 * n);
    return OSLAM_OK;
}
int h_image_bounds(void* p, float* b) { memcpy(b, ((HipOps*)p)->bounds, 16); return OSLAM_OK; }

static int download_frames(HipOps* o, int n, const oslam_keypoint_t* d_kp, const uint8_t* d_desc, const int32_t* d_cnt, const int32_t* d_st, const float* d_uR,
                           const float* d_dp, oslam_slam_frame_t* const* out) {
    o->d_kp = d_kp; o->d_desc = d_desc; o->d_cnt = d_cnt; o->cur_uRight = d_uR;
    const size_t cap = o->cap;
    StageLayout R;
    const auto rCnt = R.add<int32_t>(n), rSt = R.add<int32_t>(2); const auto rKeys = R.add<oslam_keypoint_t>(cap * n), rKeysUn = R.add<oslam_keypoint_t>(cap * n);
    const auto rDesc = R.add<uint8_t>(32 * cap * n); const auto rUr = R.add<float>(cap * n), rDp = R.add<float>(cap * n);
    OSLAM_CHECK(o->ensure_dn(R.total()));
    uint8_t* D = o->dn.bytes();
    int32_t* st = at(rSt, D);
    OSLAM_HIP_CHECK(hipMemcpyAsync(at(rCnt, D), d_cnt, rCnt.bytes, hipMemcpyDeviceToHost, o->strm));
    OSLAM_HIP_CHECK(hipMemcpyAsync(st, d_st, sizeof(*st), hipMemcpyDeviceToHost, o->strm));
    OSLAM_HIP_CHECK(hipMemcpyAsync(st + 1, o->d_status.as<int32_t>(), sizeof(*st), hipMemcpyDeviceToHost, o->strm));
    if (!o->lazy_rows) OSLAM_HIP_CHECK(hipMemcpyAsync(at(rKeys, D), d_kp, rKeys.bytes, hipMemcpyDeviceToHost, o->strm));
    OSLAM_HIP_CHECK(hipMemcpyAsync(at(rKeysUn, D), o->d_keysUn.as<oslam_keypoint_t>(), rKeysUn.bytes, hipMemcpyDeviceToHost, o->strm));
    if (!o->lazy_rows) OSLAM_HIP_CHECK(hipMemcpyAsync(at(rDesc, D), d_desc, rDesc.bytes, hipMemcpyDeviceToHost, o->strm));
    OSLAM_HIP_CHECK(hipMemcpyAsync(at(rUr, D), d_uR, rUr.bytes, hipMemcpyDeviceToHost, o->strm));
    OSLAM_HIP_CHECK(hipMemcpyAsync(at(rDp, D), d_dp, rDp.bytes, hipMemcpyDeviceToHost, o->strm));
    OSLAM_HIP_CHECK(oslam::stream_wait(o->strm));
    if (st[0]) { oslam::set_error("extractor arena overflow"); return OSLAM_E_CAPACITY; }
    if (st[1]) { oslam::set_error("keypoint outside the depth image / right extractor arena overflow"); return OSLAM_E_INVALID; }
    const int32_t* cnt = at(rCnt, D);
    o->pool->parallel_for(n, [&](int i) {
        oslam_slam_frame_t* f = out[i];
        const size_t N = cnt[i];
        f->N = (int)N;
        if (!o->lazy_rows) copy_elems(f->keys, row(rKeys, D, cap, i), N);
        copy_elems(f->keysUn, row(rKeysUn, D, cap, i), N);
        if (!o->lazy_rows) copy_elems(f->desc, row(rDesc, D, 32 * cap, i), 32 * N);
        copy_elems(f->uRight, row(rUr, D, cap, i), N);
        copy_elems(f->depth, row(rDp, D, cap, i), N);
    });
    return OSLAM_OK;
}

static int frames_impl(HipOps* o, int n, const uint8_t* const* gray, int gray_stride, const float* const* depth, const uint16_t* const* depth16, int depth_pitch,
                       float depth_factor, int on_device, oslam_slam_frame_t* const* out) {
    o->step_epoch++;
    std::swap(o->d_keysUn, o->d_keysUn_prev);
    OSLAM_HIP_CHECK(hipSetDevice(o->cfg.device));
    if (n > o->S) { oslam::set_error("frames_rgbd: n > n_sequences"); return OSLAM_E_INVALID; }
    const int W = o->cfg.width, H = o->cfg.height;
    const size_t gimg = o->gray_pitch * H, dimg = (size_t)W * H;
    const void* const* depth_table = nullptr;
    const void* const* dsrc = depth16 ? (const void* const*)depth16 : (const void* const*)depth;
    if (on_device) {
        StageLayout L;
        const auto fGray = L.add<const void*>(n), fDepth = L.add<const void*>(n);
        OSLAM_CHECK(o->ensure_up(L.total()));
        put(fGray, o->up.h.bytes(), (const void* const*)gray); put(fDepth, o->up.h.bytes(), dsrc);
        OSLAM_HIP_CHECK(hipMemcpyAsync(o->up.d.bytes(), o->up.h.bytes(), fDepth.end(), hipMemcpyHostToDevice, o->strm));
        OSLAM_CHECK(oslam_frame_gather_images_device(at(fGray, o->up.d.bytes()), n, gray_stride, W, H, o->d_gray.bytes(), gimg, (int)o->gray_pitch, o->strm));
        depth_table = at(fDepth, o->up.d.bytes());
    } else {
        StageLayout L;
        const auto fGray = L.add<uint8_t>(gimg * n); const auto fDepth = L.add<float>(dimg * n);
        OSLAM_CHECK(o->ensure_up(L.total()));
        uint8_t* U = o->up.h.bytes();
        o->pool->parallel_for(n, [&](int i) {
            for (int r = 0; r < H; r++) {
                copy_elems(row(fGray, U, gimg, i) + o->gray_pitch * r, gray[i] + (size_t)gray_stride * r, (size_t)W);
                float* drow = row(fDepth, U, dimg, i) + (size_t)W * r;
                if (depth16) { const uint16_t* srow = depth16[i] + (size_t)depth_pitch * r; for (int x = 0; x < W; x++) drow[x] = (float)srow[x] * depth_factor; }
                else copy_elems(drow, depth[i] + (size_t)depth_pitch * r, (size_t)W);
            }
        });
        OSLAM_HIP_CHECK(hipMemcpyAsync(o->d_gray.bytes(), at(fGray, U), fGray.bytes, hipMemcpyHostToDevice, o->strm));
        OSLAM_HIP_CHECK(hipMemcpyAsync(o->d_depth.as<float>(), at(fDepth, U), fDepth.bytes, hipMemcpyHostToDevice, o->strm));
    }
    o->t_begin();
    OSLAM_CHECK(oslam_orb_extract_batch_device(o->orb, o->d_gray.bytes(), n, (int)o->gray_pitch, gimg, o->strm));
    const oslam_keypoint_t* d_kp; const uint8_t* d_desc; const int32_t* d_cnt; const int32_t* d_st;
    OSLAM_CHECK(oslam_orb_results_device(o->orb, &d_kp, &d_desc, &d_cnt, &d_st));
    OSLAM_CHECK(oslam_frame_undistort_batch_device(d_kp, o->d_keysUn.as<oslam_keypoint_t>(), d_cnt, 0, o->cap, n, o->K4, o->cfg.dist, o->cfg.ndist, o->strm));
    if (depth_table && depth16) OSLAM_CHECK(oslam_frame_stereo_from_rgbd_batch_ptrs_u16_device(d_kp, o->d_keysUn.as<oslam_keypoint_t>(), d_cnt, 0, o->cap, n, (const uint16_t* const*)depth_table, H, W, depth_pitch,
                                                                                              depth_factor, o->cfg.bf, o->d_uRight.as<float>(), o->d_mvDepth.as<float>(), o->d_status.as<int32_t>(), o->strm));
    else if (depth_table) OSLAM_CHECK(oslam_frame_stereo_from_rgbd_batch_ptrs_device(d_kp, o->d_keysUn.as<oslam_keypoint_t>(), d_cnt, 0, o->cap, n, (const float* const*)depth_table, H, W, depth_pitch, o->cfg.bf,
                                                                                   o->d_uRight.as<float>(), o->d_mvDepth.as<float>(), o->d_status.as<int32_t>(), o->strm));
    else OSLAM_CHECK(oslam_frame_stereo_from_rgbd_batch_device(d_kp, o->d_keysUn.as<oslam_keypoint_t>(), d_cnt, 0, o->cap, n, o->d_depth.as<float>(), H, W, W, dimg, o->cfg.bf, o->d_uRight.as<float>(),
                                                             o->d_mvDepth.as<float>(), o->d_status.as<int32_t>(), o->strm));
    o->t_end();
    OSLAM_CHECK(download_frames(o, n, d_kp, d_desc, d_cnt, d_st, o->d_uRight.as<float>(), o->d_mvDepth.as<float>(), out));
    if (o->timing) { double bytes = 0; for (int i = 0; i < n; i++) bytes += (double)oslam_orb_algorithmic_bytes(o->orb, out[i]->N); o->t_collect(0, 14, bytes); }
    return OSLAM_OK;
// ... 781 lines not shown
    for (int i = 0; i < q.nKF; i++) nfree += q.fixed[i] == 0;
    const double n6 = 6.0 * nfree;
    return (double)(st[1] + st[3]) * (700.0 * q.nE + schur + n6 * n6 * n6 / 3.0 + 2.0 * n6 * n6 + 45.0 * q.nP);
}

struct LbaService {
    typedef LbaJob Job;
    int device = 0;
    struct Worker { oslam_lba_t* ba = nullptr; std::thread th; };
    std::vector<std::unique_ptr<Worker>> workers;
    int max_batch = 0;
    std::mutex launch_mu;
    std::mutex mu;
    std::condition_variable cv_work, cv_done;
    std::deque<Job*> queue;
    bool stop = false;
    int users = 0;
    long long calls = 0, windows = 0, max_windows = 0;

    static std::mutex& reg_mu() { static std::mutex m; return m; }
    static LbaService*& slot(int device) { static LbaService* s[64] = {nullptr}; return s[device & 63]; }

    static LbaService* acquire(int device) {
        std::lock_guard<std::mutex> lk(reg_mu());
        LbaService*& sv = slot(device);
        if (!sv) {
            LbaService* n = new LbaService;
            n->device = device;
            if (n->start()) { delete n; return nullptr; }
            sv = n;
        }
        sv->users++;
        return sv;
    }
    static void release(LbaService* sv) {
        if (!sv) return;
        std::lock_guard<std::mutex> lk(reg_mu());
        if (--sv->users > 0) return;
        { std::lock_guard<std::mutex> l2(sv->mu); sv->stop = true; }
        sv->cv_work.notify_all();
        for (auto& wk : sv->workers) if (wk->th.joinable()) wk->th.join();
        if (getenv("OSLAM_LBA_SERVICE_STATS")) fprintf(stderr, "[lba service] %lld calls, %lld windows (%.1f per call, max %lld)\n", sv->calls, sv->windows, sv->calls ? (double)sv->windows / sv->calls : 0.0, sv->max_windows);
        (void)hipSetDevice(sv->device);
        for (auto& wk : sv->workers) oslam_lba_destroy(wk->ba);
        slot(sv->device) = nullptr;
        delete sv;
    }
    int start() {
        OSLAM_HIP_CHECK(hipSetDevice(device));
        max_batch = getenv("OSLAM_LBA_SERVICE_MAX_BATCH") ? atoi(getenv("OSLAM_LBA_SERVICE_MAX_BATCH")) : 4096;
        const int nthreads = std::max(1, getenv("OSLAM_LBA_SERVICE_THREADS") ? atoi(getenv("OSLAM_LBA_SERVICE_THREADS")) : 2);
        for (int t = 0; t < nthreads; t++) {
            std::unique_ptr<Worker> wk(new Worker);
            int rc = oslam_lba_create(&wk->ba, max_batch, 1 << 16, 4096, 32768, device);
            if (!rc) rc = oslam_lba_set_mode(wk->ba, 1);
            if (rc) { oslam_lba_destroy(wk->ba); return rc; }
            oslam::lba_use_gate(wk->ba, &launch_mu);
            workers.push_back(std::move(wk));
        }
        for (auto& wk : workers) { Worker* w = wk.get(); w->th = std::thread([this, w] { run(*w); }); }
        return OSLAM_OK;
    }
    void submit(Job* j) {
        { std::lock_guard<std::mutex> lk(mu); j->done = false; queue.push_back(j); }
        cv_work.notify_one();
    }
    void wait(Job* j) {
        std::unique_lock<std::mutex> lk(mu);
        cv_done.wait(lk, [&] { return j->done; });
    }
    void run(Worker& wk) {
        (void)hipSetDevice(device);
        oslam::stream_wait_thread_mode(0);
        oslam_lba_t* ba = wk.ba;
        std::vector<Job*> take;
        std::vector<oslam_lba_problem_t> probs;
        std::vector<int32_t> st;
        for (;;) {
            take.clear();
            {
                std::unique_lock<std::mutex> lk(mu);
                cv_work.wait(lk, [&] { return stop || !queue.empty(); });
                if (queue.empty()) return;
                Job* first = queue.front();
                int total = 0;
                for (auto it = queue.begin(); it != queue.end();) {
                    Job* j = *it;
                    if (memcmp(j->K5, first->K5, sizeof(first->K5)) == 0 && (take.empty() || total + j->n <= max_batch)) { take.push_back(j); total += j->n; it = queue.erase(it); }
                    else ++it;
                }
            }
            probs.clear();
            bool timing = false;
            for (Job* j : take) { probs.insert(probs.end(), j->probs, j->probs + j->n); timing = timing || j->timing; }
            const int n = (int)probs.size();
            st.assign((size_t)4 * n, 0);
            std::vector<int32_t*> caller_stats(n);
            for (int i = 0; i < n; i++) { caller_stats[i] = probs[i].stats; probs[i].stats = &st[4 * (size_t)i]; }
            int rc = OSLAM_OK;
            double ms = 0; long long launches = 0;
            if (n > 0) {
                rc = oslam_lba_kernel_time(ba, timing ? 1 : 0, nullptr, nullptr);
                for (int at = 0; !rc && at < n; at += max_batch) rc = oslam_lba_optimize_batch(ba, std::min(max_batch, n - at), probs.data() + at, take[0]->K5);
                if (!rc && timing) rc = oslam_lba_kernel_time(ba, 0, &ms, &launches);
            }
            std::vector<int> job_rc(take.size(), 0);
            if (!rc) {
// ... 789 lines not shown
    });
    o->t_begin();
    OSLAM_CHECK(oslam_fuse_search_device(n, (int)st, at(fRef, U), at(fSl, U), at(fM, U), at(fIds, U), at(fEx, U), o->mp_tab.device_table(), at(fT, U), at(fOw, U), o->K5, o->bounds, jobs[0].th,
                                         o->logScale, o->scale, o->invSigma2, o->cfg.nLevels, at(rQm, D), o->strm));
    o->t_end();
    OSLAM_HIP_CHECK(oslam::stream_wait(o->strm));
    o->t_collect(4, 1, 0);
    o->pool->parallel_for(n, [&](int i) { copy_elems(jobs[i].q_match, row(rQm, D, st, i), (size_t)jobs[i].M); });
    return OSLAM_OK;
}

int h_bow(void* p, int n, oslam_job_bow_t* jobs) {
    HipOps* o = (HipOps*)p;
    OSLAM_HIP_CHECK(hipSetDevice(o->cfg.device));
    return oslam_match_bow_batch(o->bow, n, jobs, o->scale, o->sigma2, o->cfg.nLevels);
}

int h_triangulate(void* p, int n, oslam_job_triangulate_t* jobs) {
    HipOps* o = (HipOps*)p;
    OSLAM_HIP_CHECK(hipSetDevice(o->cfg.device));
    std::vector<oslam_tri_kf_t> k1(n), k2(n);
    std::vector<int32_t> ps(n + 1, 0), i1, i2;
    for (int i = 0; i < n; i++) {
        k1[i] = jobs[i].kf1; k2[i] = jobs[i].kf2;
        ps[i + 1] = ps[i] + jobs[i].M;
        i1.insert(i1.end(), jobs[i].idx1, jobs[i].idx1 + jobs[i].M);
        i2.insert(i2.end(), jobs[i].idx2, jobs[i].idx2 + jobs[i].M);
    }
    const int M = ps[n];
    if (M == 0) return OSLAM_OK;
    std::vector<uint8_t> ok(M);
    std::vector<float> x3(3 * (size_t)M);
    OSLAM_CHECK(oslam_mp_triangulate_pairs(o->mp, n, k1.data(), k2.data(), ps.data(), i1.data(), i2.data(), o->scale, o->sigma2, o->cfg.nLevels,
                                         1.5f * o->cfg.scaleFactor, ok.data(), x3.data()));
    for (int i = 0; i < n; i++) {
        memcpy(jobs[i].ok, &ok[ps[i]], (size_t)jobs[i].M);
        memcpy(jobs[i].x3D, &x3[3 * (size_t)ps[i]], 12 * (size_t)jobs[i].M);
    }
    return OSLAM_OK;
}

void h_destroy(void* p) {
    HipOps* o = (HipOps*)p;
    (void)hipSetDevice(o->cfg.device);
    if (o->job_active) (void)h_lba_wait(o);
    lba_service_release(o->svc);
    oslam_orb_destroy(o->orb); oslam_orb_destroy(o->orbR); oslam_stereo_destroy(o->stereo); oslam_matcher_destroy(o->m_last); oslam_matcher_destroy(o->m_map); oslam_poseopt_destroy(o->po);
    oslam_lba_destroy(o->ba1); oslam_mappoint_destroy(o->mp); oslam_frame_destroy(o->fr); oslam_bow_destroy(o->bow);
    delete o->pool;
    if (o->tev0) (void)hipEventDestroy(o->tev0);
    if (o->tevB0) (void)hipEventDestroy(o->tevB0);
    if (o->tevB1) (void)hipEventDestroy(o->tevB1);
    if (o->tev1) (void)hipEventDestroy(o->tev1);
    if (o->strm) (void)hipStreamDestroy(o->strm);
    delete o;
}

}

extern "C" int oslam_slam_make_hip_ops(const oslam_slam_config_t* cfg, oslam_slam_ops_t* ops) {
    if (oslam_device_count() <= 0 || hipSetDevice(cfg->device) != hipSuccess) {
        oslam::set_error("oslam_slam_create: no HIP device (the tracking driver has no CPU fallback)");
        return OSLAM_E_HIP;
    }
    memset(ops, 0, sizeof(*ops));
    HipOps* o = new HipOps;
    o->cfg = *cfg; o->S = cfg->n_sequences;
    o->mp_tab.resize(o->S); o->pt_aux.resize(o->S);
    o->pool = new oslam_drv::Pool(cfg->host_threads > 1 ? cfg->host_threads : 1,  false);
    if (hipStreamCreateWithFlags(&o->strm, hipStreamNonBlocking) != hipSuccess) o->strm = nullptr;
    const int dev = cfg->device;
    int rc = oslam_orb_create(&o->orb, cfg->nFeatures, cfg->scaleFactor, cfg->nLevels, cfg->iniThFAST, cfg->minThFAST, cfg->width, cfg->height, o->S, dev);
    if (!rc) {
        o->cap = oslam_orb_max_keypoints(o->orb);
        o->rec_lay = oslam::KfRecordLayout(o->cap);
        o->max_local = getenv("OSLAM_SLAM_MAX_LOCAL") ? atoi(getenv("OSLAM_SLAM_MAX_LOCAL")) : 8192;
        rc = oslam_matcher_create(&o->m_last, o->S, o->cap, o->cap, dev);
    }
    if (!rc) rc = oslam_matcher_create(&o->m_map, o->S, o->cap, o->max_local, dev);
    if (!rc && cfg->sensor == 1) rc = oslam_orb_create(&o->orbR, cfg->nFeatures, cfg->scaleFactor, cfg->nLevels, cfg->iniThFAST, cfg->minThFAST, cfg->width, cfg->height, o->S, dev);
    if (!rc && cfg->sensor == 1) rc = oslam_stereo_create(&o->stereo, o->S, o->cap, dev);
    if (!rc) rc = oslam_poseopt_create(&o->po, o->S, o->cap, dev);
    if (!rc) rc = oslam_lba_create(&o->ba1, 1, 1 << 16, 4096, 32768, dev);
    if (!rc) rc = oslam_mappoint_create(&o->mp, dev);
    if (!rc) rc = oslam_frame_create(&o->fr, dev);
    if (!rc) rc = oslam_bow_create(&o->bow, o->cap, dev);
    if (!rc && o->strm) {
        oslam::lba_use_stream(o->ba1, o->strm);
        oslam::bow_use_stream(o->bow, o->strm);
        oslam::mappoint_use_stream(o->mp, o->strm);
    }
    if (!rc) rc = oslam_orb_get_scale_tables(o->orb, o->scale, o->invScale, o->sigma2, o->invSigma2, nullptr);
    o->K4[0] = cfg->fx; o->K4[1] = cfg->fy; o->K4[2] = cfg->cx; o->K4[3] = cfg->cy;
    memcpy(o->K5, o->K4, 16); o->K5[4] = cfg->bf;
    o->cam.fx = cfg->fx; o->cam.fy = cfg->fy; o->cam.cx = cfg->cx; o->cam.cy = cfg->cy; o->cam.bf = cfg->bf; o->cam.b = cfg->bf / cfg->fx;
    o->logScale = std::log(cfg->scaleFactor);
    if (!rc) rc = oslam_frame_image_bounds(o->fr, cfg->width, cfg->height, o->K4, cfg->dist, cfg->ndist, o->bounds);
    if (!rc) {
        o->gray_pitch = oslam::align_up((size_t)cfg->width, 64);
        const size_t S = o->S;
        rc = o->d_gray.alloc(o->gray_pitch * cfg->height * S);
        if (!rc && cfg->sensor == 1) rc = o->d_grayR.alloc(o->gray_pitch * cfg->height * S);
        if (!rc) rc = o->d_depth.alloc((size_t)cfg->width * cfg->height * 4 * S);
        if (!rc) rc = o->d_keysUn.alloc(sizeof(oslam_keypoint_t) * o->cap * S);
        if (!rc) rc = o->d_keysUn_prev.alloc(sizeof(oslam_keypoint_t) * o->cap * S);
        if (!rc) rc = o->d_uRight.alloc(4 * (size_t)o->cap * S);
        if (!rc) rc = o->d_mvDepth.alloc(4 * (size_t)o->cap * S);
        if (!rc) rc = o->d_objbits.alloc((size_t)o->cap * S);
        if (!rc) rc = o->d_status.alloc(64);
        if (!rc && hipMemset(o->d_status.ptr(), 0, 64) != hipSuccess) { oslam::set_error("slam ops: hipMemset failed"); rc = OSLAM_E_HIP; }
    }
    if (!rc && hipDeviceSynchronize() != hipSuccess) { oslam::set_error("slam ops: device synchronisation failed"); rc = OSLAM_E_HIP; }
    if (rc) { h_destroy(o); return rc; }
    ops->ctx = o;
    ops->max_keypoints = h_max_keypoints; ops->scale_tables = h_scale_tables; ops->image_bounds = h_image_bounds; ops->frames_rgbd = h_frames; ops->frames_rgbd_raw16 = h_frames_raw16;
    ops->search_last = h_search_last; ops->search_local = h_search_local; ops->pose_opt = h_pose_opt; ops->mp_update = h_mp_update; ops->lba = h_lba;
    ops->fuse = h_fuse; ops->bow = h_bow; ops->triangulate = h_triangulate; ops->destroy = h_destroy; ops->frames_stereo = cfg->sensor == 1 ? h_frames_stereo : nullptr;
    ops->kernel_times = h_kernel_times; ops->object_kps = h_object_kps; ops->pose_opt2 = h_pose_opt2;
    o->svc = LbaService::acquire(dev);
    if (!o->svc) { h_destroy(o); return OSLAM_E_HIP; }
    if (cfg->local_mapping & OSLAM_SLAM_LM_DEFERRED) {
        ops->lba_submit = h_lba_submit;
        ops->lba_wait = h_lba_wait;
    }
    ops->mp_update_windows = h_mp_update_windows;

    const bool resident_points = getenv("OSLAM_SLAM_NO_RESIDENT_POINTS") == nullptr;
    const bool resident_kf = getenv("OSLAM_SLAM_NO_RESIDENT_KF") == nullptr;
    o->mp_tab_on = resident_points;
    if (resident_points) {
        ops->point_record = h_point_record;
        ops->resident_points = h_resident_points;
    }
    if (resident_kf) {
        o->lazy_rows = true;
        ops->register_keyframes = h_register_keyframes;
        ops->release_keyframes = h_release_keyframes;
        ops->keyframe_raw_keys = h_keyframe_raw_keys;
        ops->keyframe_descriptors = h_keyframe_descriptors;
        ops->frame_descriptors = h_frame_descriptors;
        ops->bow_keyed = h_bow_keyed;
// ... 18 lines not shown
```

object_slam_amd/extractor.py:

```python
import ctypes as C

import numpy as np

from . import _lib
from ._lib import KP_DTYPE, check, ptr


MAX_LEVELS = 16
RESIZE_NONE, RESIZE_PLAIN, RESIZE_WORDS, RESIZE_LDS = 0, 1, 2, 3


class OrbPlan(C.Structure):
    _fields_ = [("nlevels", C.c_int32), ("batch", C.c_int32), ("n_halves", C.c_int32), ("half_nb", C.c_int32 * 2), ("half_kpw", C.c_int32 * 2),
                ("half_src_aligned4", C.c_int32 * 2), ("half_src_aligned16", C.c_int32 * 2), ("half_oct_nodes_hbm", C.c_int32 * 2),
                ("half_big_cell_kernel", C.c_int32 * 2), ("half_resize", (C.c_int32 * MAX_LEVELS) * 2), ("big_cell", C.c_int32 * MAX_LEVELS),
                ("skipped_cells", C.c_int32 * MAX_LEVELS)]


class ORBextractor(_lib.Handle):
    def __init__(self, nfeatures, scaleFactor, nlevels, iniThFAST, minThFAST, width, height,
                 max_batch=1, device=0):
        super().__init__(_lib.lib(), "oslam_orb", nfeatures, scaleFactor, nlevels, iniThFAST, minThFAST, width, height, max_batch, device)
        self.nfeatures, self.nlevels = nfeatures, nlevels
        self.width, self.height, self.max_batch = width, height, max_batch
        self.cap = self.L.oslam_orb_max_keypoints(self.h)

    def _tables(self):
        n = self.nlevels
        sf, isf, s2, is2 = (np.zeros(n, np.float32) for _ in range(4))
        nf = np.zeros(n, np.int32)
        check(self.L.oslam_orb_get_scale_tables(self.h, ptr(sf), ptr(isf), ptr(s2), ptr(is2), ptr(nf)))
        return sf, isf, s2, is2, nf

    def GetLevels(self):
        return self.nlevels

    def GetScaleFactors(self):
        return self._tables()[0]

    def GetInverseScaleFactors(self):
        return self._tables()[1]

    def GetScaleSigmaSquares(self):
        return self._tables()[2]

    def GetInverseScaleSigmaSquares(self):
        return self._tables()[3]

    def GetFeaturesPerLevel(self):
        return self._tables()[4]

    def set_blur_rounding(self, sse2):
        check(self.L.oslam_orb_set_blur_rounding(self.h, int(sse2)))

    def __call__(self, image, mask=None):
        if image is None or image.size == 0:
            return np.zeros(0, KP_DTYPE), np.zeros((0, 32), np.uint8)
        image = np.ascontiguousarray(image, dtype=np.uint8)
        h, w = image.shape
        kps = np.zeros(self.cap, KP_DTYPE)
        desc = np.zeros((self.cap, 32), np.uint8)
        n = C.c_int(0)
        check(self.L.oslam_orb_extract(self.h, ptr(image), w, h, image.strides[0], ptr(kps), ptr(desc), self.cap,
                                       C.byref(n)))
        return kps[:n.value].copy(), desc[:n.value].copy()

    def extract_batch_device(self, d_ptr, batch, stride, image_stride, stream=None):
        check(self.L.oslam_orb_extract_batch_device(self.h, C.c_void_p(d_ptr), batch, stride, image_stride,
                                                    C.c_void_p(stream or 0)))

    def results_device(self):
        kp, desc, cnt, st = C.c_void_p(), C.c_void_p(), C.c_void_p(), C.c_void_p()
        check(self.L.oslam_orb_results_device(self.h, C.byref(kp), C.byref(desc), C.byref(cnt), C.byref(st)))
        return kp.value, desc.value, cnt.value, st.value

# ... 60 lines not shown
```

Baseline: 51170.

## Add stream registry, create LBA on caller stream, zero-copy frame rows

Adds a stream registry that tracks HIP streams by role, plus an option to create the ORB extractor without a side stream. The tracking LBA solver is now created directly on the SLAM handle's stream instead of making and then discarding its own stream. Frame rows (undistorted keypoints, right-image u coordinates, depth) are copied into double-buffered pinned buffers that callers can point into in place rather than copying. This is meant to cut hardware-queue pressure and host copy work, at the cost of more complex buffer lifetimes.

```diff
diff --git a/include/oslam_hip.h b/include/oslam_hip.h
--- a/include/oslam_hip.h
+++ b/include/oslam_hip.h
@@ -32,7 +32,12 @@
 
 int oslam_orb_create(oslam_orb_t** out, int nfeatures, float scaleFactor, int nlevels, int iniThFAST,
                      int minThFAST, int width, int height, int max_batch, int device);
+#define OSLAM_ORB_NO_SIDE_STREAM 1
+int oslam_orb_create_flags(oslam_orb_t** out, int nfeatures, float scaleFactor, int nlevels, int iniThFAST,
+                           int minThFAST, int width, int height, int max_batch, int device, int flags);
 void oslam_orb_destroy(oslam_orb_t* h);
+
+int oslam_hip_stream_stats(int device, int64_t out[8]);
 
 int oslam_orb_get_scale_tables(const oslam_orb_t* h, float* scaleFactors, float* invScaleFactors,
                                float* levelSigma2, float* invLevelSigma2, int* nFeaturesPerLevel);
@@ -258,6 +263,7 @@
 typedef struct oslam_lba oslam_lba_t;
 int oslam_lba_create(oslam_lba_t** out, int max_batch, int max_keyframes , int max_points,
                      int max_edges, int device);
+int oslam_lba_create_on_stream(oslam_lba_t** out, int max_batch, int max_keyframes, int max_points, int max_edges, int device, void* stream);
 void oslam_lba_destroy(oslam_lba_t* h);
 volatile int32_t* oslam_lba_stop_flag(oslam_lba_t* h);
 int oslam_lba_set_mode(oslam_lba_t* h, int wide);
diff --git a/include/oslam_slam.h b/include/oslam_slam.h
--- a/include/oslam_slam.h
+++ b/include/oslam_slam.h
@@ -29,6 +29,7 @@
 #define OSLAM_SLAM_OK 2
 #define OSLAM_SLAM_LOST 3
 
+#define OSLAM_SLAM_FRAME_ROWS_IN_PLACE (-1)
 typedef struct oslam_slam_frame {
     int32_t N;
     oslam_keypoint_t* keys;
diff --git a/object_slam_amd/_lib.py b/object_slam_amd/_lib.py
--- a/object_slam_amd/_lib.py
+++ b/object_slam_amd/_lib.py
@@ -38,10 +38,22 @@
         L.oslam_orb_algorithmic_bytes.argtypes = [C.c_void_p, C.c_int]
         L.oslam_orb_create.argtypes = [C.POINTER(C.c_void_p), C.c_int, C.c_float, C.c_int, C.c_int, C.c_int,
                                        C.c_int, C.c_int, C.c_int, C.c_int]
+        L.oslam_orb_create_flags.argtypes = L.oslam_orb_create.argtypes + [C.c_int]
         L.oslam_orb_destroy.argtypes = [C.c_void_p]
+        L.oslam_hip_stream_stats.argtypes = [C.c_int, C.POINTER(C.c_int64)]
         L.oslam_orb_extract_batch_device.argtypes = [C.c_void_p, C.c_void_p, C.c_int, C.c_int, C.c_size_t, C.c_void_p]
         _lib = L
     return _lib
+
+
+ORB_NO_SIDE_STREAM = 1
+STREAM_STATS_FIELDS = ("budget", "handle", "extractor_side", "solver", "service", "other", "side_declined", "live")
+
+
+def stream_stats(device=0):
+    out = (C.c_int64 * 8)()
+    check(lib().oslam_hip_stream_stats(int(device), out))
+    return dict(zip(STREAM_STATS_FIELDS, (int(v) for v in out)))
 
 
 def check(rc):
diff --git a/object_slam_amd/csrc/bow_matcher.hip b/object_slam_amd/csrc/bow_matcher.hip
--- a/object_slam_amd/csrc/bow_matcher.hip
+++ b/object_slam_amd/csrc/bow_matcher.hip
@@ -222,7 +222,7 @@
     if (!h) return;
     if (h->ev0) (void)hipEventDestroy(h->ev0);
     if (h->ev1) (void)hipEventDestroy(h->ev1);
-    if (h->strm && h->owns_strm) (void)hipStreamDestroy(h->strm);
+    if (h->strm && h->owns_strm) oslam::stream_destroy(h->strm);
     delete h;
 }
 
@@ -230,7 +230,7 @@
 namespace oslam {
 void bow_use_stream(oslam_bow* h, hipStream_t s) {
     if (!h || !s) return;
-    if (h->strm && h->owns_strm) (void)hipStreamDestroy(h->strm);
+    if (h->strm && h->owns_strm) oslam::stream_destroy(h->strm);
     h->strm = s; h->owns_strm = false;
 }
 }
@@ -406,7 +406,7 @@
         }
         c.out = (int*)(D + o.out); c.nmatches = (int*)(D + o.nm); c.q_best = (int*)(D + o.qbest);
     });
-    if (!h->strm) OSLAM_HIP_CHECK(hipStreamCreateWithFlags(&h->strm, hipStreamNonBlocking));
+    if (!h->strm) OSLAM_HIP_CHECK(oslam::stream_create(&h->strm, oslam::kStreamSolver));
     OSLAM_HIP_CHECK(hipMemcpyAsync(D, H, in_bytes, hipMemcpyHostToDevice, h->strm));
     if (h->timing) (void)hipEventRecord(h->ev0, h->strm);
     hipLaunchKernelGGL(k_search_bow_batch, dim3(n), dim3(kBowThreads), h->lds, h->strm, (const BowCtx*)D, h->max_kps);
diff --git a/object_slam_amd/csrc/common.h b/object_slam_amd/csrc/common.h
--- a/object_slam_amd/csrc/common.h
+++ b/object_slam_amd/csrc/common.h
@@ -10,6 +10,7 @@
 
 #include "../../include/oslam_hip.h"
 #include "device_buffer.h"
+#include "stream_registry.h"
 
 namespace oslam {
 
@@ -28,6 +29,7 @@
 hipError_t stream_wait(hipStream_t s);
 void stream_wait_thread_mode(int spin_us);
 void lba_use_stream(struct ::oslam_lba* h, hipStream_t s);
+int lba_create_service(struct ::oslam_lba** out, int max_batch, int max_keyframes, int max_points, int max_edges, int device);
 void lba_use_gate(struct ::oslam_lba* h, std::mutex* gate);
 void bow_use_stream(struct ::oslam_bow* h, hipStream_t s);
 void mappoint_use_stream(struct ::oslam_mappoint* h, hipStream_t s);
diff --git a/object_slam_amd/csrc/covisibility.hip b/object_slam_amd/csrc/covisibility.hip
--- a/object_slam_amd/csrc/covisibility.hip
+++ b/object_slam_amd/csrc/covisibility.hip
@@ -39,7 +39,7 @@
     hipStream_t stream = nullptr;
     oslam::StagePair io;
     std::mutex mu;
-    ~oslam_covis() { if (stream) (void)hipStreamDestroy(stream); }
+    ~oslam_covis() { oslam::stream_destroy(stream); }
 };
 
 namespace {
@@ -543,7 +543,7 @@
     }
     h->st = CovisState{h->obs.as<int2>(), h->pmeta.as<uint32_t>(), h->weights.as<int32_t>(), h->kmeta.as<uint32_t>(), h->parent.as<int32_t>(), n_graphs, max_keyframes,
                        max_points, obs_cap, W};
-    hipError_t e = hipStreamCreateWithFlags(&h->stream, hipStreamNonBlocking);
+    hipError_t e = oslam::stream_create(&h->stream, oslam::kStreamSolver);
     if (e == hipSuccess) {
         rc = covis_clear(h, 0, G);
         if (rc == OSLAM_OK) e = hipStreamSynchronize(h->stream);
diff --git a/object_slam_amd/csrc/keyframe_db.hip b/object_slam_amd/csrc/keyframe_db.hip
--- a/object_slam_amd/csrc/keyframe_db.hip
+++ b/object_slam_amd/csrc/keyframe_db.hip
@@ -475,7 +475,7 @@
         delete h;
         return rc;
     }
-    hipError_t e = hipStreamCreateWithFlags(&h->stream, hipStreamNonBlocking);
+    hipError_t e = oslam::stream_create(&h->stream, oslam::kStreamSolver);
     if (e == hipSuccess) e = hipMemsetAsync(h->nwords.ptr(), 0xff, (size_t)S * 4, h->stream);
     if (e == hipSuccess) e = hipMemsetAsync(h->serial.ptr(), 0, (size_t)S * 4, h->stream);
     if (e == hipSuccess) e = hipMemsetAsync(h->reloc.ptr(), 0, (size_t)S * 4, h->stream);
diff --git a/object_slam_amd/csrc/kfdb_state.h b/object_slam_amd/csrc/kfdb_state.h
--- a/object_slam_amd/csrc/kfdb_state.h
+++ b/object_slam_amd/csrc/kfdb_state.h
@@ -30,7 +30,7 @@
     hipStream_t stream = nullptr;
     oslam::StagePair io;
     std::mutex mu;
-    ~oslam_kfdb() { if (stream) (void)hipStreamDestroy(stream); }
+    ~oslam_kfdb() { oslam::stream_destroy(stream); }
 };
 
 namespace oslam {
diff --git a/object_slam_amd/csrc/lba.hip b/object_slam_amd/csrc/lba.hip
--- a/object_slam_amd/csrc/lba.hip
+++ b/object_slam_amd/csrc/lba.hip
@@ -1993,7 +1993,7 @@
     (void)hipSetDevice(h->device);
     if (h->ev0) (void)hipEventDestroy(h->ev0);
     if (h->ev1) (void)hipEventDestroy(h->ev1);
-    if (h->strm && h->owns_strm) (void)hipStreamDestroy(h->strm);
+    if (h->strm && h->owns_strm) oslam::stream_destroy(h->strm);
     delete h;
 }
 
@@ -2002,13 +2002,28 @@
 void lba_use_gate(oslam_lba* h, std::mutex* gate) { if (h) h->launch_gate = gate; }
 void lba_use_stream(oslam_lba* h, hipStream_t s) {
     if (!h || !s) return;
-    if (h->strm && h->owns_strm) { (void)hipStreamSynchronize(h->strm); (void)hipStreamDestroy(h->strm); }
+    if (h->strm && h->owns_strm) { (void)hipStreamSynchronize(h->strm); oslam::stream_destroy(h->strm); }
     h->strm = s; h->owns_strm = false;
 }
 }
 }
 
+static int lba_create_impl(oslam_lba_t** out, int max_batch, int max_keyframes, int max_points, int max_edges, int device, hipStream_t caller, oslam::StreamRole role);
 int oslam_lba_create(oslam_lba_t** out, int max_batch, int max_keyframes, int max_points, int max_edges, int device) {
+    return lba_create_impl(out, max_batch, max_keyframes, max_points, max_edges, device, nullptr, oslam::kStreamSolver);
+}
+int oslam_lba_create_on_stream(oslam_lba_t** out, int max_batch, int max_keyframes, int max_points, int max_edges, int device, void* stream) {
+    if (!stream) { if (out) *out = nullptr; set_error("oslam_lba_create_on_stream: stream is NULL"); return OSLAM_E_INVALID; }
+    return lba_create_impl(out, max_batch, max_keyframes, max_points, max_edges, device, (hipStream_t)stream, oslam::kStreamSolver);
+}
+extern "C++" {
+namespace oslam {
+int lba_create_service(oslam_lba** out, int max_batch, int max_keyframes, int max_points, int max_edges, int device) {
+    return lba_create_impl(out, max_batch, max_keyframes, max_points, max_edges, device, nullptr, kStreamService);
+}
+}
+}
+static int lba_create_impl(oslam_lba_t** out, int max_batch, int max_keyframes, int max_points, int max_edges, int device, hipStream_t caller, oslam::StreamRole role) {
     if (!out) { set_error("out is NULL"); return OSLAM_E_INVALID; }
     *out = nullptr;
     if (max_batch < 1 || max_keyframes < 1 || max_keyframes > kLbaMaxWindowKF || max_points < 1 || max_edges < 1) {
@@ -2020,7 +2035,8 @@
     if (device < 0 || device >= ndev) { set_error("device out of range"); return OSLAM_E_INVALID; }
     OSLAM_HIP_CHECK(hipSetDevice(device));
     oslam_lba* h = new oslam_lba();
-    if (hipStreamCreateWithFlags(&h->strm, hipStreamNonBlocking) != hipSuccess) { set_error("hipStreamCreate failed"); delete h; return OSLAM_E_HIP; }
+    if (caller) { h->strm = caller; h->owns_strm = false; }
+    else if (oslam::stream_create(&h->strm, role) != hipSuccess) { set_error("hipStreamCreate failed"); delete h; return OSLAM_E_HIP; }
     h->device = device; h->max_batch = max_batch; h->max_kf = max_keyframes;
     if (const int rc = h->h_stop.alloc_mapped(sizeof(int))) { oslam_lba_destroy(h); return rc; }
     *h->h_stop.as<int>() = 0;
diff --git a/object_slam_amd/csrc/mappoint.hip b/object_slam_amd/csrc/mappoint.hip
--- a/object_slam_amd/csrc/mappoint.hip
+++ b/object_slam_amd/csrc/mappoint.hip
@@ -215,7 +215,7 @@
     if (!h) return;
     if (h->ev0) (void)hipEventDestroy(h->ev0);
     if (h->ev1) (void)hipEventDestroy(h->ev1);
-    if (h->strm && h->owns_strm) (void)hipStreamDestroy(h->strm);
+    if (h->strm && h->owns_strm) oslam::stream_destroy(h->strm);
     delete h;
 }
 
@@ -223,7 +223,7 @@
 namespace oslam {
 void mappoint_use_stream(oslam_mappoint* h, hipStream_t s) {
     if (!h || !s) return;
-    if (h->strm && h->owns_strm) (void)hipStreamDestroy(h->strm);
+    if (h->strm && h->owns_strm) oslam::stream_destroy(h->strm);
     h->strm = s; h->owns_strm = false;
 }
 }
@@ -1081,7 +1081,7 @@
     const size_t o_ok = take((size_t)M), o_x3 = take((size_t)M * 12);
     if (at > h->st.cap()) OSLAM_HIP_CHECK(hipDeviceSynchronize());
     OSLAM_CHECK(h->st.grow(at, 4096));
-    if (!h->strm) OSLAM_HIP_CHECK(hipStreamCreateWithFlags(&h->strm, hipStreamNonBlocking));
+    if (!h->strm) OSLAM_HIP_CHECK(oslam::stream_create(&h->strm, oslam::kStreamSolver));
     uint8_t* H = h->st.h.bytes();
     uint8_t* D = h->st.d.bytes();
     int* pair_of = (int*)(H + o_pair); int* d1 = (int*)(H + o_d1); int* d2 = (int*)(H + o_d2);
diff --git a/object_slam_amd/csrc/orb_extractor.hip b/object_slam_amd/csrc/orb_extractor.hip
--- a/object_slam_amd/csrc/orb_extractor.hip
+++ b/object_slam_amd/csrc/orb_extractor.hip
@@ -5,6 +5,8 @@
 #include <vector>
 
 #include "common.h"
+#include "stream_registry.h"
+#include <unordered_map>
 
 #include <time.h>
 #include <stdlib.h>
@@ -81,6 +83,49 @@
     return (short)std::min(std::max(i, -32768), 32767);
 }
 
+namespace {
+struct StreamReg {
+    std::mutex mu;
+    std::unordered_map<hipStream_t, int> of;
+    int64_t live[64][kStreamRoles] = {{0}};
+    int64_t declined[64] = {0};
+};
+StreamReg& stream_reg() { static StreamReg* r = new StreamReg; return *r; }
+}
+int stream_queue_budget() {
+    static const int budget = [] { const char* e = getenv("GPU_MAX_HW_QUEUES"); const int v = e ? atoi(e) : 0; return v > 0 ? v : 4; }();
+    return budget;
+}
+hipError_t stream_create(hipStream_t* s, StreamRole role) {
+    int dev = 0;
+    hipError_t e = hipGetDevice(&dev);
+    if (e != hipSuccess) return e;
+    (void)stream_queue_budget();
+    e = hipStreamCreateWithFlags(s, hipStreamNonBlocking);
+    if (e != hipSuccess) return e;
+    StreamReg& r = stream_reg();
+    std::lock_guard<std::mutex> lk(r.mu);
+    r.of[*s] = (dev & 63) * kStreamRoles + (int)role;
+    r.live[dev & 63][role]++;
+    return hipSuccess;
+}
+void stream_destroy(hipStream_t s) {
+    if (!s) return;
+    {
+        StreamReg& r = stream_reg();
+        std::lock_guard<std::mutex> lk(r.mu);
+        auto it = r.of.find(s);
+        if (it != r.of.end()) { r.live[it->second / kStreamRoles][it->second % kStreamRoles]--; r.of.erase(it); }
+    }
+    (void)hipStreamDestroy(s);
+}
+void stream_note_side_declined() {
+    int dev = 0;
+    if (hipGetDevice(&dev) != hipSuccess) return;
+    StreamReg& r = stream_reg();
+    std::lock_guard<std::mutex> lk(r.mu);
+    r.declined[dev & 63]++;
+}
 }
 
 using namespace oslam;
@@ -122,6 +167,7 @@
     size_t oct_lds = 0;
     DeviceBuffer d_oct_nodes; long long oct_nodes_stride = 0;
     hipStream_t side_stream = nullptr;
+    bool prof_blur_inline = false;
     hipEvent_t ev_fork = nullptr, ev_join = nullptr;
     hipStream_t fast0_stream = nullptr;
     hipEvent_t ev_fork0 = nullptr, ev_join0 = nullptr;
@@ -170,24 +216,41 @@
     return n;
 }
 
+int oslam_hip_stream_stats(int device, int64_t out[8]) {
+    if (!out || device < 0 || device >= 64) { set_error("oslam_hip_stream_stats: invalid argument"); return OSLAM_E_INVALID; }
+    StreamReg& r = stream_reg();
+    std::lock_guard<std::mutex> lk(r.mu);
+    out[0] = stream_queue_budget();
+    int64_t all = 0;
+    for (int k = 0; k < kStreamRoles; k++) { out[1 + k] = r.live[device][k]; all += r.live[device][k]; }
+    out[6] = r.declined[device];
+    out[7] = all;
+    return OSLAM_OK;
+}
+
 void oslam_orb_destroy(oslam_orb_t* h) {
     if (!h) return;
     for (hipEvent_t e : h->ev)
         if (e) (void)hipEventDestroy(e);
     if (h->ev_fork) (void)hipEventDestroy(h->ev_fork);
     if (h->ev_join) (void)hipEventDestroy(h->ev_join);
-    if (h->side_stream) (void)hipStreamDestroy(h->side_stream);
-    if (h->fast0_stream) (void)hipStreamDestroy(h->fast0_stream);
+    stream_destroy(h->side_stream);
+    stream_destroy(h->fast0_stream);
     if (h->ev_fork0) (void)hipEventDestroy(h->ev_fork0);
     if (h->ev_join0) (void)hipEventDestroy(h->ev_join0);
-    if (h->aux_stream) (void)hipStreamDestroy(h->aux_stream);
-    if (h->aux_side_stream) (void)hipStreamDestroy(h->aux_side_stream);
+    stream_destroy(h->aux_stream);
+    stream_destroy(h->aux_side_stream);
     for (hipEvent_t e : {h->ev_fork2, h->ev_join2, h->ev_fork3, h->ev_join3}) if (e) (void)hipEventDestroy(e);
     delete h;
 }
 
 int oslam_orb_create(oslam_orb_t** out, int nfeatures, float scaleFactor_, int nlevels, int iniTh, int minTh,
                      int width, int height, int max_batch, int device) {
+    return oslam_orb_create_flags(out, nfeatures, scaleFactor_, nlevels, iniTh, minTh, width, height, max_batch, device, 0);
+}
+
+int oslam_orb_create_flags(oslam_orb_t** out, int nfeatures, float scaleFactor_, int nlevels, int iniTh, int minTh,
+                           int width, int height, int max_batch, int device, int flags) {
     if (!out) { set_error("out is NULL"); return OSLAM_E_INVALID; }
     *out = nullptr;
     if (nfeatures <= 0 || nlevels < 1 || nlevels > OSLAM_MAX_LEVELS || !(scaleFactor_ > 1.0f) || width <= 0 ||
@@ -463,11 +526,12 @@
     ORB_CREATE_CHECK(hipFuncSetAttribute((const void*)k_octree_spill, hipFuncAttributeMaxDynamicSharedMemorySize, (int)h->oct_lds));
     ORB_CREATE_CHECK(hipFuncSetAttribute((const void*)k_octree_hbm, hipFuncAttributeMaxDynamicSharedMemorySize, (int)h->oct_lds));
     {
-        ORB_CREATE_CHECK(hipStreamCreateWithFlags(&h->side_stream, hipStreamNonBlocking));
+        if (flags & OSLAM_ORB_NO_SIDE_STREAM) stream_note_side_declined();
+        else ORB_CREATE_CHECK(stream_create(&h->side_stream, kStreamExtractorSide));
     }
     ORB_CREATE_CHECK(hipEventCreateWithFlags(&h->ev_fork, hipEventDisableTiming));
     if (getenv("OSLAM_ORB_FAST0_STREAM")) {
-        ORB_CREATE_CHECK(hipStreamCreateWithFlags(&h->fast0_stream, hipStreamNonBlocking));
+        ORB_CREATE_CHECK(stream_create(&h->fast0_stream, kStreamExtractorSide));
         ORB_CREATE_CHECK(hipEventCreateWithFlags(&h->ev_fork0, hipEventDisableTiming));
         ORB_CREATE_CHECK(hipEventCreateWithFlags(&h->ev_join0, hipEventDisableTiming));
     }
@@ -475,8 +539,8 @@
     if (getenv("OSLAM_ORB_SPLIT_MIN")) h->split_min = atoi(getenv("OSLAM_ORB_SPLIT_MIN"));
     h->no_lds_resize = getenv("OSLAM_ORB_NO_LDS_RESIZE") != nullptr;
     if (max_batch >= h->split_min) {
-        ORB_CREATE_CHECK(hipStreamCreateWithFlags(&h->aux_stream, hipStreamNonBlocking));
-        ORB_CREATE_CHECK(hipStreamCreateWithFlags(&h->aux_side_stream, hipStreamNonBlocking));
+        ORB_CREATE_CHECK(stream_create(&h->aux_stream, kStreamExtractorSide));
+        ORB_CREATE_CHECK(stream_create(&h->aux_side_stream, kStreamExtractorSide));
         for (hipEvent_t* e : {&h->ev_fork2, &h->ev_join2, &h->ev_fork3, &h->ev_join3}) ORB_CREATE_CHECK(hipEventCreateWithFlags(e, hipEventDisableTiming));
     }
 #undef ORB_CREATE_CHECK
@@ -507,7 +571,7 @@
 static int collect_profile(oslam_orb* h) {
     if (!h->prof_pending) return OSLAM_OK;
     OSLAM_HIP_CHECK(hipEventSynchronize(h->ev[5]));
-    const int a[5] = {0, 1, 6, 2, 4}, b[5] = {1, 2, 7, 3, 5};
+    const int a[5] = {0, h->prof_blur_inline ? 7 : 1, 6, 2, 4}, b[5] = {1, 2, 7, 3, 5};
     OSLAM_HIP_CHECK(hipEventSynchronize(h->ev[7]));
     for (int i = 0; i < 5; i++) {
         float ms = 0;
@@ -584,10 +648,20 @@
         }
         PROF_MARK(1);
         const bool overlap = sb != sm;
+        auto blur = [&]() -> int {
+            if (pr) OSLAM_HIP_CHECK(hipEventRecord(h->ev[6], sb));
+            hipLaunchKernelGGL(k_blur_strip<false>, dim3(P.blur_block_base[P.nlevels], nb), dim3(256), 0, sb, cs, h->blur_sse2);
+            hipLaunchKernelGGL(k_blur_strip<true>, dim3(P.blurb_block_base[P.nlevels], nb), dim3(256), 0, sb, cs, h->blur_sse2);
+            if (pr) OSLAM_HIP_CHECK(hipEventRecord(h->ev[7], sb));
+            return OSLAM_OK;
+        };
         if (overlap) {
             OSLAM_HIP_CHECK(hipEventRecord(fork, sm));
             OSLAM_HIP_CHECK(hipStreamWaitEvent(sb, fork, 0));
-        }
+        } else {
+            OSLAM_CHECK(blur());
+        }
+        if (pr) h->prof_blur_inline = !overlap;
         hipLaunchKernelGGL(k_fast_cells_wave, dim3(div_up(P.total_cells - cells0, 4 * kFastCellsPerWave), nb), dim3(256), 0, sm, cs, cells0, P.total_cells);
         if (cells0 > 0) OSLAM_HIP_CHECK(hipStreamWaitEvent(sm, h->ev_join0, 0));
         if (getenv("OSLAM_ORB_DEBUG_OVF")) { int n = 0; (void)hipStreamSynchronize(sm); (void)hipMemcpy(&n, cs.ovf_count, 4, hipMemcpyDeviceToHost); fprintf(stderr, "fast overflow cells since creation: %d (this batch has %d cells)\n", n, P.total_cells * nb); }
@@ -596,10 +670,7 @@
             hipLaunchKernelGGL(k_fast_cells, dim3(P.total_cells, nb), dim3(256), 0, sm, cs);
         }
         PROF_MARK(2);
-        if (pr) OSLAM_HIP_CHECK(hipEventRecord(h->ev[6], sb));
-        hipLaunchKernelGGL(k_blur_strip<false>, dim3(P.blur_block_base[P.nlevels], nb), dim3(256), 0, sb, cs, h->blur_sse2);
-        hipLaunchKernelGGL(k_blur_strip<true>, dim3(P.blurb_block_base[P.nlevels], nb), dim3(256), 0, sb, cs, h->blur_sse2);
-        if (pr) OSLAM_HIP_CHECK(hipEventRecord(h->ev[7], sb));
+        if (overlap) OSLAM_CHECK(blur());
         if (cs.oct_nodes) {
             plan.half_oct_nodes_hbm[hi] = 1;
             hipLaunchKernelGGL(k_octree_hbm, dim3(P.nlevels, nb), dim3(kOctThreads), h->oct_lds, sm, cs);
@@ -641,7 +712,7 @@
         const int nb0 = batch / 2, nb1 = batch - nb0;
         OSLAM_HIP_CHECK(hipEventRecord(h->ev_fork2, st));
         OSLAM_HIP_CHECK(hipStreamWaitEvent(h->aux_stream, h->ev_fork2, 0));
-        if ((rc = issue(c, nb0, st, h->side_stream, h->fast0_stream, h->ev_fork, h->ev_join, prof))) return rc;
+        if ((rc = issue(c, nb0, st, h->side_stream ? h->side_stream : st, h->fast0_stream, h->ev_fork, h->ev_join, prof))) return rc;
         if ((rc = issue(sub_ctx(nb0), nb1, h->aux_stream, h->aux_side_stream, nullptr, h->ev_fork3, h->ev_join3, false))) return rc;
         OSLAM_HIP_CHECK(hipEventRecord(h->ev_join2, h->aux_stream));
         OSLAM_HIP_CHECK(hipStreamWaitEvent(st, h->ev_join2, 0));
diff --git a/object_slam_amd/csrc/slam_driver.hip b/object_slam_amd/csrc/slam_driver.hip
--- a/object_slam_amd/csrc/slam_driver.hip
+++ b/object_slam_amd/csrc/slam_driver.hip
@@ -262,12 +262,8 @@
     k.id = (int)s.map.kfs.size() - 1;
     k.frameId = f.id; k.stamp = f.stamp; k.N = f.N;
     if (!s.lazyKeys) k.keys.assign(f.keys.begin(), f.keys.begin() + f.N);
-    k.keysUn.assign(f.keysUn.begin(), f.keysUn.begin() + f.N);
-    k.oct.resize(f.N);
-    for (int i = 0; i < f.N; i++) k.oct[i] = (uint8_t)f.keysUn[i].octave;
     if (!s.lazyDesc) k.desc.assign(f.desc.begin(), f.desc.begin() + (size_t)f.N * 32);
-    k.uRight.assign(f.uRight.begin(), f.uRight.begin() + f.N);
-    k.depth.assign(f.depth.begin(), f.depth.begin() + f.N);
+    copy_frame_rows(k, f);
     k.mp.assign(f.mp.begin(), f.mp.begin() + f.N);
     k.bowNode = f.bowNode;
     k.pose.set_keyframe(f.pose.Tcw);
@@ -1956,7 +1952,7 @@
     Ctx& c = T.c; const TrackInput& in = T.in;
     std::vector<int32_t> slots(T.S);
     std::vector<oslam_slam_frame_t*> outs(T.S);
-    for (int i = 0; i < T.S; i++) { slots[i] = i; outs[i] = &T.seq(i).cur->view; }
+    for (int i = 0; i < T.S; i++) { slots[i] = i; T.seq(i).cur->offer(); outs[i] = &T.seq(i).cur->view; }
     int rc;
     if (in.kind == TrackInput::STEREO) rc = c.ops.frames_stereo(c.ops.ctx, T.S, slots.data(), in.gray, in.right, in.gray_stride, in.on_device, outs.data());
     else if (in.kind == TrackInput::RAW16) rc = c.ops.frames_rgbd_raw16(c.ops.ctx, T.S, slots.data(), in.gray, in.gray_stride, in.depth16, in.depth_pitch, in.depth_factor, in.on_device, outs.data());
diff --git a/object_slam_amd/csrc/slam_map.h b/object_slam_amd/csrc/slam_map.h
--- a/object_slam_amd/csrc/slam_map.h
+++ b/object_slam_amd/csrc/slam_map.h
@@ -71,13 +71,23 @@
     }
 };
 
+template <class T> struct FrameRow {
+    std::vector<T> own;
+    const T* p = nullptr;
+    const T& operator[](size_t i) const { return p[i]; }
+    const T* data() const { return p; }
+    const T* begin() const { return p; }
+    bool external() const { return p != own.data(); }
+};
+
 struct Frame {
     int id = -1;
     double stamp = 0;
     int N = 0;
-    std::vector<KP> keys, keysUn;
+    std::vector<KP> keys;
+    FrameRow<KP> keysUn;
     std::vector<uint8_t> desc;
-    std::vector<float> uRight, depth;
+    FrameRow<float> uRight, depth;
     std::vector<int> mp;
     std::vector<uint8_t> outlier;
     std::vector<uint32_t> bowNode;
@@ -88,12 +98,16 @@
     std::vector<Obj2D> objs;
     std::vector<int> objOfKp;
     void alloc(int cap) {
-        keys.resize(cap); keysUn.resize(cap); desc.resize((size_t)cap * 32); uRight.resize(cap); depth.resize(cap);
+        keys.resize(cap); keysUn.own.resize(cap); desc.resize((size_t)cap * 32); uRight.own.resize(cap); depth.own.resize(cap);
         mp.assign(cap, -1); outlier.assign(cap, 0);
-        view.N = 0; view.keys = keys.data(); view.keysUn = keysUn.data(); view.desc = desc.data(); view.uRight = uRight.data(); view.depth = depth.data();
-    }
+        view.keys = keys.data(); view.desc = desc.data();
+        offer(); adopt(); view.N = 0;
+    }
+    void offer() { view.N = OSLAM_SLAM_FRAME_ROWS_IN_PLACE; view.keysUn = keysUn.own.data(); view.uRight = uRight.own.data(); view.depth = depth.own.data(); }
+    void adopt() { keysUn.p = view.keysUn; uRight.p = view.uRight; depth.p = view.depth; }
     void begin(int id_, double stamp_) {
         id = id_; stamp = stamp_; N = view.N;
+        adopt();
         std::fill(mp.begin(), mp.end(), -1);
         std::fill(outlier.begin(), outlier.end(), 0);
         bowNode.clear(); pose.valid = false; refKF = -1;
@@ -183,6 +197,14 @@
     bool firstConnection = true, bad = false;
     int trackRefForFrame = 0, fuseTargetForKF = 0;
 };
+
+inline void copy_frame_rows(KeyFrm& k, const Frame& f) {
+    k.keysUn.assign(f.keysUn.begin(), f.keysUn.begin() + f.N);
+    k.oct.resize(f.N);
+    for (int i = 0; i < f.N; i++) k.oct[i] = (uint8_t)f.keysUn[i].octave;
+    k.uRight.assign(f.uRight.begin(), f.uRight.begin() + f.N);
+    k.depth.assign(f.depth.begin(), f.depth.begin() + f.N);
+}
 
 struct RelPose { M4 Tcr; int refKF; double stamp; bool lost; };
 
diff --git a/object_slam_amd/csrc/slam_ops_hip.hip b/object_slam_amd/csrc/slam_ops_hip.hip
--- a/object_slam_amd/csrc/slam_ops_hip.hip
+++ b/object_slam_amd/csrc/slam_ops_hip.hip
@@ -95,6 +95,7 @@
     std::vector<int32_t> qm, qd;
     oslam::StagePair up;
     oslam::PinnedBuffer dn;
+    oslam::PinnedBuffer frame_rows[2]; int frame_rows_at = 0;
     oslam::StagePair upB;
     oslam::PinnedBuffer dnB;
     hipEvent_t tevB0 = nullptr, tevB1 = nullptr;
@@ -229,19 +230,26 @@
     o->d_kp = d_kp; o->d_desc = d_desc; o->d_cnt = d_cnt; o->cur_uRight = d_uR;
     const size_t cap = o->cap;
     StageLayout R;
-    const auto rCnt = R.add<int32_t>(n), rSt = R.add<int32_t>(2); const auto rKeys = R.add<oslam_keypoint_t>(cap * n), rKeysUn = R.add<oslam_keypoint_t>(cap * n);
-    const auto rDesc = R.add<uint8_t>(32 * cap * n); const auto rUr = R.add<float>(cap * n), rDp = R.add<float>(cap * n);
-    OSLAM_CHECK(o->ensure_dn(R.total()));
+    const auto rCnt = R.add<int32_t>(n), rSt = R.add<int32_t>(2); const auto rKeys = R.add<oslam_keypoint_t>(cap * n, !o->lazy_rows);
+    const auto rDesc = R.add<uint8_t>(32 * cap * n, !o->lazy_rows);
+    StageLayout A;
+    A.add<int32_t>(n); A.add<int32_t>(2); A.add<oslam_keypoint_t>(2 * cap * n); A.add<uint8_t>(32 * cap * n); A.add<float>(2 * cap * n);
+    OSLAM_CHECK(o->ensure_dn(std::max(R.total(), A.total())));
+    StageLayout F;
+    const auto rKeysUn = F.add<oslam_keypoint_t>(cap * o->S); const auto rUr = F.add<float>(cap * o->S), rDp = F.add<float>(cap * o->S);
+    for (oslam::PinnedBuffer& b : o->frame_rows) if (!b.ptr()) OSLAM_CHECK(b.alloc(F.total()));
+    o->frame_rows_at ^= 1;
     uint8_t* D = o->dn.bytes();
+    uint8_t* FR = o->frame_rows[o->frame_rows_at].bytes();
     int32_t* st = at(rSt, D);
     OSLAM_HIP_CHECK(hipMemcpyAsync(at(rCnt, D), d_cnt, rCnt.bytes, hipMemcpyDeviceToHost, o->strm));
     OSLAM_HIP_CHECK(hipMemcpyAsync(st, d_st, sizeof(*st), hipMemcpyDeviceToHost, o->strm));
     OSLAM_HIP_CHECK(hipMemcpyAsync(st + 1, o->d_status.as<int32_t>(), sizeof(*st), hipMemcpyDeviceToHost, o->strm));
     if (!o->lazy_rows) OSLAM_HIP_CHECK(hipMemcpyAsync(at(rKeys, D), d_kp, rKeys.bytes, hipMemcpyDeviceToHost, o->strm));
-    OSLAM_HIP_CHECK(hipMemcpyAsync(at(rKeysUn, D), o->d_keysUn.as<oslam_keypoint_t>(), rKeysUn.bytes, hipMemcpyDeviceToHost, o->strm));
+    OSLAM_HIP_CHECK(hipMemcpyAsync(at(rKeysUn, FR), o->d_keysUn.as<oslam_keypoint_t>(), sizeof(oslam_keypoint_t) * cap * n, hipMemcpyDeviceToHost, o->strm));
     if (!o->lazy_rows) OSLAM_HIP_CHECK(hipMemcpyAsync(at(rDesc, D), d_desc, rDesc.bytes, hipMemcpyDeviceToHost, o->strm));
-    OSLAM_HIP_CHECK(hipMemcpyAsync(at(rUr, D), d_uR, rUr.bytes, hipMemcpyDeviceToHost, o->strm));
-    OSLAM_HIP_CHECK(hipMemcpyAsync(at(rDp, D), d_dp, rDp.bytes, hipMemcpyDeviceToHost, o->strm));
+    OSLAM_HIP_CHECK(hipMemcpyAsync(at(rUr, FR), d_uR, sizeof(float) * cap * n, hipMemcpyDeviceToHost, o->strm));
+    OSLAM_HIP_CHECK(hipMemcpyAsync(at(rDp, FR), d_dp, sizeof(float) * cap * n, hipMemcpyDeviceToHost, o->strm));
     OSLAM_HIP_CHECK(oslam::stream_wait(o->strm));
     if (st[0]) { oslam::set_error("extractor arena overflow"); return OSLAM_E_CAPACITY; }
     if (st[1]) { oslam::set_error("keypoint outside the depth image / right extractor arena overflow"); return OSLAM_E_INVALID; }
@@ -249,12 +257,11 @@
     o->pool->parallel_for(n, [&](int i) {
         oslam_slam_frame_t* f = out[i];
         const size_t N = cnt[i];
+        const bool in_place = f->N == OSLAM_SLAM_FRAME_ROWS_IN_PLACE;
         f->N = (int)N;
-        if (!o->lazy_rows) copy_elems(f->keys, row(rKeys, D, cap, i), N);
-        copy_elems(f->keysUn, row(rKeysUn, D, cap, i), N);
-        if (!o->lazy_rows) copy_elems(f->desc, row(rDesc, D, 32 * cap, i), 32 * N);
-        copy_elems(f->uRight, row(rUr, D, cap, i), N);
-        copy_elems(f->depth, row(rDp, D, cap, i), N);
+        if (in_place) { f->keysUn = row(rKeysUn, FR, cap, i); f->uRight = row(rUr, FR, cap, i); f->depth = row(rDp, FR, cap, i); }
+        else { copy_elems(f->keysUn, row(rKeysUn, FR, cap, i), N); copy_elems(f->uRight, row(rUr, FR, cap, i), N); copy_elems(f->depth, row(rDp, FR, cap, i), N); }
+        if (!o->lazy_rows) { copy_elems(f->keys, row(rKeys, D, cap, i), N); copy_elems(f->desc, row(rDesc, D, 32 * cap, i), 32 * N); }
     });
     return OSLAM_OK;
 }
@@ -1142,7 +1149,7 @@
         const int nthreads = std::max(1, getenv("OSLAM_LBA_SERVICE_THREADS") ? atoi(getenv("OSLAM_LBA_SERVICE_THREADS")) : 2);
         for (int t = 0; t < nthreads; t++) {
             std::unique_ptr<Worker> wk(new Worker);
-            int rc = oslam_lba_create(&wk->ba, max_batch, 1 << 16, 4096, 32768, device);
+            int rc = oslam::lba_create_service(&wk->ba, max_batch, 1 << 16, 4096, 32768, device);
             if (!rc) rc = oslam_lba_set_mode(wk->ba, 1);
             if (rc) { oslam_lba_destroy(wk->ba); return rc; }
             oslam::lba_use_gate(wk->ba, &launch_mu);
@@ -2038,7 +2045,7 @@
     if (o->tevB0) (void)hipEventDestroy(o->tevB0);
     if (o->tevB1) (void)hipEventDestroy(o->tevB1);
     if (o->tev1) (void)hipEventDestroy(o->tev1);
-    if (o->strm) (void)hipStreamDestroy(o->strm);
+    oslam::stream_destroy(o->strm);
     delete o;
 }
 
@@ -2054,9 +2061,12 @@
     o->cfg = *cfg; o->S = cfg->n_sequences;
     o->mp_tab.resize(o->S); o->pt_aux.resize(o->S);
     o->pool = new oslam_drv::Pool(cfg->host_threads > 1 ? cfg->host_threads : 1,  false);
-    if (hipStreamCreateWithFlags(&o->strm, hipStreamNonBlocking) != hipSuccess) o->strm = nullptr;
+    if (oslam::stream_create(&o->strm, oslam::kStreamHandle) != hipSuccess) o->strm = nullptr;
     const int dev = cfg->device;
-    int rc = oslam_orb_create(&o->orb, cfg->nFeatures, cfg->scaleFactor, cfg->nLevels, cfg->iniThFAST, cfg->minThFAST, cfg->width, cfg->height, o->S, dev);
+    const int orb_flags = 0;
+    int rc = o->strm ? OSLAM_OK : OSLAM_E_HIP;
+    if (rc) oslam::set_error("slam ops: hipStreamCreate failed");
+    if (!rc) rc = oslam_orb_create_flags(&o->orb, cfg->nFeatures, cfg->scaleFactor, cfg->nLevels, cfg->iniThFAST, cfg->minThFAST, cfg->width, cfg->height, o->S, dev, orb_flags);
     if (!rc) {
         o->cap = oslam_orb_max_keypoints(o->orb);
         o->rec_lay = oslam::KfRecordLayout(o->cap);
@@ -2064,15 +2074,14 @@
         rc = oslam_matcher_create(&o->m_last, o->S, o->cap, o->cap, dev);
     }
     if (!rc) rc = oslam_matcher_create(&o->m_map, o->S, o->cap, o->max_local, dev);
-    if (!rc && cfg->sensor == 1) rc = oslam_orb_create(&o->orbR, cfg->nFeatures, cfg->scaleFactor, cfg->nLevels, cfg->iniThFAST, cfg->minThFAST, cfg->width, cfg->height, o->S, dev);
+    if (!rc && cfg->sensor == 1) rc = oslam_orb_create_flags(&o->orbR, cfg->nFeatures, cfg->scaleFactor, cfg->nLevels, cfg->iniThFAST, cfg->minThFAST, cfg->width, cfg->height, o->S, dev, orb_flags);
     if (!rc && cfg->sensor == 1) rc = oslam_stereo_create(&o->stereo, o->S, o->cap, dev);
     if (!rc) rc = oslam_poseopt_create(&o->po, o->S, o->cap, dev);
-    if (!rc) rc = oslam_lba_create(&o->ba1, 1, 1 << 16, 4096, 32768, dev);
+    if (!rc) rc = oslam_lba_create_on_stream(&o->ba1, 1, 1 << 16, 4096, 32768, dev, o->strm);
     if (!rc) rc = oslam_mappoint_create(&o->mp, dev);
     if (!rc) rc = oslam_frame_create(&o->fr, dev);
     if (!rc) rc = oslam_bow_create(&o->bow, o->cap, dev);
-    if (!rc && o->strm) {
-        oslam::lba_use_stream(o->ba1, o->strm);
+    if (!rc) {
         oslam::bow_use_stream(o->bow, o->strm);
         oslam::mappoint_use_stream(o->mp, o->strm);
     }
diff --git a/object_slam_amd/csrc/stream_registry.h b/object_slam_amd/csrc/stream_registry.h
--- /dev/null
+++ b/object_slam_amd/csrc/stream_registry.h
@@ -0,0 +1,22 @@
+#pragma once
+#include <hip/hip_runtime.h>
+
+#include <cstdint>
+
+namespace oslam {
+
+enum StreamRole {
+    kStreamHandle = 0,
+    kStreamExtractorSide = 1,
+    kStreamSolver = 2,
+    kStreamService = 3,
+    kStreamOther = 4,
+    kStreamRoles = 5
+};
+
+hipError_t stream_create(hipStream_t* s, StreamRole role);
+void stream_destroy(hipStream_t s);
+void stream_note_side_declined();
+int stream_queue_budget();
+
+}
diff --git a/object_slam_amd/extractor.py b/object_slam_amd/extractor.py
--- a/object_slam_amd/extractor.py
+++ b/object_slam_amd/extractor.py
@@ -19,8 +19,13 @@
 
 class ORBextractor(_lib.Handle):
     def __init__(self, nfeatures, scaleFactor, nlevels, iniThFAST, minThFAST, width, height,
-                 max_batch=1, device=0):
-        super().__init__(_lib.lib(), "oslam_orb", nfeatures, scaleFactor, nlevels, iniThFAST, minThFAST, width, height, max_batch, device)
+                 max_batch=1, device=0, side_stream=True):
+        if side_stream:
+            super().__init__(_lib.lib(), "oslam_orb", nfeatures, scaleFactor, nlevels, iniThFAST, minThFAST, width, height, max_batch, device)
+        else:
+            L = _lib.lib()
+            self.L, self.h, self._destroy = L, C.c_void_p(), "oslam_orb_destroy"
+            check(L.oslam_orb_create_flags(C.byref(self.h), nfeatures, scaleFactor, nlevels, iniThFAST, minThFAST, width, height, max_batch, device, _lib.ORB_NO_SIDE_STREAM))
         self.nfeatures, self.nlevels = nfeatures, nlevels
         self.width, self.height, self.max_batch = width, height, max_batch
         self.cap = self.L.oslam_orb_max_keypoints(self.h)
```

New measurement: 51510 (median of 6 runs). No clear change (+0.7%).
